# facebookresearch/momentum

Hardware: AMD Instinct MI355X
Metric: character IK solves/sec (72-joint, 10 GN iters) (higher is better)
Workload: dtype f32; 1 GPU; BASELINE configs[1]: B x 72-joint humanoid, P=128, pos+ori on 16 landmarks (M=192), GN lambda=0.05, 10 it; batch_per_gpu=4096, global_batch=4096, joints=72, params=128, rows=192, solved_parameters=96, route=fused, line_search=0, precision=f32

## Files before the change

include/mmx.h:

```cpp
#ifndef MMX_H_
#define MMX_H_

#include <stddef.h>
#include <stdint.h>

#ifdef __cplusplus
extern "C" {
#endif

#define MMX_ABI_VERSION 12
#define MMX_PARAMS_PER_JOINT 7
#define MMX_INVALID_PARENT (-1)
#define MMX_MAX_MODEL_PARAMS 2048

typedef enum mmx_status {
  MMX_OK = 0,
  MMX_ERR_INVALID_ARGUMENT = 1,
  MMX_ERR_SIZE_MISMATCH = 2,
  MMX_ERR_DEVICE = 3,
  MMX_ERR_UNSUPPORTED = 4,
  MMX_ERR_OUT_OF_MEMORY = 5,
  MMX_ERR_NO_DEVICE = 6
} mmx_status;

// ... 106 lines not shown
  float limit_function_weight;
  float pos_loss_alpha, pos_loss_c;
  float ori_loss_alpha, ori_loss_c;
  int32_t num_joint_blocks;
  const mmx_joint_constraint_block* joint_blocks;
  int32_t num_ellipsoid_limits;
  const mmx_ellipsoid_limit* ellipsoid_limits;
  const float* function_weights;
  int32_t num_function_weights;
} mmx_constraint_data;

#define MMX_LINE_SEARCH_NONE 0
#define MMX_LINE_SEARCH_GAUSS_NEWTON 1
#define MMX_LINE_SEARCH_DIRECTIONAL 2

typedef struct mmx_gn_options {
  int32_t min_iterations;
  int32_t max_iterations;
  float threshold;
  float regularization;
  int32_t do_line_search;
  int32_t step_rule;
  float lm_lambda_min;
  float lm_lambda_max;
  float lm_up;
  float lm_down;
  float trust_region_radius;
  int32_t precision;
  float precision_bound;
} mmx_gn_options;

typedef struct mmx_rig mmx_rig;
typedef struct mmx_problem mmx_problem;

void mmx_gn_options_default(mmx_gn_options* opt);

int32_t mmx_abi_version(void);
const char* mmx_last_error(void);
int32_t mmx_device_count(void);

int32_t mmx_rig_create(const mmx_rig_desc* desc, int32_t device, mmx_rig** out);
void mmx_rig_destroy(mmx_rig* rig);
int32_t mmx_rig_num_joints(const mmx_rig* rig);
int32_t mmx_rig_num_params(const mmx_rig* rig);

int32_t mmx_problem_create(
    mmx_rig* rig,
    int32_t batch,
    int32_t num_pos,
    const int32_t* pos_parent,
    int32_t num_ori,
    const int32_t* ori_parent,
    mmx_problem** out);
void mmx_problem_destroy(mmx_problem* problem);

int32_t mmx_problem_set_instance_rig(
    mmx_problem* problem,
    const float* translation_offset,
    const float* pre_rotation,
    int32_t memory,
    void* stream);

int32_t mmx_problem_set_instance_parents(
    mmx_problem* problem,
    const int32_t* pos_parent,
    const int32_t* ori_parent,
    int32_t memory,
    void* stream);

#define MMX_ROUTE_AUTO 0
#define MMX_ROUTE_FUSED 1
#define MMX_ROUTE_WIDE 2
#define MMX_ROUTE_EXPLICIT_JACOBIAN 3
#define MMX_ROUTE_WAVE 4
#define MMX_WAVE_MAX_JOINTS 64
#define MMX_WAVE_MAX_SOLVED 32
#define MMX_WAVE_MAX_UNITS 192
typedef struct mmx_tuning {
  int32_t route;
  int32_t max_refinement_steps;
  float mixed_tolerance;
  int32_t mixed_max_cg;
  int32_t joint_pruning;
  int32_t reserved[3];
} mmx_tuning;
int32_t mmx_problem_set_tuning(mmx_problem* problem, const mmx_tuning* tuning);
int32_t mmx_problem_last_route(const mmx_problem* problem);
int32_t mmx_problem_num_solve_joints(const mmx_problem* problem);

int32_t mmx_problem_num_rows(const mmx_problem* problem);
int32_t mmx_problem_batch(const mmx_problem* problem);

int32_t mmx_problem_set_enabled(mmx_problem* problem, const uint8_t* enabled);

int32_t mmx_problem_set_constraints(
    mmx_problem* problem,
    const mmx_constraint_data* data,
    void* stream);
int32_t mmx_problem_set_constraints_sized(
    mmx_problem* problem,
    const mmx_constraint_data* data,
    size_t data_size,
    void* stream);

int32_t mmx_eval_jacobian(
    mmx_problem* problem,
    const float* theta_dev,
    float* jac_dev,
    float* res_dev,
    double* err_dev,
    int32_t layout,
    void* stream);

int32_t mmx_eval_jacobian_timed(
    mmx_problem* problem,
    const float* theta_dev,
    float* jac_dev,
    float* res_dev,
    double* err_dev,
    int32_t layout,
    void* stream,
    float* kernel_ms);

int32_t mmx_debug_store_pattern(mmx_problem* problem, float* jac_dev, void* stream, float* kernel_ms);

int32_t mmx_eval_skeleton_state(
    mmx_problem* problem,
    const float* theta_dev,
    float* state_dev,
    void* stream);

int32_t mmx_eval_normal_equations(
    mmx_problem* problem,
    const float* theta_dev,
    float* jtj_dev,
    float* jtr_dev,
    double* err_dev,
    void* stream);

int32_t mmx_solve(
    mmx_problem* problem,
    const mmx_gn_options* options,
    float* theta_dev,
    double* final_error,
    int32_t* iterations,
    int32_t* status,
    double* error_history,
    void* stream);

int32_t mmx_solve_f64(
    mmx_problem* problem,
    const mmx_gn_options* options,
    double* theta_dev,
    double* final_error,
    int32_t* iterations,
    int32_t* status,
    double* error_history,
    void* stream);

int32_t mmx_solve_with_history(
    mmx_problem* problem,
    const mmx_gn_options* options,
    float* theta_dev,
    double* final_error,
    int32_t* iterations,
    int32_t* status,
    double* error_history,
    float* parameter_history,
    void* stream);

int32_t mmx_solve_with_step_history(
// ... 9 lines not shown
    void* stream);

int32_t mmx_solve_frames(
    mmx_problem* problem,
    const mmx_gn_options* options,
    int32_t num_frames,
    float* theta_dev,
    double* final_error,
    int32_t* iterations,
    int32_t* status,
    double* error_history,
    float* parameter_history,
    void* stream);
int32_t mmx_solve_frames_host(
    mmx_problem* problem,
    const mmx_gn_options* options,
    int32_t num_frames,
    float* theta_host,
    double* final_error_host,
    int32_t* iterations_host,
    int32_t* status_host);

int32_t mmx_problem_solve_diagnostics(mmx_problem* problem, float* diag_dev, void* stream);

int32_t mmx_debug_fused_normal_equations(
    mmx_problem* problem,
    const float* theta_dev,
    float* jtj_dev,
    float* jtr_dev,
    int32_t* solve_list_host,
    int32_t* num_solved,
    void* stream);

int32_t mmx_debug_tree_normal_equations(mmx_problem* problem, const float* theta_dev, float* jtj_dev, float* jtr_dev, void* stream);

int32_t mmx_solve_host(
    mmx_problem* problem,
    const mmx_gn_options* options,
    float* theta_host,
    double* final_error_host,
    int32_t* iterations_host,
    int32_t* status_host);
int32_t mmx_solve_f64_host(
    mmx_problem* problem,
    const mmx_gn_options* options,
    double* theta_host,
    double* final_error_host,
    int32_t* iterations_host,
    int32_t* status_host);
int32_t mmx_eval_jacobian_host(
    mmx_problem* problem,
    const float* theta_host,
    float* jac_host,
    float* res_host,
    double* err_host,
    int32_t layout);
int32_t mmx_eval_skeleton_state_host(mmx_problem* problem, const float* theta_host, float* state_host);

#define MMX_COMM_ID_BYTES 128
typedef struct mmx_comm mmx_comm;
int32_t mmx_comm_unique_id(uint8_t id[MMX_COMM_ID_BYTES]);
int32_t mmx_comm_create(const uint8_t id[MMX_COMM_ID_BYTES], int32_t world_size, int32_t rank, int32_t device, mmx_comm** out);
int32_t mmx_comm_create_all(int32_t num_devices, const int32_t* devices, mmx_comm** out );
int32_t mmx_comm_world_size(const mmx_comm* comm);
int32_t mmx_comm_rank(const mmx_comm* comm);
int32_t mmx_comm_all_reduce_norms(mmx_comm* comm, double* norms_dev, void* stream);
int32_t mmx_comm_all_reduce_norms_host(mmx_comm* comm, double norms_host[3]);
int32_t mmx_residual_norms(int32_t batch, const double* final_error, const int32_t* iterations, const int32_t* status, double* norms_dev, void* stream);
void mmx_comm_destroy(mmx_comm* comm);

int32_t mmx_host_tables(
    const mmx_rig_desc* desc,
    const uint8_t* enabled,
    int32_t* level,
    int32_t* tin,
    int32_t* tout,
    uint8_t* active_joint_params,
    int32_t* enabled_list,
    int32_t* num_enabled);

int32_t mmx_host_elimination_order(const mmx_rig_desc* desc, const uint8_t* enabled, int32_t* order, int32_t* num_enabled);
int32_t mmx_host_tile_structure(int32_t n, const uint8_t* related, uint32_t* row_mask, uint32_t* col_mask, int64_t* products);
int32_t mmx_host_live_joints(const mmx_rig_desc* desc, int32_t n, const int32_t* joints, uint8_t* live, int32_t* compact_of, int32_t* num_live);
int32_t mmx_problem_tile_structure(mmx_problem* problem, uint32_t* row_mask, uint32_t* col_mask, int32_t* num_blocks, int32_t* num_tiles, int64_t* products);
int32_t mmx_host_tile_level_schedule(int32_t n, const uint8_t* related, int32_t* steps);
int32_t mmx_host_f64_assembly_list(
    const mmx_rig_desc* desc,
    const int32_t* solve_list,
    int32_t n,
    const int32_t* pos_parent,
    int32_t num_pos,
    const int32_t* ori_parent,
    int32_t num_ori,
    int32_t units_per_chunk,
    uint32_t* groups,
    int32_t* num_groups,
    int32_t* extra,
    int32_t* num_extra,
    int32_t* chunk_start,
    int32_t* num_chunks);

#ifdef __cplusplus
}
#endif
#endif
```

momentum_amd/_abi.py:

```python
from __future__ import annotations

import ctypes as C

import numpy as np

c_float_p = C.POINTER(C.c_float)
c_double_p = C.POINTER(C.c_double)
c_int32_p = C.POINTER(C.c_int32)
c_uint8_p = C.POINTER(C.c_uint8)

MMX_ABI_VERSION = 12
MMX_OK = 0
MMX_SOLVE_OK, MMX_SOLVE_NONFINITE, MMX_SOLVE_NOT_PD = 0, 1, 2
MMX_SOLVE_DAMPING_FLOORED = 4
MMX_SOLVE_PRECISION_SUSPECT = 8
MMX_SOLVE_ESCALATED_F64 = 16
MMX_SOLVE_MIXED = 32
MMX_SOLVE_ERROR_MASK = 3
MMX_PRECISION_F32, MMX_PRECISION_F64, MMX_PRECISION_AUTO, MMX_PRECISION_MIXED = 0, 1, 2, 3
MMX_MEM_HOST, MMX_MEM_DEVICE = 0, 1
MMX_LAYOUT_COL_MAJOR, MMX_LAYOUT_ROW_MAJOR = 0, 1
MMX_STEP_GN_FIXED_LAMBDA, MMX_STEP_LM_SCHEDULE, MMX_STEP_TRUST_REGION = 0, 1, 2


# ... 219 lines not shown
        ("ori_weight", C.c_void_p),
        ("pos_function_weight", C.c_float),
        ("ori_function_weight", C.c_float),
        ("memory", C.c_int32),
        ("model_target", C.c_void_p),
        ("model_weights", C.c_void_p),
        ("model_function_weight", C.c_float),
        ("num_limits", C.c_int32),
        ("limits", C.c_void_p),
        ("limit_function_weight", C.c_float),
        ("pos_loss_alpha", C.c_float),
        ("pos_loss_c", C.c_float),
        ("ori_loss_alpha", C.c_float),
        ("ori_loss_c", C.c_float),
        ("num_joint_blocks", C.c_int32),
        ("joint_blocks", C.c_void_p),
        ("num_ellipsoid_limits", C.c_int32),
        ("ellipsoid_limits", C.c_void_p),
        ("function_weights", C.c_void_p),
        ("num_function_weights", C.c_int32),
    ]


class GnOptions(C.Structure):

    _fields_ = [
        ("min_iterations", C.c_int32),
        ("max_iterations", C.c_int32),
        ("threshold", C.c_float),
        ("regularization", C.c_float),
        ("do_line_search", C.c_int32),
        ("step_rule", C.c_int32),
        ("lm_lambda_min", C.c_float),
        ("lm_lambda_max", C.c_float),
        ("lm_up", C.c_float),
        ("lm_down", C.c_float),
        ("trust_region_radius", C.c_float),
        ("precision", C.c_int32),
        ("precision_bound", C.c_float),
    ]

    @classmethod
    def make(
        cls,
        min_iterations=1,
        max_iterations=2,
        threshold=1.0,
        regularization=0.05,
        do_line_search=False,
        step_rule=MMX_STEP_GN_FIXED_LAMBDA,
        lm_lambda_min=1e-6,
        lm_lambda_max=1e6,
        lm_up=4.0,
        lm_down=0.5,
        trust_region_radius=1.0,
        precision=MMX_PRECISION_F32,
        precision_bound=1e-5,
    ) -> "GnOptions":
        return cls(
            int(min_iterations),
            int(max_iterations),
            float(threshold),
            float(regularization),
            int(do_line_search),
            int(step_rule),
            float(lm_lambda_min),
            float(lm_lambda_max),
            float(lm_up),
            float(lm_down),
            float(trust_region_radius),
            int(precision),
            float(precision_bound),
        )


ROUTES = {"auto": 0, "fused": 1, "wide": 2, "explicit_jacobian": 3, "wave": 4}
WAVE_MAX_JOINTS = 64
WAVE_MAX_SOLVED = 32
WAVE_MAX_UNITS = 192


class Tuning(C.Structure):

    _fields_ = [("route", C.c_int32), ("max_refinement_steps", C.c_int32), ("mixed_tolerance", C.c_float), ("mixed_max_cg", C.c_int32), ("joint_pruning", C.c_int32), ("reserved", C.c_int32 * 3)]


def as_ptr(a: np.ndarray, ctype):
    assert a.flags["C_CONTIGUOUS"], "array must be C-contiguous"
    return a.ctypes.data_as(C.POINTER(ctype))


def void_p(a) -> C.c_void_p:
    if a is None:
        return C.c_void_p(0)
    if isinstance(a, np.ndarray):
        assert a.flags["C_CONTIGUOUS"]
        return C.c_void_p(a.ctypes.data)
    return C.c_void_p(int(a))
```

momentum_amd/capi.py:

```python
from __future__ import annotations

import ctypes as C
import os
from typing import Optional

import numpy as np

from . import _abi
from ._abi import ConstraintData, GnOptions, RigDesc, as_ptr
from .rigs import Rig

_HERE = os.path.dirname(os.path.abspath(__file__))
LIB_PATH = os.environ.get("MMX_LIB") or os.path.join(_HERE, "libmmx_hip.so")
_lib: Optional[C.CDLL] = None

SYMBOLS = [
    "mmx_gn_options_default", "mmx_abi_version", "mmx_last_error", "mmx_device_count",
    "mmx_rig_create", "mmx_rig_destroy", "mmx_rig_num_joints", "mmx_rig_num_params",
    "mmx_problem_create", "mmx_problem_destroy", "mmx_problem_num_rows", "mmx_problem_batch",
    "mmx_problem_set_tuning", "mmx_problem_last_route", "mmx_problem_num_solve_joints",
    "mmx_problem_set_enabled", "mmx_problem_set_constraints", "mmx_problem_set_constraints_sized", "mmx_problem_set_instance_rig", "mmx_problem_set_instance_parents", "mmx_eval_jacobian", "mmx_eval_jacobian_timed", "mmx_debug_store_pattern",
    "mmx_eval_skeleton_state", "mmx_eval_normal_equations", "mmx_solve", "mmx_solve_with_history", "mmx_solve_with_step_history", "mmx_problem_solve_diagnostics", "mmx_solve_f64", "mmx_solve_f64_host", "mmx_solve_host",
    "mmx_solve_frames", "mmx_solve_frames_host",
    "mmx_eval_jacobian_host", "mmx_eval_skeleton_state_host", "mmx_host_tables", "mmx_debug_fused_normal_equations", "mmx_debug_tree_normal_equations",
    "mmx_host_elimination_order", "mmx_host_tile_structure", "mmx_host_tile_level_schedule", "mmx_host_f64_assembly_list", "mmx_problem_tile_structure", "mmx_host_live_joints",
    "mmx_comm_unique_id", "mmx_comm_create", "mmx_comm_create_all", "mmx_comm_world_size", "mmx_comm_rank",
    "mmx_comm_all_reduce_norms", "mmx_comm_all_reduce_norms_host", "mmx_residual_norms", "mmx_comm_destroy",
]


class MmxError(RuntimeError):

    def __init__(self, code: int, msg: str):
        super().__init__(f"mmx error {code}: {msg}")
        self.code = code


def lib() -> C.CDLL:
    global _lib
    if _lib is not None:
        return _lib
    if not os.path.exists(LIB_PATH):
        raise MmxError(-1, f"{LIB_PATH} is missing: build it with `python -m momentum_amd.build` (no CPU fallback exists)")
    try:
        import torch
    except Exception:
        pass
    L = C.CDLL(LIB_PATH)
    vp, i32 = C.c_void_p, C.c_int32
    L.mmx_last_error.restype = C.c_char_p
    L.mmx_gn_options_default.restype = None
    L.mmx_gn_options_default.argtypes = [C.POINTER(GnOptions)]
    L.mmx_rig_create.argtypes = [C.POINTER(RigDesc), i32, C.POINTER(vp)]
    L.mmx_rig_destroy.argtypes = [vp]
    L.mmx_rig_destroy.restype = None
    L.mmx_rig_num_joints.argtypes = [vp]
    L.mmx_rig_num_params.argtypes = [vp]
    L.mmx_problem_create.argtypes = [vp, i32, i32, _abi.c_int32_p, i32, _abi.c_int32_p, C.POINTER(vp)]
    L.mmx_problem_destroy.argtypes = [vp]
    L.mmx_problem_destroy.restype = None
    L.mmx_problem_num_rows.argtypes = [vp]
    L.mmx_problem_batch.argtypes = [vp]
    L.mmx_problem_set_enabled.argtypes = [vp, _abi.c_uint8_p]
    L.mmx_problem_set_tuning.argtypes = [vp, C.POINTER(_abi.Tuning)]
    L.mmx_problem_last_route.argtypes = [vp]
    L.mmx_problem_num_solve_joints.argtypes = [vp]
    L.mmx_problem_set_constraints.argtypes = [vp, C.POINTER(ConstraintData), vp]
    L.mmx_problem_set_constraints_sized.argtypes = [vp, C.POINTER(ConstraintData), C.c_size_t, vp]
    L.mmx_problem_set_instance_rig.argtypes = [vp, vp, vp, i32, vp]
    L.mmx_problem_set_instance_parents.argtypes = [vp, vp, vp, i32, vp]
    L.mmx_eval_jacobian.argtypes = [vp, vp, vp, vp, vp, i32, vp]
    L.mmx_eval_jacobian_timed.argtypes = [vp, vp, vp, vp, vp, i32, vp, C.POINTER(C.c_float)]
    L.mmx_debug_store_pattern.argtypes = [vp, vp, vp, C.POINTER(C.c_float)]
    L.mmx_eval_skeleton_state.argtypes = [vp, vp, vp, vp]
    L.mmx_eval_normal_equations.argtypes = [vp, vp, vp, vp, vp, vp]
    L.mmx_solve.argtypes = [vp, C.POINTER(GnOptions), vp, vp, vp, vp, vp, vp]
    L.mmx_solve_with_history.argtypes = [vp, C.POINTER(GnOptions), vp, vp, vp, vp, vp, vp, vp]
    L.mmx_solve_with_step_history.argtypes = [vp, C.POINTER(GnOptions), vp, vp, vp, vp, vp, vp, vp, vp]
    L.mmx_problem_solve_diagnostics.argtypes = [vp, vp, vp]
    L.mmx_solve_f64.argtypes = [vp, C.POINTER(GnOptions), vp, vp, vp, vp, vp, vp]
    L.mmx_solve_host.argtypes = [vp, C.POINTER(GnOptions), vp, vp, vp, vp]
    L.mmx_solve_f64_host.argtypes = [vp, C.POINTER(GnOptions), vp, vp, vp, vp]
    L.mmx_solve_frames.argtypes = [vp, C.POINTER(GnOptions), i32, vp, vp, vp, vp, vp, vp, vp]
    L.mmx_solve_frames_host.argtypes = [vp, C.POINTER(GnOptions), i32, vp, vp, vp, vp]
    L.mmx_eval_jacobian_host.argtypes = [vp, vp, vp, vp, vp, i32]
    L.mmx_eval_skeleton_state_host.argtypes = [vp, vp, vp]
    L.mmx_debug_tree_normal_equations.argtypes = [vp, vp, vp, vp, vp]
    L.mmx_debug_fused_normal_equations.argtypes = [vp, vp, vp, vp, _abi.c_int32_p, _abi.c_int32_p, vp]
    L.mmx_comm_unique_id.argtypes = [vp]
    L.mmx_comm_create.argtypes = [vp, i32, i32, i32, C.POINTER(vp)]
    L.mmx_comm_create_all.argtypes = [i32, _abi.c_int32_p, C.POINTER(vp)]
    L.mmx_comm_world_size.argtypes = [vp]
    L.mmx_comm_rank.argtypes = [vp]
    L.mmx_comm_all_reduce_norms.argtypes = [vp, vp, vp]
    L.mmx_comm_all_reduce_norms_host.argtypes = [vp, vp]
    L.mmx_residual_norms.argtypes = [i32, vp, vp, vp, vp, vp]
    L.mmx_comm_destroy.argtypes = [vp]
    L.mmx_comm_destroy.restype = None
    L.mmx_host_tables.argtypes = [
        C.POINTER(RigDesc), _abi.c_uint8_p, _abi.c_int32_p, _abi.c_int32_p, _abi.c_int32_p,
        _abi.c_uint8_p, _abi.c_int32_p, _abi.c_int32_p,
    ]
    u32p, i64p = C.POINTER(C.c_uint32), C.POINTER(C.c_int64)
    L.mmx_host_elimination_order.argtypes = [C.POINTER(RigDesc), _abi.c_uint8_p, _abi.c_int32_p, _abi.c_int32_p]
    L.mmx_host_tile_structure.argtypes = [i32, _abi.c_uint8_p, u32p, u32p, i64p]
    L.mmx_host_tile_level_schedule.argtypes = [i32, _abi.c_uint8_p, C.POINTER(C.c_int32)]
    L.mmx_problem_tile_structure.argtypes = [vp, u32p, u32p, _abi.c_int32_p, _abi.c_int32_p, i64p]
    L.mmx_host_live_joints.argtypes = [C.POINTER(RigDesc), i32, _abi.c_int32_p, _abi.c_uint8_p, _abi.c_int32_p, _abi.c_int32_p]
    _lib = L
    return L


def _check(rc: int) -> None:
    if rc != 0:
        raise MmxError(rc, lib().mmx_last_error().decode("utf-8", "replace"))


def device_count() -> int:
    return int(lib().mmx_device_count())


def host_tables(rig: Rig, enabled=None) -> dict:
    J, P = rig.num_joints, rig.num_params
    level, tin, tout = (np.zeros(J, np.int32) for _ in range(3))
    active = np.zeros(7 * J, np.uint8)
    elist = np.zeros(P, np.int32)
    n = C.c_int32(0)
    d = rig.desc()
    if enabled is None:
        eptr = _abi.c_uint8_p()
    else:
        e = np.ascontiguousarray(enabled, dtype=np.uint8)
        eptr = as_ptr(e, C.c_uint8)
    _check(
        lib().mmx_host_tables(
            C.byref(d), eptr, as_ptr(level, C.c_int32), as_ptr(tin, C.c_int32), as_ptr(tout, C.c_int32),
            as_ptr(active, C.c_uint8), as_ptr(elist, C.c_int32), C.byref(n),
        )
    )
    order = np.zeros(P, np.int32)
    _check(lib().mmx_host_elimination_order(C.byref(d), eptr, as_ptr(order, C.c_int32), C.byref(n)))
    return dict(level=level, tin=tin, tout=tout, active_joint_params=active, enabled_list=elist[: n.value].copy(),
                elimination_order=order[: n.value].copy())


def host_live_joints(rig: Rig, joints) -> dict:
    J = rig.num_joints
    jl = np.ascontiguousarray(joints, dtype=np.int32).reshape(-1)
    live, compact = np.zeros(J, np.uint8), np.zeros(J, np.int32)
    n = C.c_int32(0)
    d = rig.desc()
    jptr = as_ptr(jl, C.c_int32) if jl.size else _abi.c_int32_p()
    _check(lib().mmx_host_live_joints(C.byref(d), C.c_int32(jl.size), jptr, as_ptr(live, C.c_uint8), as_ptr(compact, C.c_int32), C.byref(n)))
    return dict(live=live, compact_of=compact, num_live=int(n.value))


def host_tile_structure(related: np.ndarray):
    rel = np.ascontiguousarray(related, dtype=np.uint8)
    n = rel.shape[0]
    assert rel.shape == (n, n)
    row, col = np.zeros(32, np.uint32), np.zeros(32, np.uint32)
    prod = C.c_int64(0)
    _check(lib().mmx_host_tile_structure(C.c_int32(n), as_ptr(rel, C.c_uint8), as_ptr(row, C.c_uint32), as_ptr(col, C.c_uint32), C.byref(prod)))
    return dict(row_mask=row, col_mask=col, products=prod.value)


def host_tile_level_schedule(related: np.ndarray):
    rel = np.ascontiguousarray(related, dtype=np.uint8)
    n = rel.shape[0]
    assert rel.shape == (n, n)
    words = np.zeros(1 + 4 * 32, np.int32)
    _check(lib().mmx_host_tile_level_schedule(C.c_int32(n), as_ptr(rel, C.c_uint8), as_ptr(words, C.c_int32)))
    steps = []
    for s in range(int(words[0])):
        steps.append([(int(w) & 0xff, (int(w) >> 8) & 0xf, (int(w) >> 12) & 0xf) for w in words[1 + 4 * s : 5 + 4 * s] if w >= 0])
    return steps


def host_f64_assembly_list(rig: Rig, solve_list, pos_parent, ori_parent, units_per_chunk: int):
    sl = np.ascontiguousarray(solve_list, dtype=np.int32)
    pp = np.ascontiguousarray(pos_parent, dtype=np.int32)
    op = np.ascontiguousarray(ori_parent, dtype=np.int32)
    d = rig.desc()
    ng, ne, nc = C.c_int32(0), C.c_int32(0), C.c_int32(0)
    i32p = C.POINTER(C.c_int32)
    args = lambda g, e, cs: (C.byref(d), as_ptr(sl, C.c_int32), C.c_int32(len(sl)), as_ptr(pp, C.c_int32), C.c_int32(len(pp)), as_ptr(op, C.c_int32),
                             C.c_int32(len(op)), C.c_int32(units_per_chunk), g, C.byref(ng), e, C.byref(ne), cs, C.byref(nc))
    f = lib().mmx_host_f64_assembly_list
    f.restype = C.c_int32
    _check(f(*args(None, None, None)))
    groups = np.zeros(2 * max(ng.value, 1), np.uint32)
    extra = np.zeros(max(ne.value, 1), np.int32)
    cstart = np.zeros(2 * nc.value + 1, np.int32)
    _check(f(*args(groups.ctypes.data_as(C.POINTER(C.c_uint32)), extra.ctypes.data_as(i32p), cstart.ctypes.data_as(i32p))))
    chunks = []
    for ch in range(nc.value):
        entries = []
        for g in range(cstart[ch], cstart[ch + 1]):
            w0, w1 = int(groups[2 * g]), int(groups[2 * g + 1])
            c, ul, count = w0 & 0xfff, (w0 >> 12) & 0x3f, w0 >> 18
            entries.append((c, ul, [w1] if count == 1 else [int(x) for x in extra[w1 : w1 + count]]))
        chunks.append(dict(block_mask=int(cstart[nc.value + 1 + ch]), entries=entries))
    return chunks


def _stream_ptr() -> C.c_void_p:
    import torch

    return C.c_void_p(torch.cuda.current_stream().cuda_stream)


def _dev(t) -> C.c_void_p:
    return C.c_void_p(0 if t is None else t.data_ptr())


class RigHandle:

    def __init__(self, rig: Rig, device: int = 0):
        self.rig = rig
        self.device = int(device)
        self._h = C.c_void_p(0)
        d = rig.desc()
        _check(lib().mmx_rig_create(C.byref(d), self.device, C.byref(self._h)))

    def close(self) -> None:
        if self._h:
            lib().mmx_rig_destroy(self._h)
            self._h = C.c_void_p(0)

    def __del__(self):
        try:
            self.close()
        except Exception:
            pass


default_route = "auto"


class Problem:

    def __init__(self, rig_handle: RigHandle, batch: int, pos_parent, ori_parent):
        import torch

        self.rh = rig_handle
        self.B = int(batch)
        self.P = rig_handle.rig.num_params
        self.J = rig_handle.rig.num_joints
        self.pos_parent = np.ascontiguousarray(pos_parent, dtype=np.int32).reshape(-1)
        self.ori_parent = np.ascontiguousarray(ori_parent, dtype=np.int32).reshape(-1)
        self.Kp, self.Ko = len(self.pos_parent), len(self.ori_parent)
        self.M = 3 * self.Kp + 9 * self.Ko
        self.n = self.P
        self.device = torch.device("cuda", rig_handle.device)
        self._h = C.c_void_p(0)
        self._keep = []
        _check(
            lib().mmx_problem_create(
                rig_handle._h, self.B, self.Kp, as_ptr(self.pos_parent, C.c_int32), self.Ko,
                as_ptr(self.ori_parent, C.c_int32), C.byref(self._h),
            )
        )
        self._prefer_wide = default_route == "prefer_wide"
        if default_route not in ("auto", "prefer_wide"):
            self.set_route(default_route)

    def close(self) -> None:
        if self._h:
            lib().mmx_problem_destroy(self._h)
            self._h = C.c_void_p(0)

    def __del__(self):
        try:
            self.close()
        except Exception:
            pass

    def set_route(self, route: str, max_refinement_steps: int = 0) -> None:
        self._prefer_wide = default_route == "prefer_wide" and route == "auto"
        self._set_tuning(route, max_refinement_steps)

    def _set_tuning(self, route: str, max_refinement_steps: int = 0) -> None:
        t = _abi.Tuning()
        t.route = _abi.ROUTES[route]
        t.max_refinement_steps = int(max_refinement_steps)
        t.mixed_tolerance, t.mixed_max_cg = getattr(self, "_mixed", (0.0, 0))
        t.joint_pruning = 0 if getattr(self, "_joint_pruning", True) else -1
        self._route_args = (route, int(max_refinement_steps))
        _check(lib().mmx_problem_set_tuning(self._h, C.byref(t)))

    def set_mixed(self, tolerance: float = 0.0, max_cg: int = 0) -> None:
        self._mixed = (float(tolerance), int(max_cg))
        self._set_tuning(*getattr(self, "_route_args", ("auto", 0)))

    def set_joint_pruning(self, on: bool = True) -> None:
        self._joint_pruning = bool(on)
        self._set_tuning(*getattr(self, "_route_args", ("auto", 0)))

    def num_solve_joints(self) -> int:
        return int(lib().mmx_problem_num_solve_joints(self._h))

    def last_route(self) -> str:
        r = int(lib().mmx_problem_last_route(self._h))
        return {v: k for k, v in _abi.ROUTES.items()}[r]

    def set_enabled(self, enabled) -> None:
        e = np.ascontiguousarray(enabled, dtype=np.uint8).reshape(-1)
        assert e.shape[0] == self.P
        _check(lib().mmx_problem_set_enabled(self._h, as_ptr(e, C.c_uint8)))
        self.n = int(np.count_nonzero(e))

    def set_constraints(
        self, pos_offset, pos_target, pos_weight, ori_offset, ori_target, ori_weight,
        pos_function_weight: float = 1.0, ori_function_weight: float = 1.0,
        limits=None, limit_function_weight: float = 1.0,
        model_target=None, model_weights=None, model_function_weight: float = 1.0,
        pos_loss=(2.0, 1.0), ori_loss=(2.0, 1.0), joint_blocks=None, ellipsoid_limits=None, function_weights=None,
    ) -> None:
        import torch

        arrs = [pos_offset, pos_target, pos_weight, ori_offset, ori_target, ori_weight]
        shapes = [(self.B, self.Kp, 3), (self.B, self.Kp, 3), (self.B, self.Kp), (self.B, self.Ko, 4), (self.B, self.Ko, 4), (self.B, self.Ko)]
        if model_target is not None:
            arrs += [model_target, model_weights]
            shapes += [(self.B, self.P), (self.B, self.P)]
        on_dev = all(isinstance(a, torch.Tensor) for a in arrs)
        keep, ptrs = [], []
        for a, shp in zip(arrs, shapes):
            if on_dev:
                assert a.is_cuda and a.dtype == torch.float32 and a.is_contiguous() and tuple(a.shape) == shp, (a.shape, shp)
                keep.append(a)
                ptrs.append(C.c_void_p(a.data_ptr() if a.numel() else 0))
            else:
                x = np.ascontiguousarray(a, dtype=np.float32).reshape(shp)
                keep.append(x)
                ptrs.append(C.c_void_p(x.ctypes.data if x.size else 0))
        if model_target is None:
            ptrs += [C.c_void_p(0), C.c_void_p(0)]
        fw_ptr, fw_cols = C.c_void_p(0), 0
        if function_weights is not None:
            if on_dev:
                assert function_weights.is_cuda and function_weights.dtype == torch.float32 and function_weights.is_contiguous() and function_weights.shape[0] == self.B
                keep.append(function_weights)
                fw_ptr, fw_cols = C.c_void_p(function_weights.data_ptr()), int(function_weights.shape[1])
            else:
                fwh = np.ascontiguousarray(function_weights, dtype=np.float32).reshape(self.B, -1)
                keep.append(fwh)
                fw_ptr, fw_cols = C.c_void_p(fwh.ctypes.data), int(fwh.shape[1])
        limits = list(limits) if limits else []
        larr = _abi.limit_array(limits)
        blocks = list(joint_blocks) if joint_blocks else []
        bkeep: list = []
        barr = _abi.joint_block_array(blocks, bkeep, self.B, on_dev)
        ells = list(ellipsoid_limits) if ellipsoid_limits else []
        earr = _abi.ellipsoid_array(ells)
        cd = ConstraintData(
            *ptrs[:6], float(pos_function_weight), float(ori_function_weight), _abi.MMX_MEM_DEVICE if on_dev else _abi.MMX_MEM_HOST,
            ptrs[6], ptrs[7], float(model_function_weight), len(limits), C.cast(larr, C.c_void_p) if limits else None, float(limit_function_weight),
            float(pos_loss[0]), float(pos_loss[1]), float(ori_loss[0]), float(ori_loss[1]),
            len(blocks), C.cast(barr, C.c_void_p) if blocks else None,
            len(ells), C.cast(earr, C.c_void_p) if ells else None,
            fw_ptr, fw_cols,
        )
        _check(lib().mmx_problem_set_constraints_sized(self._h, C.byref(cd), C.sizeof(cd), _stream_ptr()))
        self._keep = keep + bkeep if on_dev else []
        self.M = int(lib().mmx_problem_num_rows(self._h))

    def set_instance_rig(self, translation_offset=None, pre_rotation=None) -> None:
        self._keep_rig = self._instance_call(
            lib().mmx_problem_set_instance_rig, [(translation_offset, (self.B, self.J, 3)), (pre_rotation, (self.B, self.J, 4))], "float32"
        )

    def set_instance_parents(self, pos_parent=None, ori_parent=None) -> None:
        self._keep_parents = self._instance_call(
            lib().mmx_problem_set_instance_parents, [(pos_parent, (self.B, self.Kp)), (ori_parent, (self.B, self.Ko))], "int32"
        )

    def _instance_call(self, fn, arrays, dtype):
        import torch

# ... 285 lines not shown
```

momentum_amd/csrc/mmx_capi.hip:

```cpp
#include "../../include/mmx.h"

#include <hip/hip_runtime.h>

#include <dlfcn.h>

#include <cfloat>
#include <cmath>
#include <cstdio>
#include <cstdlib>
#include <cstring>
#include <algorithm>
#include <new>
#include <map>
#include <memory>
#include <string>
#include <vector>

#include "mmx_host_tables.hpp"
#include "mmx_kernels.hpp"

namespace {

thread_local std::string g_lastError;

// ... 112 lines not shown

struct mmx_rig {
  int32_t device = 0;
  int32_t J = 0, P = 0;
  std::vector<int32_t> parent, ptOuter, ptInner;
  std::vector<float> preRot, offset, ptValue, ptOffsets;
  mmx::HostTables topo;
  DevBuf dParent, dPreRot, dOffset, dPtOuter, dPtInner, dPtValue, dPtOffsets, dLevelOrder, dLevelStart, dPtEll, dJumpParent, dPtRowRec;
  mmx::RigDev dev{};

  mmx_rig_desc desc() const {
    mmx_rig_desc d{};
    d.num_joints = J;
    d.num_params = P;
    d.parent = parent.data();
    d.pre_rotation = preRot.data();
    d.translation_offset = offset.data();
    d.pt_outer = ptOuter.data();
    d.pt_inner = ptInner.data();
    d.pt_value = ptValue.data();
    d.pt_offsets = ptOffsets.data();
    return d;
  }
};

struct mmx_problem {
  mmx_rig* rig = nullptr;
  int32_t B = 0, Kp = 0, Ko = 0, U = 0, M = 0;
  std::vector<int32_t> posParent, oriParent;
  mmx::RigDev rigDev{};
  DevBuf oInstOffset, oInstPreRot, oInstPosParent, oInstOriParent, dJointTin;
  std::vector<int32_t> unionPos, unionOri;
  std::vector<int32_t> instPosHost, instOriHost;
  bool instParentsFromHost = false;
  bool instPos = false, instOri = false;
  mmx::HostTables tables;
  mmx::FusedTables fused;
  DevBuf dUnitJoint, dUnitTin, dColStart, dColSources, dEnabledList, dJacRecs, dMultiCols, dZeroCols;
  DevBuf dSubSize, dPosUnitStart, dPosUnits, dSolveList, dSrcStart, dSrcs, dTerms, dTerms16, dComb, dDfsJoint, dLoadedPos;
  DevBuf dLimStart, dLimOf, dPairDest, dPairStart, dPairLim, dPairCols;
  mmx::FusedDev fdev{};
  DevBuf oPosOffset, oPosTarget, oPosWeight, oOriOffset, oOriTarget, oOriWeight, oMpTarget, oMpWeights, dLimits, dEnabledMask, oFnWeights;
  std::vector<mmx_parameter_limit> limits;
  struct JointBlockHost {
    int32_t type = 0, count = 0;
    std::vector<int32_t> parent;
    std::vector<int32_t> parentB;
    DevBuf oLocalPoint, oLocalDir, oGlobal, oPlaneD, oWeight, oProjection;
  };
  std::vector<std::unique_ptr<JointBlockHost>> blocks;
  std::vector<mmx::JointBlockDev> blockDev;
  std::vector<mmx_ellipsoid_limit> ellipsoids;
  DevBuf dEllipsoids;
  DevBuf dBlocks, dGenJoint, dGenTin, dGenBlock;
  int32_t genRows = 0;
  bool haveConstraints = false;
  bool tablesDirty = false;
  mmx::ProblemDev dev{};
  int32_t solveN = 0;
  DevBuf dSolveListV1;
  DevBuf sHess2F64;
  DevBuf dSolveListF64;
  std::vector<int32_t> solveListF64;
  std::vector<std::pair<int32_t, int32_t>> limitPairs;
  DevBuf dTileMasks, dTileList;
  mmx::TileMasks tileMasks;
  std::vector<int32_t> solveListV1;
  DevBuf sJac, sRes, sErr, sJtj, sJtr, sFactor, sThetaInit, sTheta;
  DevBuf sTreeState, sDvec, sRhoVec, sRefState, sGenState;
  DevBuf sJacColMajor;
  DevBuf sJacF64, sHessF64;
  DevBuf dF64Groups, dF64Extra, dF64ChunkStart;
  int32_t f64ListUnitsPerChunk = 0;
  DevBuf sDone, sIters, sStatus, sLastErr, sFinalErr, sHist, sClk, sDelta, sStepIter, sLambda, sTrust;
  DevBuf sFusedArgs;
  DevBuf sDiag;
  DevBuf sDiagAcc;
  DevBuf sDiagErr0;
  bool diagValid = false;
  DevBuf sThetaAuto, sAutoMap, sAutoCount;
  bool autoAbort = false;
  mmx_tuning tuning{};
  int32_t lastRoute = MMX_ROUTE_AUTO;
  mmx::LiveJoints liveJoints;
  bool viewBuilt = false;
  mmx::RigDev vRig{};
  int32_t vNnz = 0;
  DevBuf vParent, vPreRot, vOffset, vPtOuter, vPtInner, vPtValue, vPtOffsets, vLevelOrder, vLevelStart, vPtEll, vJumpParent, vPtRowRec;
  DevBuf vUnitJoint, vUnitTin, vJointTin, vGenJoint, vGenTin, vEllipsoids, vLimits;
  DevBuf vSubSize, vDfsJoint, vLoadedPos, vPosUnitStart, vSrcs;
};

namespace {

std::vector<int32_t> limitParameters(const mmx_rig* rig, const mmx_parameter_limit& lm) {
  std::vector<int32_t> out;
  auto add = [&](int32_t p) {
    if (std::find(out.begin(), out.end(), p) == out.end()) {
      out.push_back(p);
    }
  };
  auto addRow = [&](int32_t row) {
    for (int32_t k = rig->ptOuter[size_t(row)]; k < rig->ptOuter[size_t(row) + 1]; ++k) {
      add(rig->ptInner[size_t(k)]);
    }
  };
  switch (lm.type) {
    case MMX_LIMIT_MINMAX:
      add(lm.index0);
      break;
    case MMX_LIMIT_LINEAR:
    case MMX_LIMIT_HALFPLANE:
      add(lm.index0);
      add(lm.index1);
      break;
    case MMX_LIMIT_MINMAX_JOINT:
      addRow(lm.index0);
      break;
    case MMX_LIMIT_LINEAR_JOINT:
      addRow(lm.index1);
      addRow(lm.index0);
      break;
    default:
      break;
  }
  return out;
}

struct RigDerived {
  std::vector<int32_t> ell, jumpParent, rowRec;
  bool ellOk = true;
  int32_t jumpRounds = 0;
};
RigDerived deriveRigTables(
    int32_t J, int32_t P, const std::vector<int32_t>& parent, const std::vector<int32_t>& ptOuter, const std::vector<int32_t>& ptInner,
    const std::vector<float>& ptValue, int32_t numLevels) {
  RigDerived o;
  const int32_t R = MMX_PARAMS_PER_JOINT * J;
  o.ell.assign(size_t(R) * 4, 0);
  o.jumpParent.assign(size_t(J), 0);
  for (int32_t row = 0; row < R; ++row) {
    const int32_t k0 = ptOuter[size_t(row)], k1 = ptOuter[size_t(row) + 1];
    if (k1 - k0 > 2) {
      o.ellOk = false;
      break;
    }
    for (int s = 0; s < 2; ++s) {
      int32_t idx = -1, bits = 0;
      if (k0 + s < k1) {
        idx = ptInner[size_t(k0 + s)];
        std::memcpy(&bits, &ptValue[size_t(k0 + s)], 4);
      }
      o.ell[4 * size_t(row) + 2 * s] = idx;
      o.ell[4 * size_t(row) + 2 * s + 1] = bits;
    }
  }
  for (int32_t j = 0; j < J; ++j) {
    o.jumpParent[size_t(j)] = ((parent[size_t(j)] + 1) << 16) | (parent[size_t(j)] + 1);
  }
  if (R < 65536 && P <= 65535) {
    std::vector<int32_t> rows;
    for (int32_t row = 0; row < R; ++row) {
      if (ptOuter[size_t(row) + 1] > ptOuter[size_t(row)]) {
        rows.push_back(row);
      }
    }
// ... 1228 lines not shown
  if (batch <= 0 || num_pos < 0 || num_ori < 0) {
    return fail(MMX_ERR_INVALID_ARGUMENT, "batch must be > 0 and constraint counts >= 0");
  }
  if ((num_pos > 0 && pos_parent == nullptr) || (num_ori > 0 && ori_parent == nullptr)) {
    return fail(MMX_ERR_INVALID_ARGUMENT, "constraint parent array is null");
  }
  for (int32_t c = 0; c < num_pos; ++c) {
    if (pos_parent[c] < 0 || pos_parent[c] >= rig->J) {
      return fail(MMX_ERR_INVALID_ARGUMENT, "position constraint parent joint out of range");
    }
  }
  for (int32_t c = 0; c < num_ori; ++c) {
    if (ori_parent[c] < 0 || ori_parent[c] >= rig->J) {
      return fail(MMX_ERR_INVALID_ARGUMENT, "orientation constraint parent joint out of range");
    }
  }
  mmx_problem* pb = new (std::nothrow) mmx_problem();
  if (pb == nullptr) {
    return fail(MMX_ERR_OUT_OF_MEMORY, "host allocation failed");
  }
  pb->rig = rig;
  pb->B = batch;
  pb->Kp = num_pos;
  pb->Ko = num_ori;
  pb->U = num_pos + 3 * num_ori;
  pb->M = 3 * pb->U;
  pb->dev.lossPos = mmx::LossDev{0, 2.f, 1.f, 1.f};
  pb->dev.lossOri = mmx::LossDev{0, 2.f, 1.f, 1.f};
  if (num_pos > 0) {
    pb->posParent.assign(pos_parent, pos_parent + num_pos);
  }
  if (num_ori > 0) {
    pb->oriParent.assign(ori_parent, ori_parent + num_ori);
  }
  pb->tables = rig->topo;
  pb->rigDev = rig->dev;
  pb->dev.wPos = 1.f;
  pb->dev.wOri = 1.f;
  const int32_t rc = uploadProblemTables(pb);
  if (rc != MMX_OK) {
    delete pb;
    return rc;
  }
  *out = pb;
  return MMX_OK;
}

void mmx_problem_destroy(mmx_problem* pb) {
  if (pb != nullptr) {
    if (pb->rig != nullptr) {
      (void)hipSetDevice(pb->rig->device);
    }
    delete pb;
  }
}

int32_t mmx_problem_num_rows(const mmx_problem* pb) {
  return pb ? pb->M : 0;
}
int32_t mmx_problem_batch(const mmx_problem* pb) {
  return pb ? pb->B : 0;
}

int32_t mmx_problem_set_tuning(mmx_problem* pb, const mmx_tuning* tuning) {
  int32_t rc = checkProblem(pb, false);
  if (rc != MMX_OK) {
    return rc;
  }
  if (tuning == nullptr) {
    return fail(MMX_ERR_INVALID_ARGUMENT, "tuning is null");
  }
  if (tuning->route < MMX_ROUTE_AUTO || tuning->route > MMX_ROUTE_WAVE) {
    return fail(MMX_ERR_INVALID_ARGUMENT, "mmx_tuning::route: unknown MMX_ROUTE_* value");
  }
  if (tuning->max_refinement_steps < -1 || tuning->max_refinement_steps > 3) {
    return fail(MMX_ERR_INVALID_ARGUMENT, "mmx_tuning::max_refinement_steps: -1 (none), 0 (default) or 1..3");
  }
  if (!(tuning->mixed_tolerance >= 0.f) || tuning->mixed_tolerance > 1e-2f || tuning->mixed_max_cg < 0 || tuning->mixed_max_cg > 64) {
    return fail(MMX_ERR_INVALID_ARGUMENT, "mmx_tuning::mixed_tolerance: 0 (default) or (0, 1e-2]; mixed_max_cg: 0 (default) or 1..64");
  }
  if (tuning->joint_pruning != 0 && tuning->joint_pruning != -1) {
    return fail(MMX_ERR_INVALID_ARGUMENT, "mmx_tuning::joint_pruning: 0 (on) or -1 (off)");
  }
  for (int32_t r : tuning->reserved) {
    if (r != 0) {
      return fail(MMX_ERR_INVALID_ARGUMENT, "mmx_tuning::reserved must be zero");
    }
  }
  pb->tuning = *tuning;
  return MMX_OK;
}

int32_t mmx_problem_last_route(const mmx_problem* pb) {
  return pb != nullptr ? pb->lastRoute : MMX_ROUTE_AUTO;
}

int32_t mmx_problem_num_solve_joints(const mmx_problem* pb) {
  if (pb == nullptr || pb->rig == nullptr) {
    return 0;
  }
  return solveViewActive(pb) ? pb->liveJoints.numLive : pb->rig->J;
}

int32_t mmx_problem_set_enabled(mmx_problem* pb, const uint8_t* enabled) {
  MMX_ZONE("mmx_problem_set_enabled");
  int32_t rc = checkProblem(pb, false);
  if (rc != MMX_OK) {
    return rc;
  }
  if (enabled == nullptr) {
    return fail(MMX_ERR_INVALID_ARGUMENT, "enabled is null");
  }
  if (!pb->tablesDirty && pb->tables.enabled.size() == size_t(pb->rig->P)) {
    bool same = true;
    for (size_t p = 0; p < pb->tables.enabled.size() && same; ++p) {
      same = (pb->tables.enabled[p] != 0) == (enabled[p] != 0);
    }
    if (same) {
      return MMX_OK;
    }
  }
  const mmx_rig_desc d = pb->rig->desc();
  std::string err;
  mmx::HostTables t;
  rc = mmx::buildHostTables(&d, enabled, t, err);
  if (rc != MMX_OK) {
    return fail(rc, err);
  }
  pb->tables = std::move(t);
  return uploadProblemTables(pb);
}

int32_t mmx_problem_set_instance_rig(mmx_problem* pb, const float* translation_offset, const float* pre_rotation, int32_t memory, void* stream) {
  MMX_ZONE("mmx_problem_set_instance_rig");
  int32_t rc = checkProblem(pb, false);
  if (rc != MMX_OK) {
    return rc;
  }
  if (memory != MMX_MEM_HOST && memory != MMX_MEM_DEVICE) {
    return fail(MMX_ERR_INVALID_ARGUMENT, "instance rig: unknown memory space");
  }
  MMX_HIP(hipSetDevice(pb->rig->device));
  hipStream_t s = static_cast<hipStream_t>(stream);
  const size_t B = size_t(pb->B), J = size_t(pb->rig->J);
  auto bring = [&](DevBuf& buf, const float* src, size_t count, const float*& dst) -> hipError_t {
    if (src == nullptr) {
      dst = nullptr;
      return hipSuccess;
    }
    if (memory == MMX_MEM_DEVICE) {
      dst = src;
      return hipSuccess;
    }
    hipError_t e = buf.ensure(count * sizeof(float));
    if (e != hipSuccess) {
      return e;
    }
    dst = buf.as<float>();
    return hipMemcpyAsync(buf.p, src, count * sizeof(float), hipMemcpyHostToDevice, s);
  };
  const float *off = nullptr, *pre = nullptr;
  MMX_HIP(bring(pb->oInstOffset, translation_offset, B * J * 3, off));
  MMX_HIP(bring(pb->oInstPreRot, pre_rotation, B * J * 4, pre));
  if (memory == MMX_MEM_HOST) {
    MMX_HIP(hipStreamSynchronize(s));
  }
  pb->rigDev.instOffset = off;
  pb->rigDev.instPreRot = pre;
  return MMX_OK;
}

int32_t mmx_problem_set_instance_parents(mmx_problem* pb, const int32_t* pos_parent, const int32_t* ori_parent, int32_t memory, void* stream) {
  MMX_ZONE("mmx_problem_set_instance_parents");
  int32_t rc = checkProblem(pb, false);
  if (rc != MMX_OK) {
    return rc;
  }
  if (memory != MMX_MEM_HOST && memory != MMX_MEM_DEVICE) {
    return fail(MMX_ERR_INVALID_ARGUMENT, "instance parents: unknown memory space");
  }
  MMX_HIP(hipSetDevice(pb->rig->device));
  hipStream_t s = static_cast<hipStream_t>(stream);
  const size_t B = size_t(pb->B);
  std::vector<int32_t> hp, ho;
// ... 658 lines not shown
    double* error_history,
    double* step_history,
    const mmx::F64Select& select,
    void* stream);
static int32_t preflightF64(mmx_problem* pb);

static bool mixedUsable(const mmx_problem* pb, const mmx_gn_options* o) {
  if (o == nullptr || pb == nullptr || pb->rig == nullptr) {
    return false;
  }
  const int32_t route = pb->tuning.route;
  return (route == MMX_ROUTE_AUTO || route == MMX_ROUTE_FUSED) && o->step_rule != MMX_STEP_TRUST_REGION && pb->fdev.GT == 0 &&
      pb->U > 0 && pb->fdev.n > 0 && fusedUsable(pb) &&
      mmx::fusedMixedUsable(pb->rig->J, pb->rig->P, pb->U, pb->fdev.nsrc, pb->fdev.n, pb->fdev.numCells);
}

static const char* waveRefusal(const mmx_problem* pb, const mmx_gn_options* o, bool frames = false) {
  const mmx::ProblemDev& d = pb->dev;
  if (pb->rig->J > MMX_WAVE_MAX_JOINTS) {
    return "MMX_ROUTE_WAVE: more than MMX_WAVE_MAX_JOINTS (64) joints";
  }
  if (pb->fdev.n > MMX_WAVE_MAX_SOLVED) {
    return "MMX_ROUTE_WAVE: more than MMX_WAVE_MAX_SOLVED (32) solved parameters";
  }
  if (pb->fdev.n <= 0 || pb->U <= 0) {
    return "MMX_ROUTE_WAVE: no solved parameter, or no position / orientation constraint";
  }
  if (pb->U > MMX_WAVE_MAX_UNITS) {
    return "MMX_ROUTE_WAVE: more than MMX_WAVE_MAX_UNITS (192) constraint vectors (positions + 3 x orientations)";
  }
  if (d.lossPos.type != 0 || d.lossOri.type != 0) {
    return "MMX_ROUTE_WAVE: robust losses are outside the route (L2 only)";
  }
  if (d.numBlocks > 0 || d.G > 0 || pb->fdev.GT > 0) {
    return "MMX_ROUTE_WAVE: further joint-constraint blocks are outside the route";
  }
  if (d.NE > 0) {
    return "MMX_ROUTE_WAVE: ellipsoid limits are outside the route";
  }
  if (d.NL > 0) {
    return "MMX_ROUTE_WAVE: parameter limits are outside the route";
  }
  if (d.hasModel != 0 || d.M > d.rowsJoint) {
    return "MMX_ROUTE_WAVE: the model-parameter prior is outside the route";
  }
  if (d.instPosParent != nullptr || d.instOriParent != nullptr) {
    return "MMX_ROUTE_WAVE: per-instance constraint parents are outside the route";
  }
  if (o->step_rule != MMX_STEP_GN_FIXED_LAMBDA) {
    return "MMX_ROUTE_WAVE: only MMX_STEP_GN_FIXED_LAMBDA (not the LM schedule, not the trust region)";
  }
  if (mmx::waveLdsBytes(pb->rig->J, pb->rig->P, pb->U, pb->fdev.n, frames) > 160 * 1024) {
    return "MMX_ROUTE_WAVE: the parameter vector does not fit a wave's share of LDS";
  }
  return nullptr;
}

static int32_t solveMixedImpl(
    mmx_problem* pb,
    const mmx_gn_options* o,
    float* theta_dev,
    double* final_error,
    int32_t* iterations,
    int32_t* status,
    double* error_history,
    float* parameter_history,
    double* step_history,
    const mmx::MixSelect& sel,
    void* stream) {
  MMX_ZONE("mmx_solve, mixed precision (SolverT<double>::solve around a single-precision factor)");
  if (o->max_iterations < 0 || o->min_iterations < 0) {
    return fail(MMX_ERR_INVALID_ARGUMENT, "iteration counts must be >= 0");
  }
  if (o->step_rule != MMX_STEP_GN_FIXED_LAMBDA && o->step_rule != MMX_STEP_LM_SCHEDULE) {
    return fail(MMX_ERR_INVALID_ARGUMENT, "unknown step_rule");
  }
  if (o->do_line_search != MMX_LINE_SEARCH_NONE && o->do_line_search != MMX_LINE_SEARCH_GAUSS_NEWTON && o->do_line_search != MMX_LINE_SEARCH_DIRECTIONAL) {
    return fail(MMX_ERR_INVALID_ARGUMENT, "unknown do_line_search rule");
  }
  const size_t B = size_t(pb->B), P = size_t(pb->rig->P);
  hipStream_t s = static_cast<hipStream_t>(stream);
  const bool escalation = sel.map != nullptr;
  pb->lastRoute = MMX_ROUTE_FUSED;
  MMX_HIP(pb->sIters.ensure(B * sizeof(int32_t)));
  MMX_HIP(pb->sStatus.ensure(B * sizeof(int32_t)));
  MMX_HIP(pb->sFinalErr.ensure(B * sizeof(double)));
  mmx::SolveStateDev fst{};
  fst.iterations = iterations != nullptr ? iterations : pb->sIters.as<int32_t>();
  fst.status = status != nullptr ? status : pb->sStatus.as<int32_t>();
  fst.finalError = final_error != nullptr ? final_error : pb->sFinalErr.as<double>();
  fst.errorHistory = error_history;
  fst.paramHistory = parameter_history;
  fst.stepHistory = step_history;
  if (!escalation) {
    MMX_HIP(pb->sDiag.ensure(B * 4 * sizeof(float)));
    fst.diag = pb->sDiag.as<float>();
    pb->diagValid = true;
    if (step_history != nullptr && o->max_iterations > 0) {
      MMX_HIP(mmx::zeroAsync(step_history, B * size_t(o->max_iterations) * 2 * sizeof(double), s));
    }
    if (error_history != nullptr && o->max_iterations > 0) {
      MMX_HIP(mmx::zeroAsync(error_history, B * size_t(o->max_iterations) * sizeof(double), s));
    }
    if (parameter_history != nullptr && o->max_iterations > 0) {
      MMX_HIP(mmx::zeroAsync(parameter_history, B * size_t(o->max_iterations) * P * sizeof(float), s));
    }
  }
  fst.precisionBound = o->precision_bound > 0.f ? o->precision_bound : 1e-5f;
  mmx::FusedParams fp{};
  fp.lambda = o->regularization;
  fp.threshold = o->threshold;
  fp.minIterations = o->min_iterations;
  fp.maxIterations = o->max_iterations;
  fp.refine = 0;
  fp.doLineSearch = o->do_line_search;
  fp.stepRule = o->step_rule;
  fp.lmLambdaMin = o->lm_lambda_min;
  fp.lmLambdaMax = o->lm_lambda_max;
  fp.lmUp = o->lm_up;
  fp.lmDown = o->lm_down;
  fp.trustRadius = 1.f;
  fp.mixTol = pb->tuning.mixed_tolerance > 0.f ? pb->tuning.mixed_tolerance : 3e-9f;
  fp.mixMaxCg = pb->tuning.mixed_max_cg > 0 ? pb->tuning.mixed_max_cg : 12;
  long long* clk = nullptr;
  if (phaseClocksWanted()) {
    MMX_HIP(pb->sClk.ensure(32 * sizeof(long long)));
    MMX_HIP(hipMemsetAsync(pb->sClk.p, 0, 32 * sizeof(long long), s));
    clk = pb->sClk.as<long long>();
    MMX_HIP(armPhaseStop(clk, s));
  }
  const SolveView sv = solveView(pb);
  MMX_HIP(mmx::launchFusedMixed(sv.rig, sv.pb, sv.fd, theta_dev, fst, fp, sel, pb->B, clk, s));
  if (clk != nullptr) {
    long long h[32];
    MMX_HIP(hipMemcpyAsync(h, clk, sizeof(h), hipMemcpyDeviceToHost, s));
    MMX_HIP(hipStreamSynchronize(s));
    static const char* names[24] = {"-", "A-C fk + units (double)", "(reused state)", "D subtree sums", "E srcTables", "F g (double adjoint)",
                                    "G combine + pull", "H cholesky(tail)", "-", "-", "K update",
                                    "G extras: records", "G term records", "H.bc panel", "H.d mfma", "D own sums", "CG z0 solve + rz",
                                    "CG operator (double)", "CG decide + direction", "CG dots + update", "CG solve", "G extras: loads", "H.b load+barrier", "H.b chain"};
    long long tot = 0;
    for (int i = 0; i < 24; ++i) {
      tot += h[i];
    }
    fprintf(stderr, "[mmx phase clocks, MIXED, block 0, all iterations] total %lld\n", tot);
    for (int i = 0; i < 24; ++i) {
      fprintf(stderr, "  %-26s %10lld  %5.1f%%\n", names[i], h[i], 100.0 * double(h[i]) / double(tot > 0 ? tot : 1));
    }
  }
  return MMX_OK;
}

static int32_t solveImpl(
    mmx_problem* pb,
    const mmx_gn_options* o,
    float* theta_dev,
    double* final_error,
    int32_t* iterations,
    int32_t* status,
    double* error_history,
    float* parameter_history,
    double* step_history,
    void* stream) {
  if (o == nullptr || o->precision == MMX_PRECISION_F32) {
    return solveF32Impl(pb, o, theta_dev, final_error, iterations, status, error_history, parameter_history, step_history, stream);
  }
// ... 21 lines not shown
    return solveMixedImpl(pb, o, theta_dev, final_error, iterations, status, error_history, parameter_history, step_history, mmx::MixSelect{nullptr, nullptr, nullptr}, stream);
  }
  const bool autoTrust = o->precision == MMX_PRECISION_AUTO && o->step_rule == MMX_STEP_TRUST_REGION;
  if (o->precision == MMX_PRECISION_F64 || o->precision == MMX_PRECISION_MIXED || autoTrust) {
    return solveF64Impl(pb, o, nullptr, final_error, iterations, status, error_history, step_history, mmx::F64Select{nullptr, nullptr, theta_dev, theta_dev}, stream);
  }
  rc = preflightF64(pb);
  if (rc != MMX_OK) {
    return rc;
  }
  MMX_HIP(pb->sThetaAuto.ensure(B * P * sizeof(float)));
  MMX_HIP(pb->sAutoMap.ensure(B * sizeof(int32_t)));
  MMX_HIP(pb->sAutoCount.ensure(sizeof(int32_t)));
  MMX_HIP(pb->sStatus.ensure(B * sizeof(int32_t)));
  MMX_HIP(hipMemcpyAsync(pb->sThetaAuto.p, theta_dev, B * P * sizeof(float), hipMemcpyDeviceToDevice, s));
  int32_t* st = status != nullptr ? status : pb->sStatus.as<int32_t>();
  pb->autoAbort = mixedOk;
  rc = solveF32Impl(pb, o, theta_dev, final_error, iterations, st, error_history, nullptr, step_history, stream);
  pb->autoAbort = false;
  if (rc != MMX_OK) {
    return rc;
  }
  const int32_t mask = MMX_SOLVE_ERROR_MASK | MMX_SOLVE_PRECISION_SUSPECT | (pb->diagValid ? 0 : MMX_SOLVE_DAMPING_FLOORED);
  MMX_HIP(mmx::launchSelectSuspect(st, pb->B, mask, pb->sAutoMap.as<int32_t>(), pb->sAutoCount.as<int32_t>(), s));
  if (mixedOk) {
    rc = solveMixedImpl(
        pb, o, theta_dev, final_error, iterations, st, error_history, nullptr, step_history,
        mmx::MixSelect{pb->sAutoMap.as<int32_t>(), pb->sAutoCount.as<int32_t>(), pb->sThetaAuto.as<float>()}, stream);
    if (rc != MMX_OK) {
      return rc;
    }
    MMX_HIP(mmx::launchSelectSuspect(st, pb->B, MMX_SOLVE_ERROR_MASK | MMX_SOLVE_PRECISION_SUSPECT, pb->sAutoMap.as<int32_t>(), pb->sAutoCount.as<int32_t>(), s, MMX_SOLVE_MIXED));
  }
  return solveF64Impl(
      pb, o, nullptr, final_error, iterations, st, error_history, step_history,
      mmx::F64Select{pb->sAutoMap.as<int32_t>(), pb->sAutoCount.as<int32_t>(), pb->sThetaAuto.as<float>(), theta_dev}, stream);
}

static int32_t solveF32Impl(
    mmx_problem* pb,
    const mmx_gn_options* o,
    float* theta_dev,
    double* final_error,
    int32_t* iterations,
    int32_t* status,
    double* error_history,
    float* parameter_history,
    double* step_history,
    void* stream) {
  MMX_ZONE("mmx_solve (SolverT::solve)");
  int32_t rc = checkProblem(pb, true);
  if (rc != MMX_OK) {
    return rc;
  }
  if (o == nullptr || theta_dev == nullptr) {
    return fail(MMX_ERR_INVALID_ARGUMENT, "options / theta is null");
  }
  if (o->max_iterations < 0 || o->min_iterations < 0) {
    return fail(MMX_ERR_INVALID_ARGUMENT, "iteration counts must be >= 0");
  }
  if (o->step_rule != MMX_STEP_GN_FIXED_LAMBDA && o->step_rule != MMX_STEP_LM_SCHEDULE && o->step_rule != MMX_STEP_TRUST_REGION) {
    return fail(MMX_ERR_INVALID_ARGUMENT, "unknown step_rule");
  }
  if (o->do_line_search != MMX_LINE_SEARCH_NONE && o->do_line_search != MMX_LINE_SEARCH_GAUSS_NEWTON &&
      o->do_line_search != MMX_LINE_SEARCH_DIRECTIONAL) {
    return fail(MMX_ERR_INVALID_ARGUMENT, "unknown do_line_search rule");
  }
  const size_t B = size_t(pb->B), P = size_t(pb->rig->P);
  mmx::ProblemDev ds = pb->dev;
  ds.n = pb->solveN;
  ds.enabledList = pb->dSolveListV1.as<int32_t>();
  const int n = ds.n;
  MMX_HIP(hipSetDevice(pb->rig->device));
  hipStream_t s = static_cast<hipStream_t>(stream);
  const int32_t route = pb->tuning.route;
  if (route == MMX_ROUTE_WAVE) {
    if (const char* why = waveRefusal(pb, o)) {
      return fail(MMX_ERR_UNSUPPORTED, why);
    }
    if (step_history != nullptr) {
      return fail(MMX_ERR_UNSUPPORTED, "MMX_ROUTE_WAVE: step_history is the LM schedule's");
    }
    pb->lastRoute = MMX_ROUTE_WAVE;
    pb->diagValid = false;
    MMX_HIP(pb->sIters.ensure(B * sizeof(int32_t)));
    MMX_HIP(pb->sStatus.ensure(B * sizeof(int32_t)));
    MMX_HIP(pb->sFinalErr.ensure(B * sizeof(double)));
    mmx::SolveStateDev wst{};
    wst.iterations = iterations != nullptr ? iterations : pb->sIters.as<int32_t>();
    wst.status = status != nullptr ? status : pb->sStatus.as<int32_t>();
    wst.finalError = final_error != nullptr ? final_error : pb->sFinalErr.as<double>();
    wst.errorHistory = error_history;
    wst.paramHistory = parameter_history;
    if (error_history != nullptr && o->max_iterations > 0) {
      MMX_HIP(mmx::zeroAsync(error_history, B * size_t(o->max_iterations) * sizeof(double), s));
    }
    if (parameter_history != nullptr && o->max_iterations > 0) {
      MMX_HIP(mmx::zeroAsync(parameter_history, B * size_t(o->max_iterations) * P * sizeof(float), s));
    }
    mmx::FusedParams wp{};
    wp.lambda = o->regularization;
    wp.threshold = o->threshold;
    wp.minIterations = o->min_iterations;
    wp.maxIterations = o->max_iterations;
    wp.refine = refineSteps(pb);
    wp.doLineSearch = o->do_line_search;
    wp.stepRule = o->step_rule;
    MMX_ZONE("wave solve: all iterations in one launch, one wavefront per instance");
    const SolveView sv = solveView(pb);
    MMX_HIP(mmx::launchWaveSolve(sv.rig, sv.pb, sv.fd, theta_dev, wst, wp, s));
    return MMX_OK;
  }
  const bool forceWide = route == MMX_ROUTE_WIDE;
  const bool trust = o->step_rule == MMX_STEP_TRUST_REGION;
  const bool trustNeedsWide = trust && (!fusedUsable(pb) || pb->fdev.GT > 0);
  const bool preferWide = (forceWide || trustNeedsWide || (!trust && mmx::fusedBlocksFor(pb->fdev.n) >= 10)) &&
      treeNormalEquationsUsable(pb) && route != MMX_ROUTE_FUSED && route != MMX_ROUTE_EXPLICIT_JACOBIAN;
  const bool legacy = route == MMX_ROUTE_EXPLICIT_JACOBIAN;
  const bool takeFused = fusedUsable(pb) && !legacy && !preferWide && !(pb->fdev.GT > 0 && o->step_rule == MMX_STEP_TRUST_REGION);
  if (route == MMX_ROUTE_FUSED && !takeFused) {
    return fail(MMX_ERR_UNSUPPORTED, "MMX_ROUTE_FUSED: the problem does not fit the one-launch solve (more than 224 solved parameters, or its tables beyond the LDS budget)");
  }
  if (route == MMX_ROUTE_WIDE && !preferWide) {
    return fail(MMX_ERR_UNSUPPORTED, "MMX_ROUTE_WIDE: the problem is outside the tree kernels' scope");
  }
  if (takeFused) {
    pb->lastRoute = MMX_ROUTE_FUSED;
    MMX_HIP(pb->sIters.ensure(B * sizeof(int32_t)));
    MMX_HIP(pb->sStatus.ensure(B * sizeof(int32_t)));
    MMX_HIP(pb->sFinalErr.ensure(B * sizeof(double)));
    mmx::SolveStateDev fst{};
    fst.done = nullptr;
    fst.iterations = iterations != nullptr ? iterations : pb->sIters.as<int32_t>();
    fst.status = status != nullptr ? status : pb->sStatus.as<int32_t>();
    fst.lastError = nullptr;
    fst.finalError = final_error != nullptr ? final_error : pb->sFinalErr.as<double>();
    fst.errorHistory = error_history;
    fst.paramHistory = parameter_history;
    fst.stepHistory = step_history;
    MMX_HIP(pb->sDiag.ensure(B * 4 * sizeof(float)));
    fst.diag = pb->sDiag.as<float>();
    fst.precisionBound = o->precision_bound > 0.f ? o->precision_bound : 1e-5f;
    pb->diagValid = true;
    if (step_history != nullptr && o->max_iterations > 0) {
      MMX_HIP(mmx::zeroAsync(step_history, B * size_t(o->max_iterations) * 2 * sizeof(double), s));
    }
    if (error_history != nullptr && o->max_iterations > 0) {
      MMX_HIP(mmx::zeroAsync(error_history, B * size_t(o->max_iterations) * sizeof(double), s));
    }
    if (parameter_history != nullptr && o->max_iterations > 0) {
      MMX_HIP(mmx::zeroAsync(parameter_history, B * size_t(o->max_iterations) * P * sizeof(float), s));
    }
    mmx::FusedParams fp{};
    fp.lambda = o->regularization;
    fp.threshold = o->threshold;
    fp.minIterations = o->min_iterations;
    fp.maxIterations = o->max_iterations;
    fp.refine = refineSteps(pb);
    fp.doLineSearch = o->do_line_search;
    fp.stepRule = o->step_rule;
    fp.lmLambdaMin = o->lm_lambda_min;
    fp.lmLambdaMax = o->lm_lambda_max;
    fp.lmUp = o->lm_up;
    fp.lmDown = o->lm_down;
    fp.trustRadius = o->trust_region_radius > 0.f ? o->trust_region_radius : 1.f;
    fp.autoAbort = pb->autoAbort ? 1 : 0;
    long long* clk = nullptr;
    if (phaseClocksWanted()) {
      MMX_HIP(pb->sClk.ensure(32 * sizeof(long long)));
      MMX_HIP(hipMemsetAsync(pb->sClk.p, 0, 32 * sizeof(long long), s));
      clk = pb->sClk.as<long long>();
      MMX_HIP(armPhaseStop(clk, s));
    }
    {
      MMX_ZONE("fused solve: all iterations of GaussNewtonSolverT::doIteration in one launch");
      MMX_HIP(pb->sFusedArgs.ensure(mmx::fusedArgsBytes()));
      const SolveView sv = solveView(pb);
      MMX_HIP(mmx::launchFusedSolve(sv.rig, sv.pb, sv.fd, theta_dev, fst, fp, nullptr, nullptr, clk, pb->sFusedArgs.p, s));
    }
    if (clk != nullptr) {
      long long h[32];
      MMX_HIP(hipMemcpyAsync(h, clk, sizeof(h), hipMemcpyDeviceToHost, s));
      MMX_HIP(hipStreamSynchronize(s));
      static const char* names[24] = {"A jointParams", "B fk", "C units", "D subtree sums", "E srcTables", "F g + zero tiles",
                                      "G combine + pull", "H cholesky(tail)", "I solve", "J tail (d0 += rho)", "K update",
                                      "G extras: records", "G term records", "H.bc panel", "H.d mfma", "D own sums", "J jd",
                                      "J tangent+own", "J subtree", "J rho", "J solve", "G extras: loads", "H.b load+barrier", "H.b chain"};
      long long tot = h[24] + h[25] + h[26];
      for (int i = 0; i < 24; ++i) {
        tot += h[i];
      }
      fprintf(stderr, "[mmx phase clocks, block 0, all iterations] total %lld  (termRounds %d, numComb %d, nsrc %d, n %d)\n", tot, pb->fdev.termRounds, pb->fdev.numComb, pb->fdev.nsrc, pb->fdev.n);
      for (int i = 0; i < 24; ++i) {
        fprintf(stderr, "  %-16s %10lld  %5.1f%%\n", names[i], h[i], 100.0 * double(h[i]) / double(tot > 0 ? tot : 1));
      }
      fprintf(stderr, "  (of B fk: joint parameters %lld, local transforms %lld, pointer jumping %lld, axes = the rest of B)\n", h[26], h[24], h[25]);
    }
    return MMX_OK;
  }
  if (trust && !(preferWide && treeNormalEquationsUsable(pb) && route != MMX_ROUTE_EXPLICIT_JACOBIAN)) {
    return fail(MMX_ERR_UNSUPPORTED, "MMX_STEP_TRUST_REGION: available in the one-launch solve and on the wide route (tree kernels); this problem takes neither (MMX_ROUTE_EXPLICIT_JACOBIAN, or outside the tree kernels' scope)");
  }
  if (n > mmx::kMaxSolved) {
    return fail(MMX_ERR_UNSUPPORTED, "more than 2048 solved parameters (kMaxModelParams; 512 on the tree routes, the explicit-Jacobian route takes the rest)");
  }
  const bool wide = mmx::choleskyStepLdsBytes(ds.n, ds.M) > 160 * 1024;
  const bool treeRefine = (wide || preferWide) && treeNormalEquationsUsable(pb) && route != MMX_ROUTE_EXPLICIT_JACOBIAN;
  if (route == MMX_ROUTE_WIDE && !treeRefine) {
    return fail(MMX_ERR_UNSUPPORTED, "MMX_ROUTE_WIDE: the tree-refined wide solve is not available for this problem");
  }
  pb->lastRoute = treeRefine ? MMX_ROUTE_WIDE : MMX_ROUTE_EXPLICIT_JACOBIAN;
  rc = ensureStepScratch(pb, !treeRefine);
  if (rc != MMX_OK) {
    return rc;
  }
  MMX_HIP(pb->sThetaInit.ensure(B * P * sizeof(float)));
  MMX_HIP(pb->sDone.ensure(B * sizeof(int32_t)));
  MMX_HIP(pb->sIters.ensure(B * sizeof(int32_t)));
  MMX_HIP(pb->sStatus.ensure(B * sizeof(int32_t)));
  MMX_HIP(pb->sLastErr.ensure(B * sizeof(double)));
  MMX_HIP(pb->sFinalErr.ensure(B * sizeof(double)));
  mmx::SolveStateDev st{};
  st.done = pb->sDone.as<int32_t>();
  st.iterations = iterations != nullptr ? iterations : pb->sIters.as<int32_t>();
  st.status = status != nullptr ? status : pb->sStatus.as<int32_t>();
  st.lastError = pb->sLastErr.as<double>();
  st.finalError = final_error != nullptr ? final_error : pb->sFinalErr.as<double>();
  st.errorHistory = error_history;
  st.paramHistory = nullptr;
  st.stepHistory = step_history;
  pb->diagValid = false;
  if (step_history != nullptr && o->max_iterations > 0) {
    MMX_HIP(mmx::zeroAsync(step_history, B * size_t(o->max_iterations) * 2 * sizeof(double), s));
  }
  if (error_history != nullptr && o->max_iterations > 0) {
    MMX_HIP(mmx::zeroAsync(error_history, B * size_t(o->max_iterations) * sizeof(double), s));
  }
  MMX_HIP(hipMemcpyAsync(pb->sThetaInit.p, theta_dev, B * P * sizeof(float), hipMemcpyDeviceToDevice, s));
  const bool deferred = trust || o->do_line_search != 0 || o->step_rule == MMX_STEP_LM_SCHEDULE;
  const bool schedule = trust || o->step_rule == MMX_STEP_LM_SCHEDULE;
  if (deferred) {
    MMX_HIP(pb->sDelta.ensure(B * size_t(std::max(n, 1)) * sizeof(float)));
    MMX_HIP(pb->sStepIter.ensure(B * sizeof(int32_t)));
    MMX_HIP(mmx::zeroAsync(pb->sStepIter.p, B * sizeof(int32_t), s));
  }
  if (schedule) {
    MMX_HIP(pb->sLambda.ensure(B * sizeof(float)));
  }
  const bool wideDiag = treeRefine && !trust && refineSteps(pb) > 0;
  if (wideDiag) {
    MMX_HIP(pb->sDiag.ensure(B * 4 * sizeof(float)));
    MMX_HIP(pb->sDiagAcc.ensure(B * 4 * sizeof(float)));
    MMX_HIP(pb->sDiagErr0.ensure(B * sizeof(float)));
    st.diag = pb->sDiag.as<float>();
    st.precisionBound = o->precision_bound > 0.f ? o->precision_bound : 1e-5f;
    pb->diagValid = true;
  }
  MMX_HIP(mmx::launchSolveInit(st, pb->B, schedule ? pb->sLambda.as<float>() : nullptr, o->regularization, s, wideDiag ? pb->sDiagAcc.as<float>() : nullptr));
  mmx::StepParams sp{};
  sp.diagAcc = wideDiag ? pb->sDiagAcc.as<float>() : nullptr;
  sp.diagErr0 = wideDiag ? pb->sDiagErr0.as<float>() : nullptr;
  sp.lambda = o->regularization;
  sp.threshold = o->threshold;
  sp.minIterations = o->min_iterations;
  sp.maxIterations = o->max_iterations;
  sp.refine = refineSteps(pb);
  sp.tileMasks = pb->dTileMasks.as<uint32_t>();
  sp.numTiles = int32_t(pb->tileMasks.tiles.size());
  sp.delta = deferred ? pb->sDelta.as<float>() : nullptr;
  sp.stepIter = deferred ? pb->sStepIter.as<int32_t>() : nullptr;
  sp.lambdaPer = schedule ? pb->sLambda.as<float>() : nullptr;
  sp.stepHistory = step_history;
  sp.doLineSearch = trust ? 0 : o->do_line_search;
  sp.stepRule = o->step_rule;
  if (trust) {
    MMX_HIP(pb->sTrust.ensure(B * 6 * sizeof(int32_t) + 16));
    char* base = static_cast<char*>(pb->sTrust.p);
    sp.tr.lambda = reinterpret_cast<float*>(base);
    sp.tr.radius = reinterpret_cast<float*>(base + B * 4);
    sp.tr.phase = reinterpret_cast<int32_t*>(base + B * 8);
    sp.tr.newton = reinterpret_cast<int32_t*>(base + B * 12);
    sp.tr.step = reinterpret_cast<int32_t*>(base + B * 16);
    sp.tr.mask = reinterpret_cast<int32_t*>(base + B * 20);
    sp.tr.active = reinterpret_cast<int32_t*>(base + B * 24);
    MMX_HIP(mmx::launchTrustInit(sp.tr, pb->B, o->trust_region_radius > 0.f ? o->trust_region_radius : 1.f, s));
  }
  sp.lmLambdaMin = o->lm_lambda_min;
  sp.lmLambdaMax = o->lm_lambda_max;
  sp.lmUp = o->lm_up;
  sp.lmDown = o->lm_down;
  if (phaseClocksWanted()) {
    MMX_HIP(pb->sClk.ensure(32 * sizeof(long long)));
    MMX_HIP(hipMemsetAsync(pb->sClk.p, 0, 32 * sizeof(long long), s));
    sp.clk = pb->sClk.as<long long>();
// ... 305 lines not shown

int32_t mmx_solve_host(
    mmx_problem* pb,
    const mmx_gn_options* o,
    float* theta_host,
    double* final_error_host,
    int32_t* iterations_host,
    int32_t* status_host) {
  MMX_ZONE("mmx_solve_host");
  int32_t rc = checkProblem(pb, true);
  if (rc != MMX_OK) {
    return rc;
  }
  if (theta_host == nullptr) {
    return fail(MMX_ERR_INVALID_ARGUMENT, "theta is null");
  }
  const size_t B = size_t(pb->B), P = size_t(pb->rig->P);
  MMX_HIP(hipSetDevice(pb->rig->device));
  MMX_HIP(pb->sTheta.ensure(B * P * sizeof(float)));
  MMX_HIP(pb->sIters.ensure(B * sizeof(int32_t)));
  MMX_HIP(pb->sStatus.ensure(B * sizeof(int32_t)));
  MMX_HIP(pb->sFinalErr.ensure(B * sizeof(double)));
  MMX_HIP(hipMemcpy(pb->sTheta.p, theta_host, B * P * sizeof(float), hipMemcpyHostToDevice));
  rc = mmx_solve(pb, o, pb->sTheta.as<float>(), pb->sFinalErr.as<double>(), pb->sIters.as<int32_t>(), pb->sStatus.as<int32_t>(), nullptr, nullptr);
  if (rc != MMX_OK) {
    return rc;
  }
  MMX_HIP(hipDeviceSynchronize());
  MMX_HIP(hipMemcpy(theta_host, pb->sTheta.p, B * P * sizeof(float), hipMemcpyDeviceToHost));
  if (final_error_host) {
    MMX_HIP(hipMemcpy(final_error_host, pb->sFinalErr.p, B * sizeof(double), hipMemcpyDeviceToHost));
  }
  if (iterations_host) {
    MMX_HIP(hipMemcpy(iterations_host, pb->sIters.p, B * sizeof(int32_t), hipMemcpyDeviceToHost));
  }
  if (status_host) {
    MMX_HIP(hipMemcpy(status_host, pb->sStatus.p, B * sizeof(int32_t), hipMemcpyDeviceToHost));
  }
  return MMX_OK;
}

int32_t mmx_solve_frames(
    mmx_problem* pb,
    const mmx_gn_options* o,
    int32_t num_frames,
    float* theta_dev,
    double* final_error,
    int32_t* iterations,
    int32_t* status,
    double* error_history,
    float* parameter_history,
    void* stream) {
  MMX_ZONE("mmx_solve_frames (SolverT::solve per frame, warm-started along the sequence)");
  int32_t rc = checkProblem(pb, true);
  if (rc != MMX_OK) {
    return rc;
  }
  if (o == nullptr || theta_dev == nullptr) {
    return fail(MMX_ERR_INVALID_ARGUMENT, "options / theta is null");
  }
  if (num_frames < 1 || pb->B % num_frames != 0) {
    return fail(MMX_ERR_INVALID_ARGUMENT, "mmx_solve_frames: num_frames must be >= 1 and divide the problem's batch (num_frames x sequences instances, frame-major)");
  }
  if (o->max_iterations < 0 || o->min_iterations < 0) {
    return fail(MMX_ERR_INVALID_ARGUMENT, "iteration counts must be >= 0");
  }
  if (o->do_line_search != MMX_LINE_SEARCH_NONE && o->do_line_search != MMX_LINE_SEARCH_GAUSS_NEWTON &&
      o->do_line_search != MMX_LINE_SEARCH_DIRECTIONAL) {
    return fail(MMX_ERR_INVALID_ARGUMENT, "unknown do_line_search rule");
  }
  if (o->precision != MMX_PRECISION_F32) {
    return fail(MMX_ERR_UNSUPPORTED, "mmx_solve_frames runs on MMX_ROUTE_WAVE: only MMX_PRECISION_F32 (not F64 / AUTO / MIXED)");
  }
  if (pb->tuning.route != MMX_ROUTE_AUTO && pb->tuning.route != MMX_ROUTE_WAVE) {
    return fail(MMX_ERR_UNSUPPORTED, "mmx_solve_frames runs on the one-wavefront route only: the handle's route is pinned to another (MMX_ROUTE_AUTO or MMX_ROUTE_WAVE)");
  }
  if (const char* why = waveRefusal(pb, o, true)) {
    return fail(MMX_ERR_UNSUPPORTED, why);
  }
  const size_t B = size_t(pb->B), P = size_t(pb->rig->P);
  MMX_HIP(hipSetDevice(pb->rig->device));
  hipStream_t s = static_cast<hipStream_t>(stream);
  pb->lastRoute = MMX_ROUTE_WAVE;
  pb->diagValid = false;
  MMX_HIP(pb->sIters.ensure(B * sizeof(int32_t)));
  MMX_HIP(pb->sStatus.ensure(B * sizeof(int32_t)));
  MMX_HIP(pb->sFinalErr.ensure(B * sizeof(double)));
  mmx::SolveStateDev wst{};
  wst.iterations = iterations != nullptr ? iterations : pb->sIters.as<int32_t>();
  wst.status = status != nullptr ? status : pb->sStatus.as<int32_t>();
  wst.finalError = final_error != nullptr ? final_error : pb->sFinalErr.as<double>();
  wst.errorHistory = error_history;
  wst.paramHistory = parameter_history;
  if (error_history != nullptr && o->max_iterations > 0) {
    MMX_HIP(mmx::zeroAsync(error_history, B * size_t(o->max_iterations) * sizeof(double), s));
  }
  if (parameter_history != nullptr && o->max_iterations > 0) {
    MMX_HIP(mmx::zeroAsync(parameter_history, B * size_t(o->max_iterations) * P * sizeof(float), s));
  }
  mmx::FusedParams wp{};
  wp.lambda = o->regularization;
  wp.threshold = o->threshold;
  wp.minIterations = o->min_iterations;
  wp.maxIterations = o->max_iterations;
  wp.refine = refineSteps(pb);
  wp.doLineSearch = o->do_line_search;
  wp.stepRule = o->step_rule;
  const SolveView sv = solveView(pb);
  MMX_HIP(mmx::launchWaveFrames(sv.rig, sv.pb, sv.fd, theta_dev, wst, wp, num_frames, s));
  return MMX_OK;
}

int32_t mmx_solve_frames_host(
    mmx_problem* pb,
    const mmx_gn_options* o,
    int32_t num_frames,
    float* theta_host,
    double* final_error_host,
    int32_t* iterations_host,
    int32_t* status_host) {
  MMX_ZONE("mmx_solve_frames_host");
  int32_t rc = checkProblem(pb, true);
  if (rc != MMX_OK) {
    return rc;
  }
  if (theta_host == nullptr) {
    return fail(MMX_ERR_INVALID_ARGUMENT, "theta is null");
  }
  const size_t B = size_t(pb->B), P = size_t(pb->rig->P);
  MMX_HIP(hipSetDevice(pb->rig->device));
  MMX_HIP(pb->sTheta.ensure(B * P * sizeof(float)));
  MMX_HIP(pb->sIters.ensure(B * sizeof(int32_t)));
  MMX_HIP(pb->sStatus.ensure(B * sizeof(int32_t)));
  MMX_HIP(pb->sFinalErr.ensure(B * sizeof(double)));
  MMX_HIP(hipMemcpy(pb->sTheta.p, theta_host, B * P * sizeof(float), hipMemcpyHostToDevice));
  rc = mmx_solve_frames(pb, o, num_frames, pb->sTheta.as<float>(), pb->sFinalErr.as<double>(), pb->sIters.as<int32_t>(), pb->sStatus.as<int32_t>(), nullptr, nullptr, nullptr);
  if (rc != MMX_OK) {
    return rc;
  }
  MMX_HIP(hipDeviceSynchronize());
  MMX_HIP(hipMemcpy(theta_host, pb->sTheta.p, B * P * sizeof(float), hipMemcpyDeviceToHost));
  if (final_error_host) {
    MMX_HIP(hipMemcpy(final_error_host, pb->sFinalErr.p, B * sizeof(double), hipMemcpyDeviceToHost));
  }
  if (iterations_host) {
    MMX_HIP(hipMemcpy(iterations_host, pb->sIters.p, B * sizeof(int32_t), hipMemcpyDeviceToHost));
  }
  if (status_host) {
    MMX_HIP(hipMemcpy(status_host, pb->sStatus.p, B * sizeof(int32_t), hipMemcpyDeviceToHost));
  }
  return MMX_OK;
}

int32_t mmx_solve_f64_host(
    mmx_problem* pb,
    const mmx_gn_options* o,
    double* theta_host,
    double* final_error_host,
    int32_t* iterations_host,
    int32_t* status_host) {
  MMX_ZONE("mmx_solve_f64_host");
  int32_t rc = checkProblem(pb, true);
  if (rc != MMX_OK) {
    return rc;
  }
  if (theta_host == nullptr) {
// ... 91 lines not shown
```

momentum_amd/csrc/mmx_fused.hip:

```cpp
#include "mmx_device.hpp"
#include "mmx_kernels.hpp"
#include "mmx_mixed.hpp"
#include "mmx_tree.hpp"

#include <cfloat>
#include <cstdlib>

namespace mmx {

struct FusedLds {
  int16_t* mStart;
  int* mTin;
  int* mInfo;
  float* mW;
  float* th;
  float* js;
  float* up;
  float* ur;
  float* uy;
  float* us;
  float* own1;
  float* sub1;
  float* g;
  float* d0;
  float* rho;
  float* invDiag;
  float* dfull;
  float* jd;
  float* tanOwn;
  float* tanPre;
  double* red;
  int* flags;
  float* gEv;
  float* gRes;
  float* gW;
  float* gJ;
  double* fkA;
  double* fkB;
  float* own2;
  float* umom;
  float* sub2;
  float* L;
  float* srcT;
};

struct RigView {
  int32_t J, P, R, numLevels, jumpRounds;
  const int32_t* parent;
  const float* preRot;
  const float* offset;
  const int32_t* ptOuter;
  const int32_t* ptInner;
  const float* ptValue;
  const float* ptOffsets;
  bool hasOffsets;
  const int32_t* levelOrder;
  const int32_t* levelStart;
  const int4* rowRec;
  int32_t numRowRec;
};
template <class I>
struct FusedViewT {
  int32_t U, Kp;
  const I* subSize;
  const I* dfsJoint;
  const I* loadedPos;
  int32_t numLoaded;
  const I* colToSolve;
  const I* unitPos;
  const I* posUnitStart;
  const I* posUnits;
  const I* solveList;
};
using FusedView = FusedViewT<int32_t>;
using FusedViewS = FusedViewT<int16_t>;

__host__ __device__ __forceinline__ size_t alignUp4(size_t x) {
  return (x + 3) & ~size_t(3);
}
__host__ __device__ __forceinline__ int srcStrideFor(int nsrc) {
  int x = (nsrc + 15) & ~15;
  return (x & 31) == 16 ? x : x + 16;
}
constexpr int kSrcCh = 15;

__device__ __forceinline__ void firstOrderMoments(float* o, F3 p, float yx, float yy, float yz, bool point) {
  o[3] = p.y * yz - p.z * yy;
  o[4] = p.z * yx - p.x * yz;
  o[5] = p.x * yy - p.y * yx;
  o[0] = point ? yx : 0.f;
  o[1] = point ? yy : 0.f;
  o[2] = point ? yz : 0.f;
  o[6] = point ? p.x * yx + p.y * yy + p.z * yz : 0.f;
}

template <int NCH, int STRIDE, int kT = 256, class FV = FusedView, bool kSecondOnly = false>
__device__ __forceinline__ void gatherOwnSums(const FV& fd, const FusedLds& s, const float* umom, int tid) {
  for (int item = tid; item < fd.numLoaded * NCH; item += kT) {
    const int li = item / NCH, c = item - li * NCH;
    const int k = fd.loadedPos[li];
    float acc = 0.f;
    const int e1 = fd.posUnitStart[k + 1];
    for (int e = fd.posUnitStart[k]; e < e1; ++e) {
      acc += umom[STRIDE * fd.posUnits[e] + c];
    }
    if (kSecondOnly) {
      s.own2[kC2 * k + c] = acc;
    } else if (c < kC1) {
      s.own1[kC1 * k + c] = acc;
    } else {
      s.own2[kC2 * k + (c - kC1)] = acc;
    }
  }
}
constexpr int kUmom = 25;

template <int kT = 256, class FV = FusedView, bool kSecondOnly = false>
__device__ __forceinline__ void ownSums(const FV& fd, const FusedLds& s, float* umom, int U, int tid, const double* upD = nullptr, const double* usD = nullptr) {
  constexpr int NCH = kSecondOnly ? kC2Used : kC1 + kC2Used;
  for (int u = tid; u < U; u += kT) {
    const F3 p = kSecondOnly ? F3{float(upD[3 * u]), float(upD[3 * u + 1]), float(upD[3 * u + 2])} : F3{s.up[3 * u], s.up[3 * u + 1], s.up[3 * u + 2]};
    const bool point = u < fd.Kp;
    float* o = umom + kUmom * u;
    if (!kSecondOnly) {
      firstOrderMoments(o, p, s.uy[3 * u], s.uy[3 * u + 1], s.uy[3 * u + 2], point);
    }
    const float sg = kSecondOnly ? float(usD[u]) : s.us[u];
    const float s2 = sg * sg;
    float* o2 = kSecondOnly ? o : o + kC1;
#pragma unroll
    for (int c = 0; c < kC2Used; ++c) {
      o2[c] = 0.f;
    }
    const int q = point ? 4 : 10;
    o2[q + 0] = s2 * p.x * p.x;
    o2[q + 1] = s2 * p.x * p.y;
    o2[q + 2] = s2 * p.x * p.z;
    o2[q + 3] = s2 * p.y * p.y;
    o2[q + 4] = s2 * p.y * p.z;
    o2[q + 5] = s2 * p.z * p.z;
    if (point) {
      o2[0] = s2;
      o2[1] = s2 * p.x;
// ... 98 lines not shown
  }
  return o;
}
template <bool kJacobianRows>
__device__ __forceinline__ double paramRowsErrorD(const RigDev& rig, const ProblemDev& pb, int P, const double* th, int b, int tid) {
  double e = 0.0;
  if (pb.NL > 0 && pb.wLimit > 0.f) {
    const double tWeight = double(1e+1f * pb.wLimit);
    for (int l = tid; l < pb.NL; l += 256) {
      e += evalLimit<double>(rig, pb.limits[l], th, pb.enabledMask, tWeight).err;
    }
  }
  if (pb.hasModel && pb.wModel > 0.f) {
    const float* tp = pb.mpTarget + size_t(b) * P;
    const float* tw = pb.mpWeights + size_t(b) * P;
    double em = 0.0;
    for (int i = tid; i < P; i += 256) {
      if (pb.enabledMask[i] != 0) {
        const double w = double(tw[i]);
        if (!kJacobianRows || w > 0.0) {
          const double pd = w * (th[i] - double(tp[i]));
          em += pd * pd;
        }
      }
    }
    e += em * double(pb.wModel) * 1e-1;
  }
  return e;
}

template <int kT = 256, typename Gather, typename Store>
__device__ __forceinline__ void csrRowsPrefetched(const int32_t* outer, const int32_t* inner, const float* value, int R, int tid, Gather x, Store out) {
  for (int r0 = tid; r0 < R; r0 += 4 * kT) {
    int ka[4], kb[4], in0[4];
    float v0[4];
#pragma unroll
    for (int i = 0; i < 4; ++i) {
      const int r = min(r0 + kT * i, R - 1);
      ka[i] = outer[r], kb[i] = outer[r + 1];
    }
#pragma unroll
    for (int i = 0; i < 4; ++i) {
      const bool has = kb[i] > ka[i];
      in0[i] = has ? inner[ka[i]] : 0, v0[i] = has ? value[ka[i]] : 0.f;
    }
#pragma unroll
    for (int i = 0; i < 4; ++i) {
      const int r = r0 + kT * i;
      if (r < R) {
        decltype(x(0)) acc = 0;
        if (kb[i] > ka[i]) {
          acc += v0[i] * x(in0[i]);
          for (int k = ka[i] + 1; k < kb[i]; ++k) {
            acc += value[k] * x(inner[k]);
          }
        }
        out(r, acc);
      }
    }
  }
}

template <int kT = 256, typename Gather, typename Store>
__device__ __forceinline__ void csrRowsFromRecords(const int4* rec, int numRec, const int32_t* inner, const float* value, int R, int tid, Gather x, Store out) {
  for (int t = tid; t < numRec; t += kT) {
    const int4 q = rec[t];
    const int row = q.x & 0xffff, span = int(uint32_t(q.x) >> 16), in0 = q.y & 0xffff, cnt = int(uint32_t(q.y) >> 16);
    auto acc = __int_as_float(q.z) * x(in0);
    for (int k = q.w + 1; k < q.w + cnt; ++k) {
      acc += value[k] * x(inner[k]);
    }
    out(row, acc);
    for (int r = row + 1; r < row + span; ++r) {
      out(r, decltype(acc)(0));
    }
    if (t == 0) {
      for (int r = 0; r < row; ++r) {
        out(r, decltype(acc)(0));
      }
    }
  }
}

template <bool kGlobalTables = false, int kT = 256>
__device__ __forceinline__ void
blockFk(const RigView& rig, const FusedLds& s, const float* th, int tid, bool withAxes, long long* clk = nullptr, long long* clkLast = nullptr) {
  auto stamp = [&](int slot) {
    if (clk != nullptr && blockIdx.x == 0 && threadIdx.x == 0) {
      const long long now = clock64();
      clk[slot] += now - *clkLast;
      *clkLast = now;
    }
  };
  if (kGlobalTables && rig.rowRec != nullptr) {
    csrRowsFromRecords<kT>(
        rig.rowRec, rig.numRowRec, rig.ptInner, rig.ptValue, rig.R, tid, [&](int c) { return th[c]; }, [&](int r, float acc) { s.jd[r] = acc + (rig.hasOffsets ? rig.ptOffsets[r] : 0.f); });
  } else if (kGlobalTables) {
    csrRowsPrefetched<kT>(
        rig.ptOuter, rig.ptInner, rig.ptValue, rig.R, tid, [&](int c) { return th[c]; }, [&](int r, float acc) { s.jd[r] = acc + (rig.hasOffsets ? rig.ptOffsets[r] : 0.f); });
  } else {
    for (int r = tid; r < rig.R; r += kT) {
      const float off = rig.hasOffsets ? rig.ptOffsets[r] : 0.f;
      float acc = 0.f;
      const int k1 = rig.ptOuter[r + 1];
      for (int k = rig.ptOuter[r]; k < k1; ++k) {
        acc += rig.ptValue[k] * th[rig.ptInner[k]];
      }
      s.jd[r] = acc + off;
    }
  }
  float pre[4] = {0.f, 0.f, 0.f, 1.f}, off3[3] = {0.f, 0.f, 0.f};
  if (tid < rig.J) {
#pragma unroll
    for (int d = 0; d < 4; ++d) {
      pre[d] = rig.preRot[4 * tid + d];
    }
#pragma unroll
    for (int d = 0; d < 3; ++d) {
      off3[d] = rig.offset[3 * tid + d];
    }
  }
  __syncthreads();
  stamp(26);
  const int Jp = fkPad(rig.J);
  for (int j = tid; j < rig.J; j += kT) {
    float* slot = s.js + kJs * j;
    float loc[8];
    if (j == tid) {
      fkLocalFromParams(s.jd + 7 * j, pre, off3, loc, slot + 8);
    } else {
      fkLocalFromParams(s.jd + 7 * j, rig.preRot + 4 * j, rig.offset + 3 * j, loc, slot + 8);
    }
    if (rig.jumpRounds == 0) {
#pragma unroll
      for (int c = 0; c < 8; ++c) {
        slot[c] = loc[c];
      }
    } else {
      fkStoreLocalD(s.fkA, Jp, j, loc, rig.parent[j] + 1);
    }
  }
  __syncthreads();
  stamp(24);
  fkJumpRoundsD(s.js, s.fkA, s.fkB, rig.J, rig.jumpRounds, tid, kT);
  stamp(25);
  if (withAxes) {
    for (int j = tid; j < rig.J; j += kT) {
      fkAxesInPlaceP(rig, j, rig.parent[j], s.js);
    }
    __syncthreads();
  }
}

struct MixRowRec {
  int4 q{0, 0, 0, 0};
  bool has = false;
};
template <typename Gather, typename Store>
__device__ __forceinline__ void mixTransformRows(const RigView& rig, int tid, Gather x, Store out, const MixRowRec& regRec = MixRowRec{}) {
  if (regRec.has) {
    if (tid < rig.numRowRec) {
      const int4 q = regRec.q;
      const int row = q.x & 0xffff, span = int(uint32_t(q.x) >> 16), in0 = q.y & 0xffff, cnt = int(uint32_t(q.y) >> 16);
      auto acc = __int_as_float(q.z) * x(in0);
      for (int k = q.w + 1; k < q.w + cnt; ++k) {
        acc += rig.ptValue[k] * x(rig.ptInner[k]);
      }
      out(row, acc);
      for (int r = row + 1; r < row + span; ++r) {
        out(r, decltype(acc)(0));
      }
      if (tid == 0) {
        for (int r = 0; r < row; ++r) {
          out(r, decltype(acc)(0));
        }
      }
    }
  } else if (rig.rowRec != nullptr) {
    csrRowsFromRecords<256>(rig.rowRec, rig.numRowRec, rig.ptInner, rig.ptValue, rig.R, tid, x, out);
  } else {
    csrRowsPrefetched<256>(rig.ptOuter, rig.ptInner, rig.ptValue, rig.R, tid, x, out);
  }
}

__device__ __forceinline__ void blockFkD(const RigView& rig, const MixLds& m, const double* th, int tid, int myLevel, bool withAxes, const MixRowRec& regRec = MixRowRec{}) {
  mixTransformRows(
      rig, tid, [&](int c) { return th[c]; }, [&](int r, double acc) { m.X[r] = acc + (rig.hasOffsets ? double(rig.ptOffsets[r]) : 0.0); }, regRec);
  __syncthreads();
  double loc[8];
  const int j = tid;
  double* slot = m.js + kJsD * (j < rig.J ? j : 0);
  if (j < rig.J) {
    fkLocalFromParamsD(m.X + 7 * j, rig.preRot + 4 * j, rig.offset + 3 * j, loc, slot + 8);
    if (myLevel == 0) {
#pragma unroll
      for (int c = 0; c < 8; ++c) {
        slot[c] = loc[c];
      }
    }
  }
  __syncthreads();
  for (int lvl = 1; lvl < rig.numLevels; ++lvl) {
    if (j < rig.J && myLevel == lvl) {
      const double* w = m.js + kJsD * rig.parent[j];
      const DQ qp{w[3], w[4], w[5], w[6]};
      const D3 t = D3{w[0], w[1], w[2]} + dqrot(qp, w[7] * D3{loc[0], loc[1], loc[2]});
      const DQ q = dqmul(qp, DQ{loc[3], loc[4], loc[5], loc[6]});
      slot[0] = t.x, slot[1] = t.y, slot[2] = t.z, slot[3] = q.x, slot[4] = q.y, slot[5] = q.z, slot[6] = q.w, slot[7] = w[7] * loc[7];
    }
    __syncthreads();
  }
  if (withAxes) {
    if (j < rig.J) {
      fkAxesInPlaceD(rig.preRot + 4 * j, j, rig.parent[j], m.js);
    }
    __syncthreads();
  }
}

template <bool kStore>
__device__ __forceinline__ double mixUnits(const ProblemDev& pb, const FusedLds& s, const MixLds& m, int b, int U, int tid) {
  double e = 0.0;
  for (int u = tid; u < U; u += 256) {
    const UnitD un = evalUnitD(pb, loadUnitInput(pb, b, u), m.js, u);
    if (kStore) {
      m.up[3 * u] = un.v.x, m.up[3 * u + 1] = un.v.y, m.up[3 * u + 2] = un.v.z;
      m.uf[3 * u] = un.f.x, m.uf[3 * u + 1] = un.f.y, m.uf[3 * u + 2] = un.f.z;
      m.us[u] = un.sigma;
    }
    e += un.werr;
  }
// ... 118 lines not shown
      const int par = rig.parent[q];
      Tv = d[0] * transAxisColD(m.js, par, 0) + d[1] * transAxisColD(m.js, par, 1) + d[2] * transAxisColD(m.js, par, 2);
    }
    const D3 Om = d[3] * D3{ja[8], ja[9], ja[10]} + d[4] * D3{ja[11], ja[12], ja[13]} + d[5] * D3{ja[14], ja[15], ja[16]};
    const D3 C = Tv - dcross(Om, ta) - (kLn2D * d[6]) * ta;
    acc[0] = C.x, acc[1] = C.y, acc[2] = C.z, acc[3] = Om.x, acc[4] = Om.y, acc[5] = Om.z, acc[6] = d[6];
    target = parentPos[tid];
    double* o = m.Y + kTanD * tid;
#pragma unroll
    for (int c = 0; c < 7; ++c) {
      o[c] = acc[c];
    }
    reinterpret_cast<int*>(o + 7)[0] = target;
  }
  __syncthreads();
  for (int r = 0; r < rig.jumpRounds; ++r) {
    int next = -1;
    if (target >= 0) {
      const double* t = m.Y + kTanD * target;
#pragma unroll
      for (int c = 0; c < 7; ++c) {
        acc[c] += t[c];
      }
      next = reinterpret_cast<const int*>(t + 7)[0];
    }
    __syncthreads();
    if (target >= 0) {
      double* o = m.Y + kTanD * tid;
#pragma unroll
      for (int c = 0; c < 7; ++c) {
        o[c] = acc[c];
      }
      reinterpret_cast<int*>(o + 7)[0] = next;
    }
    target = next;
    __syncthreads();
  }
}

template <class FV>
__device__ __forceinline__ void mixApply(
    const RigView& rig, const FV& fd, const FusedLds& s, const MixLds& m, const int16_t* parentPos, int J, int NP, int n, int nsrc, double mu, const double* p, double* q, int tid, const MixRowRec& regRec = MixRowRec{}) {
  mixTangent(
      rig, fd, m, parentPos, J, tid,
      [&](int c) {
        const int cs = fd.colToSolve[c];
        return cs >= 0 ? p[cs] : 0.0;
      },
      regRec);
  mixAdjoint(
      fd, s, m, J, NP, n, nsrc, tid,
      [&](int u, int k, const D3& pu) {
        const double* pre = m.Y + kTanD * k;
        D3 v = dcross(D3{pre[3], pre[4], pre[5]}, pu);
        if (u < fd.Kp) {
          v = D3{pre[0], pre[1], pre[2]} + v + (kLn2D * pre[6]) * pu;
        }
        const double sg = m.us[u];
        return (sg * sg) * v;
      },
      q);
  for (int c = tid; c < n; c += 256) {
    q[c] += mu * p[c];
  }
  __syncthreads();
}

constexpr int kGenEv = 29;

template <int NB, bool kTR, bool kGen, int kRule>
struct FusedFour {
  static constexpr bool value = NB <= 6 && !kGen && !kTR;
};

struct FusedLayout {
  size_t uyFloats;
  size_t auxOff;
  size_t cellOff;
  size_t t9;
  size_t arenaFloats;
  size_t umomFloats;
  size_t regionFloats;
  size_t genFloats;
  size_t total;
};
__host__ __device__ inline FusedLayout fusedLayout(int NB, int J, int P, int U, int nsrc, int n, int numCells, bool cellsBehindRho, int GT, int genRows, bool separateUy = false, size_t csrFloats = 0, bool mix = false) {
  auto a4 = [](size_t x) { return (x + 3) & ~size_t(3); };
  auto h4 = [&](size_t x) { return a4((x + 1) / 2); };
  auto mx = [](size_t x, size_t y) { return x > y ? x : y; };
  const size_t T = size_t(NB) * (NB + 1) / 2, NP = 16 * size_t(NB);
  FusedLayout l;
  l.cellOff = cellsBehindRho ? 2 * NP : 0;
  const size_t aux = a4(mx(2 * NP, mx(size_t(nsrc), l.cellOff + size_t(numCells))));
  l.auxOff = separateUy ? a4(3 * size_t(U)) : 0;
  l.uyFloats = separateUy ? l.auxOff + aux : mx(a4(3 * size_t(U)), aux);
  l.t9 = a4(size_t(kTan) * J);
  l.arenaFloats = mx(size_t(kSrcCh - 1) * size_t(srcStrideFor(nsrc)), 2 * l.t9 + a4(P));
  if (mix) {
    l.arenaFloats = mx(size_t(kSrcCh - 1) * size_t(srcStrideFor(nsrc)), a4(2 * (mixXDoubles(J, nsrc) + mixYDoubles(J, P))));
  }
  l.umomFloats = mx(a4(size_t(kUmom) * U), a4(size_t(kC1) * J));
  const size_t scratch = fkBufFloats(J) + 2 * a4(size_t(kC2) * J) + l.umomFloats;
  l.regionFloats = mx(scratch, T * 256);
  const size_t rowsGp = a4(size_t(genRows));
  l.genFloats = GT > 0 ? a4(size_t(kGenEv) * GT) + 2 * a4(rowsGp) + a4(rowsGp * size_t(srcStrideFor(int(NP)))) : 0;
  const size_t meta = h4(NP + 1) + 3 * a4(nsrc) + a4(J) + 4 * h4(J) + h4(size_t(J) + 1) + 2 * h4(U) + h4(n) + h4(P);
  size_t fixed = a4(P) + a4(size_t(kJs) * J) + 2 * a4(3 * size_t(U)) + a4(U) + 2 * a4(NP) + l.uyFloats + 16 + 8;
  if (mix) {
    fixed = l.uyFloats + 40 + 8 + a4(2 * mixPersistentDoubles(J, P, U, int(NP))) + 2 * h4(J);
  }
  l.total = meta + fixed + l.genFloats + l.arenaFloats + l.regionFloats + csrFloats;
  return l;
}

__device__ __forceinline__ double generalRowsError(const ProblemDev& pb, const float* js, int b, int tid) {
  double e = 0.0;
  for (int g = tid; g < pb.G; g += 256) {
    const JointBlockDev k = jointBlockOf(pb, b, pb.genBlock[g]);
    e += double(evalJointConstraint(k, js, pb.genJoint[g], jointBlockSecondJoint(pb, k, g), size_t(b) * size_t(k.count) + size_t(g - k.first)).werr);
  }
  if (pb.wLimit > 0.f) {
    const float tWeightE = 1e+1f * pb.wLimit;
    for (int q = tid; q < pb.NE; q += 256) {
      e += double(evalEllipsoid(pb.ellipsoids[q], js, tWeightE).werr);
    }
  }
  return e;
}

__device__ __forceinline__ double generalRowsEvaluate(const ProblemDev& pb, const float* js, int b, int U, int tid, float* gEv, float* gRes) {
  double e = 0.0;
  int* evi = reinterpret_cast<int*>(gEv);
  for (int g = tid; g < pb.G; g += 256) {
    const JointBlockDev k = jointBlockOf(pb, b, pb.genBlock[g]);
    const int i = g - k.first;
    const JointEval o = evalJointConstraint(k, js, pb.genJoint[g], jointBlockSecondJoint(pb, k, g), size_t(b) * size_t(k.count) + size_t(i));
    const int row = k.rowStart + o.nrows * i - 3 * U;
    e += double(o.werr);
    for (int q = 0; q < o.nrows; ++q) {
      gRes[row + q] = o.sigma * o.f[q];
    }
    const float sg = fabsf(o.sigma) <= 1e-9f ? 0.f : o.sigma;
    float* w = gEv + kGenEv * g;
    w[0] = o.vp.x, w[1] = o.vp.y, w[2] = o.vp.z;
    w[3] = o.vn.x, w[4] = o.vn.y, w[5] = o.vn.z;
#pragma unroll
    for (int q = 0; q < 9; ++q) {
      w[6 + q] = sg * o.dp[q];
      w[15 + q] = sg * o.dn[q];
    }
    evi[kGenEv * g + 24] = pb.genTin[g];
    evi[kGenEv * g + 25] = row;
    evi[kGenEv * g + 26] = jointEvalFlags(o);
    evi[kGenEv * g + 27] = jointBlockSecondTin(pb, k, g);
  }
  const float tWeightE = 1e+1f * pb.wLimit;
  for (int q = tid; q < pb.NE; q += 256) {
    const EllipsoidDev ct = pb.ellipsoids[q];
    const int row = pb.rowsJoint - 3 * pb.NE + 3 * q - 3 * U, g = pb.G + q;
    EllipsoidEval o = evalEllipsoid(ct, js, tWeightE);
    if (!(pb.wLimit > 0.f)) {
      o.jwgt = o.werr = 0.f;
    }
    e += double(o.werr);
    gRes[row] = o.diff.x * o.jwgt, gRes[row + 1] = o.diff.y * o.jwgt, gRes[row + 2] = o.diff.z * o.jwgt;
    float* w = gEv + kGenEv * g;
    w[0] = o.position.x, w[1] = o.position.y, w[2] = o.position.z;
    w[3] = w[4] = w[5] = 0.f;
#pragma unroll
    for (int k = 0; k < 9; ++k) {
      w[6 + k] = (k == 0 || k == 4 || k == 8) ? o.jwgt : 0.f;
      w[15 + k] = 0.f;
    }
    evi[kGenEv * g + 24] = ct.tinParent;
    evi[kGenEv * g + 25] = row;
    evi[kGenEv * g + 26] = 3 | 16;
    evi[kGenEv * g + 27] = ct.tinStop;
  }
  return e;
}

struct GenSlot {
  int tin, tout, joint, dof, parent;
  float weight;
};
template <typename SlotFn, typename ExtrasFn>
__device__ __forceinline__ void generalRowsGather(const float* js, const float* gEv, float* gJ, int gst, int GT, int n, int tid, SlotFn slot, ExtrasFn extras) {
  const int* evi = reinterpret_cast<const int*>(gEv);
  for (int item = tid; item < GT * n; item += 256) {
    const int c = item / GT, g = item - c * GT;
    const float* w = gEv + kGenEv * g;
    const int tin = evi[kGenEv * g + 24], row = evi[kGenEv * g + 25], fl = evi[kGenEv * g + 26], tinStop = evi[kGenEv * g + 27];
    const bool hasPoint = (fl & 16) != 0, hasDir = (fl & 32) != 0;
    const F3 vp{w[0], w[1], w[2]}, vn{w[3], w[4], w[5]};
    float acc[3] = {0.f, 0.f, 0.f};
    auto addSlot = [&](int e) {
      const GenSlot sl = slot(e);
      if (!(sl.tin <= tin && tin < sl.tout)) {
        return;
      }
      if (tinStop >= 0 && sl.tin <= tinStop && tinStop < sl.tout) {
        return;
      }
      const float* a = js + kJs * sl.joint;
      F3 gp{0.f, 0.f, 0.f}, gn{0.f, 0.f, 0.f};
      if (sl.dof >= 3 && sl.dof < 6) {
        const float* ax = a + 8 + 3 * (sl.dof - 3);
        const F3 axis{ax[0], ax[1], ax[2]};
        if (hasPoint) {
          gp = cross(axis, vp - F3{a[0], a[1], a[2]});
        }
        if (hasDir) {
          gn = cross(axis, vn);
        }
      } else if (hasPoint) {
        gp = sl.dof < 3 ? transAxisCol(js, sl.parent, sl.dof) : kLn2 * (vp - F3{a[0], a[1], a[2]});
      }
#pragma unroll
      for (int q = 0; q < 3; ++q) {
        const float jc = (w[6 + 3 * q] * gp.x + w[7 + 3 * q] * gp.y + w[8 + 3 * q] * gp.z) +
            (w[15 + 3 * q] * gn.x + w[16 + 3 * q] * gn.y + w[17 + 3 * q] * gn.z);
        acc[q] += jc * sl.weight;
      }
    };
    auto addSlotPair = [&](int e) {
      const GenSlot sl = slot(e);
      const bool anc = sl.tin <= tin && tin < sl.tout, anc2 = sl.tin <= tinStop && tinStop < sl.tout;
      if (!anc && !anc2) {
        return;
      }
      const F3 gd = pairSourceDerivative(js, sl.joint, sl.dof, anc, anc2, vp, vn, [&]() { return transAxisCol(js, sl.parent, sl.dof); });
      acc[0] += (w[6] * gd.x + w[7] * gd.y + w[8] * gd.z) * sl.weight;
    };
    int e0, e1;
    extras(c, e0, e1);
    if ((fl & 64) != 0) {
      addSlotPair(c);
      for (int e = e0; e < e1; ++e) {
        addSlotPair(e);
      }
    } else {
      addSlot(c);
      for (int e = e0; e < e1; ++e) {
        addSlot(e);
      }
    }
    gJ[row * gst + c] = acc[0];
    if ((fl & 15) >= 2) {
      gJ[(row + 1) * gst + c] = acc[1];
    }
    if ((fl & 15) == 3) {
      gJ[(row + 2) * gst + c] = acc[2];
    }
  }
}

template <bool kGen = false, bool kStore = false, bool kGlobalCsr = true, class FV = FusedViewS>
__device__ __forceinline__ double blockError(
    const RigDev& rigDev,
    const RigView& rig,
    const ProblemDev& pb,
    const FV& fd,
    const FusedLds& s,
    const float* th,
    int b,
    int tid,
    double* unrounded = nullptr) {
  const int lane = tid & 63, wave = tid >> 6;
  blockFk<kGlobalCsr>(rig, s, th, tid, kStore);
  double e = 0.0;
  for (int u = tid; u < fd.U; u += 256) {
    const Unit un = evalUnit(pb, s.js, b, u);
    if (kStore) {
      s.up[3 * u] = un.v.x, s.up[3 * u + 1] = un.v.y, s.up[3 * u + 2] = un.v.z;
      const float rx = un.sigma * un.f.x, ry = un.sigma * un.f.y, rz = un.sigma * un.f.z;
      s.ur[3 * u] = rx, s.ur[3 * u + 1] = ry, s.ur[3 * u + 2] = rz;
      s.uy[3 * u] = un.sigma * rx, s.uy[3 * u + 1] = un.sigma * ry, s.uy[3 * u + 2] = un.sigma * rz;
      s.us[u] = un.sigma;
    }
    e += double(un.werr);
  }
  if (pb.M > pb.rowsJoint) {
    e += paramRowsError<false>(rigDev, pb, rig.P, th, b, tid);
  }
  if (kGen) {
    e += generalRowsError(pb, s.js, b, tid);
  }
  e = waveReduceSum(e);
  if (lane == 0) {
    s.red[wave] = e;
  }
  __syncthreads();
  const double tot = (s.red[0] + s.red[1]) + (s.red[2] + s.red[3]);
  __syncthreads();
  if (unrounded != nullptr) {
    *unrounded = tot;
  }
  return double(float(tot));
}

__device__ __forceinline__ float blockSumF(const FusedLds& s, float v, int tid) {
  v = waveReduceSumF(v);
  if ((tid & 63) == 0) {
    s.red[4 + (tid >> 6)] = double(v);
  }
  __syncthreads();
  const float tot = float((s.red[4] + s.red[5]) + (s.red[6] + s.red[7]));
  __syncthreads();
  return tot;
}

__device__ __forceinline__ float quadSum(float v) {
  v += __int_as_float(__builtin_amdgcn_update_dpp(0, __float_as_int(v), 0xB1, 0xF, 0xF, true));
  v += __int_as_float(__builtin_amdgcn_update_dpp(0, __float_as_int(v), 0x4E, 0xF, 0xF, true));
  return v;
}

template <int NB>
__device__ __forceinline__ void solveLLtLeft(const float* L, const float* invDiag, float* x, int tid) {
  if (tid < 64) {
    const int i = tid >> 2, g = tid & 3;
#pragma unroll
    for (int k = 0; k < NB; ++k) {
      float acc = 0.f;
#pragma unroll
      for (int j = 0; j < k; ++j) {
        acc = dot4(ldsRow4(L + 256 * tileIndex(k, j), i, g), *reinterpret_cast<const float4*>(x + 16 * j + 4 * g), acc);
      }
      acc = quadSum(acc);
      float* xk = x + 16 * k;
      const float rhs = xk[i] - acc;
      const float invd = invDiag[16 * k + i];
      const float* Dk = L + 256 * tileIndex(k, k);
      float p = 0.f;
#pragma unroll
      for (int t = 0; t < 4; ++t) {
        const int c = 4 * t + g;
        const float m = Dk[tileAddr(c, i)];
        const float rc = __shfl(rhs, 4 * c, 64);
        p += (c < i ? m : (c == i ? invd : 0.f)) * rc;
      }
      p = quadSum(p);
      if (g == 0) {
        xk[i] = p;
      }
      __builtin_amdgcn_fence(__ATOMIC_ACQ_REL, "wavefront");
    }
#pragma unroll
    for (int k = NB - 1; k >= 0; --k) {
      float acc = 0.f;
#pragma unroll
      for (int j = k + 1; j < NB; ++j) {
        const float* Tj = L + 256 * tileIndex(j, k);
#pragma unroll
        for (int t = 0; t < 4; ++t) {
// ... 311 lines not shown
  for (int k = tid; k < J; k += 256) {
    if (posUnitStart[k + 1] > posUnitStart[k]) {
      int rank = 0;
      for (int q = 0; q < k; ++q) {
        rank += posUnitStart[q + 1] > posUnitStart[q] ? 1 : 0;
      }
      loadedPos[rank] = I(k);
    }
  }
  int numLoaded = 0;
  for (int k = 0; k < J; ++k) {
    numLoaded += posUnitStart[k + 1] > posUnitStart[k] ? 1 : 0;
  }
  __syncthreads();
  return numLoaded;
}

struct FusedArgs {
  RigDev rig;
  ProblemDev pb;
  FusedDev fd;
  SolveStateDev st;
  FusedParams fp;
};
static __global__ void stashFusedArgsKernel(FusedArgs a, FusedArgs* dst) {
  *dst = a;
}
template <int NB, int MODE, bool kTR, bool kGen = false, int kRule = -1, bool kArgLazy = false, bool kMix = false>
__global__ void __launch_bounds__(256, (NB <= 6 && !kGen ? (FusedFour<NB, kTR, kGen, kRule>::value && !kMix ? 4 : 3) : (NB <= 8 ? 2 : 1))) fusedSolveKernel(
    const FusedArgs* __restrict__ argsDev,
    const RigDev rigArg,
    const ProblemDev pbArg,
    FusedDev fdV,
    float* __restrict__ theta,
    SolveStateDev stV,
    FusedParams fpV,
    float* __restrict__ dbgH,
    float* __restrict__ dbgG,
    long long* __restrict__ dbgClk,
    MixSelect sel) {
  static_assert(!kMix || (!kTR && !kGen && kRule == -1 && !kArgLazy), "the mixed-precision instantiation: generic rule, reference rows");
  constexpr int T = NB * (NB + 1) / 2;
  constexpr int NP = 16 * NB;
  constexpr bool kLook = NB <= 8;
  long long clkLast = 0;
  const int dbgStop = (MODE == 2 && dbgClk != nullptr) ? int(dbgClk[31]) : 0;
#define MMX_CLK(slot)                                             \
  if (MODE == 2 && blockIdx.x == 0 && threadIdx.x == 0) {         \
    const long long now_ = clock64();                             \
    dbgClk[slot] += now_ - clkLast;                               \
    clkLast = now_;                                               \
  }                                                               \
  if (MODE == 2 && dbgStop == (slot) + 1) {                       \
    __builtin_amdgcn_endpgm();                                    \
  }
  extern __shared__ __attribute__((aligned(16))) float smem[];
  int bSel = blockIdx.x;
  if (kMix && sel.map != nullptr) {
    if (int(blockIdx.x) >= *sel.count) {
      return;
    }
    bSel = sel.map[blockIdx.x];
  }
  const int b = bSel, tid = threadIdx.x;
  const int wave = tid >> 6, lane = tid & 63;
  RigDev rigV;
  ProblemDev pbV;
  if (!kArgLazy) {
    rigV = rigArg;
    pbV = pbArg;
    selectInstanceRig(rigV, b);
    selectInstanceWeights(pbV, b);
  }
  const RigDev& rig = kArgLazy ? argsDev->rig : rigV;
  const ProblemDev& pb = kArgLazy ? argsDev->pb : pbV;
  const FusedDev& fd = kArgLazy ? argsDev->fd : fdV;
  const SolveStateDev& st = kArgLazy ? argsDev->st : stV;
  const FusedParams& fp = kArgLazy ? argsDev->fp : fpV;
  const int J = rig.J, P = rig.P, U = fd.U, n = fd.n, nsrc = fd.nsrc;
  const int JL = rig.layoutJ;
  const int kR = rig.R;

  FusedLds s;
  int16_t *lParentPos, *lSubSize, *lPosUnitStart, *lPosUnits, *lUnitJoint, *lSolveList, *lDfsJoint, *lLoadedPos, *lColToSolve;
  int *lParent, *lPtOuter = nullptr, *lPtInner = nullptr;
  float *srcGu, *cells, *arena, *lPtValue = nullptr;
  constexpr bool kFour = FusedFour<NB, kTR, kGen, kRule>::value && !kMix;
  constexpr bool kCsrLds = !kFour && !kMix;
  constexpr bool kLeanSolve = kFour;
  constexpr bool kRide = kFour && NB >= 2;
  constexpr bool kLeanOps = kFour;
  constexpr bool kLeanAcc = kFour;
  const int kNnz = fd.nnz;
  const FusedLayout lay = fusedLayout(NB, JL, P, U, nsrc, n, fd.numCells, kRule < 0, kGen ? fd.GT : 0, kGen ? fd.genRows : 0, kTR, 0, kMix);
  MixLds m{};
  m.layoutJ = JL;
  {
    float* p = smem;
    auto take = [&](size_t count) {
      float* r = p;
      p += alignUp4(count);
      return r;
    };
    auto takeS = [&](size_t count) { return reinterpret_cast<int16_t*>(take((count + 1) / 2)); };
    s.mStart = takeS(NP + 1);
    s.mTin = reinterpret_cast<int*>(take(nsrc));
    s.mInfo = reinterpret_cast<int*>(take(nsrc));
    s.mW = take(nsrc);
    lParent = reinterpret_cast<int*>(take(JL));
    lParentPos = takeS(JL);
    lSubSize = takeS(JL);
    lPosUnitStart = takeS(JL + 1);
    lPosUnits = takeS(U);
    lUnitJoint = takeS(U);
    lSolveList = takeS(n);
    lDfsJoint = takeS(JL);
    lLoadedPos = takeS(JL);
    lColToSolve = takeS(P);
    if (kCsrLds) {
      lPtOuter = reinterpret_cast<int*>(take(kR + 1));
      lPtInner = reinterpret_cast<int*>(take(kNnz));
      lPtValue = take(kNnz);
    }
    if (kMix) {
      s.th = s.js = s.up = s.us = s.ur = s.g = s.d0 = nullptr;
      m.lo = takeS(JL);
      m.hi = takeS(JL);
    } else {
      s.th = take(P);
      s.js = take(size_t(kJs) * JL);
      s.up = take(3 * size_t(U));
      s.ur = take(3 * size_t(U));
      s.us = take(U);
      s.g = take(NP);
      s.d0 = take(NP);
    }
    s.uy = take(lay.uyFloats);
    s.rho = s.uy + lay.auxOff, s.invDiag = s.rho + NP, srcGu = s.rho, cells = s.rho + lay.cellOff;
    s.red = reinterpret_cast<double*>(take(kMix ? 40 : 16));
    s.flags = reinterpret_cast<int*>(take(8));
    s.gEv = s.gRes = s.gW = s.gJ = nullptr;
    if (kGen) {
      const int rowsGp = (fd.genRows + 3) & ~3;
      s.gEv = take(size_t(kGenEv) * size_t(fd.GT));
      s.gRes = take(rowsGp);
      s.gW = take(rowsGp);
      s.gJ = take(size_t(rowsGp) * size_t(srcStrideFor(NP)));
    }
    arena = take(lay.arenaFloats);
    if (kMix) {
      m.X = reinterpret_cast<double*>(arena);
      m.Y = m.X + mixXDoubles(JL, nsrc);
    }
    s.srcT = arena;
    s.tanOwn = arena, s.jd = arena + lay.t9, s.tanPre = arena + lay.t9, s.dfull = arena + 2 * lay.t9;
    float* region = p;
    s.fkA = reinterpret_cast<double*>(take(fkBufFloats(JL)));
    s.fkB = reinterpret_cast<double*>(p);
    s.own2 = take(size_t(kC2) * JL);
    s.sub2 = take(size_t(kC2) * JL);
    s.umom = take(lay.umomFloats);
    s.own1 = region, s.sub1 = s.umom;
    s.L = region;
    if (kMix) {
      double* d = reinterpret_cast<double*>(smem + (lay.total - alignUp4(2 * mixPersistentDoubles(JL, P, U, NP))));
      m.th = d, d += P;
      m.js = d, d += size_t(kJsD) * JL;
      m.up = d, d += 3 * size_t(U);
      m.uf = d, d += 3 * size_t(U);
      m.us = d, d += U;
      m.g = d, d += NP;
      m.x = d, d += NP;
      m.r = d, d += NP;
      m.p = d, d += NP;
      m.q = d;
    }
  }

  float* thg = theta + size_t(b) * P;
  if (kMix) {
    const float* th0 = sel.thetaInit != nullptr ? sel.thetaInit + size_t(b) * P : thg;
    for (int i = tid; i < P; i += 256) {
      m.th[i] = double(th0[i]);
    }
  } else {
    for (int i = tid; i < P; i += 256) {
      s.th[i] = thg[i];
    }
  }
  for (int c = tid; c <= NP; c += 256) {
    s.mStart[c] = int16_t(fd.srcStart[c]);
  }
  for (int e = tid; e < nsrc; e += 256) {
    const ColumnSourceDev cs = fd.srcs[e];
    s.mTin[e] = cs.tin | (cs.tout << 16);
    s.mInfo[e] = cs.joint | (cs.dof << 12) | ((cs.parent + 1) << 16);
    s.mW[e] = cs.weight;
  }
  for (int i = tid; i < J; i += 256) {
    lParent[i] = rig.parent[i];
    lSubSize[i] = int16_t(fd.subSize[i]);
  }
  for (int i = tid; i <= J; i += 256) {
    lPosUnitStart[i] = int16_t(fd.posUnitStart[i]);
  }
  if (kCsrLds) {
    for (int i = tid; i <= kR; i += 256) {
      lPtOuter[i] = rig.ptOuter[i];
    }
    for (int i = tid; i < kNnz; i += 256) {
      lPtInner[i] = rig.ptInner[i];
      lPtValue[i] = rig.ptValue[i];
    }
  }
  for (int i = tid; i < U; i += 256) {
    lPosUnits[i] = int16_t(fd.posUnits[i]);
    lUnitJoint[i] = int16_t(pb.unitTin[i]);
  }
  for (int i = tid; i < n; i += 256) {
    lSolveList[i] = int16_t(fd.solveList[i]);
  }
  for (int i = tid; i < J; i += 256) {
    lDfsJoint[i] = int16_t(fd.dfsJoint[i]);
    lLoadedPos[i] = int16_t(i < fd.numLoaded ? fd.loadedPos[i] : 0);
  }
  for (int i = tid; i < P; i += 256) {
    lColToSolve[i] = -1;
  }
  if (kGen) {
    const int rowsGp = (fd.genRows + 3) & ~3;
    for (int i = tid; i < rowsGp * srcStrideFor(NP); i += 256) {
      s.gJ[i] = 0.f;
    }
    for (int i = tid; i < rowsGp; i += 256) {
      s.gRes[i] = 0.f;
      s.gW[i] = 0.f;
    }
  }
  __syncthreads();
  for (int i = tid; i < n; i += 256) {
    lColToSolve[fd.solveList[i]] = int16_t(i);
  }
  int numLoadedInst = fd.numLoaded;
  if (pb.instPosParent != nullptr || pb.instOriParent != nullptr) {
    __syncthreads();
    numLoadedInst = buildInstanceUnitTables(pb, fd, b, J, U, tid, lUnitJoint, lPosUnitStart, lPosUnits, lLoadedPos);
  }
  {
    int* posOf = reinterpret_cast<int*>(s.fkA);
    for (int k = tid; k < J; k += 256) {
      posOf[fd.dfsJoint[k]] = k;
    }
    __syncthreads();
    for (int k = tid; k < J; k += 256) {
      const int par = rig.parent[fd.dfsJoint[k]];
      lParentPos[k] = int16_t(par >= 0 ? posOf[par] : -1);
    }
  }
  RigView rv;
  rv.J = J, rv.P = P, rv.R = kR, rv.numLevels = rig.numLevels, rv.jumpRounds = rig.jumpRounds;
  rv.parent = lParent, rv.preRot = asGlobal(rig.preRot), rv.offset = asGlobal(rig.offset);
  rv.ptOuter = kCsrLds ? lPtOuter : asGlobal(rig.ptOuter), rv.ptInner = kCsrLds ? lPtInner : asGlobal(rig.ptInner), rv.ptValue = kCsrLds ? lPtValue : asGlobal(rig.ptValue);
  rv.ptOffsets = asGlobal(rig.ptOffsets);
  rv.hasOffsets = rig.ptOffsetsNonZero != 0;
  rv.levelOrder = nullptr, rv.levelStart = nullptr;
  rv.rowRec = asGlobal(rig.ptRowRec), rv.numRowRec = rig.numRowRec;
  FusedViewS fv;
  fv.U = U, fv.Kp = fd.Kp;
  fv.dfsJoint = lDfsJoint, fv.loadedPos = lLoadedPos, fv.numLoaded = numLoadedInst, fv.colToSolve = lColToSolve;
  fv.subSize = lSubSize, fv.unitPos = lUnitJoint, fv.posUnitStart = lPosUnitStart, fv.posUnits = lPosUnits;
  fv.solveList = lSolveList;
  float* estAcc = reinterpret_cast<float*>(s.flags + 4);
  if (tid == 0) {
    s.flags[0] = 0;
    s.flags[1] = 0;
    s.flags[2] = 0;
    estAcc[0] = estAcc[1] = 0.f, estAcc[2] = -1.f;
  }
  int4 mixRec{0, 0, 0, 0};
  const bool mixHasRec = kMix && rv.rowRec != nullptr && rv.numRowRec <= 256;
  if (mixHasRec && tid < rv.numRowRec) {
    mixRec = rv.rowRec[tid];
  }
  const MixRowRec mixRecP{mixRec, mixHasRec};
  int mixLevel = 0;
  if (kMix && tid < J) {
    for (int a = lParent[tid]; a >= 0; a = lParent[a]) {
      ++mixLevel;
    }
  }
  if (kMix) {
    for (int k = tid; k < J; k += 256) {
      const int end = k + lSubSize[k];
      int lo = 0, hi = 0;
      for (int li = 0; li < numLoadedInst; ++li) {
        const int pp = lLoadedPos[li];
        lo += pp < k ? 1 : 0;
        hi += pp < end ? 1 : 0;
      }
      m.lo[k] = int16_t(lo), m.hi[k] = int16_t(hi);
    }
  }
  const bool hasParamRows = kRule >= 0 ? false : (pb.M > pb.rowsJoint);
  double lastError = DBL_MAX;
  float lambda = fp.lambda;
  double lambdaD = double(fp.lambda);
  bool mixUnconverged = false;
  int mixApplied = 0;
  float trRadius = fp.trustRadius;
  double curError = DBL_MAX;
  int itersDone = 0;
  float pivotWorst = 0.f;
  float refineWorst = 0.f;
  constexpr bool kReuse = !kGen && !kTR && kRule != 0;
  const int stepRule = kRule < 0 ? fp.stepRule : (kRule == 1 ? 1 : 0);
  const int doLineSearch = kRule < 0 || kRule == 2 ? fp.doLineSearch : 0;
  bool stateValid = false;
  double stateError = 0.0;
  __syncthreads();

  if (MODE == 2) {
    clkLast = clock64();
  }
  const int tidOuter = tid;
  for (int it = 0; it < fp.maxIterations; ++it) {
    int tid = tidOuter;
    asm volatile("" : "+v"(tid));
    const int lane = tid & 63;
    const int wave = __builtin_amdgcn_readfirstlane(tid >> 6);
    constexpr bool kLateUnit = kFour || kMix;
    const UnitInput uin0 = kLateUnit ? UnitInput{} : loadUnitInput(pb, b, tid < U ? tid : U);
    float trLambda = 1e-10f;
    int trustStep = 0;
    bool trNoStep = false;
    float trDn2 = 0.f, trDg = 0.f, trMu = 0.f;
    bool notPd = false;
    bool badPivot = false;
    bool floored = false;
    for (;;) {
    int tidT = tid;
    if (kTR) {
      asm volatile("" : "+v"(tidT));
    }
    {
    const int tid = tidT;
    const int lane = tid & 63;
    const int wave = __builtin_amdgcn_readfirstlane(tid >> 6);
    if (kReuse && stateValid) {
      curError = stateError;
    } else if (kMix) {
      blockFkD(rv, m, m.th, tid, mixLevel, true, mixRecP);
      double e = mixUnits<true>(pb, s, m, b, U, tid);
      if (hasParamRows) {
        e += paramRowsErrorD<true>(rig, pb, P, m.th, b, tid);
      }
      e = waveReduceSum(e);
      if (lane == 0) {
        s.red[wave] = e;
      }
      __syncthreads();
      curError = (s.red[0] + s.red[1]) + (s.red[2] + s.red[3]);
      MMX_CLK(1)
    } else {
    blockFk<!kCsrLds>(rv, s, s.th, tid, true, MODE == 2 ? dbgClk : nullptr, &clkLast);
    MMX_CLK(1)
    {
      double e = 0.0;
      for (int u = tid; u < U; u += 256) {
        const Unit un = evalUnitFrom(pb, (!kLateUnit && u == tid) ? uin0 : loadUnitInput(pb, b, u), s.js, u);
        s.up[3 * u] = un.v.x, s.up[3 * u + 1] = un.v.y, s.up[3 * u + 2] = un.v.z;
        const float rx = un.sigma * un.f.x, ry = un.sigma * un.f.y, rz = un.sigma * un.f.z;
        s.ur[3 * u] = rx, s.ur[3 * u + 1] = ry, s.ur[3 * u + 2] = rz;
        s.uy[3 * u] = un.sigma * rx, s.uy[3 * u + 1] = un.sigma * ry, s.uy[3 * u + 2] = un.sigma * rz;
        s.us[u] = un.sigma;
        e += double(un.werr);
      }
      if (hasParamRows) {
        e += paramRowsError<true>(rig, pb, P, s.th, b, tid);
      }
      if (kGen) {
        e += generalRowsEvaluate(pb, s.js, b, U, tid, s.gEv, s.gRes);
      }
      e = waveReduceSum(e);
      if (lane == 0) {
        s.red[wave] = e;
      }
    }
    __syncthreads();
    curError = (s.red[0] + s.red[1]) + (s.red[2] + s.red[3]);
    }
    if (kGen) {
      generalRowsGather(
          s.js, s.gEv, s.gJ, srcStrideFor(NP), fd.GT, n, tid,
          [&](int e) {
            const int span = s.mTin[e], info = s.mInfo[e];
            return GenSlot{span & 0xffff, span >> 16, info & 0xfff, (info >> 12) & 7, (info >> 16) - 1, s.mW[e]};
          },
          [&](int c, int& e0, int& e1) { e0 = NP + s.mStart[c], e1 = NP + s.mStart[c + 1]; });
      __syncthreads();
    }
    MMX_CLK(2)
    if (kMix) {
      __syncthreads();
      mixAdjoint(
          fv, s, m, J, NP, n, nsrc, tid,
          [&](int u, int, const D3&) {
            const double sg = m.us[u];
            return (sg * sg) * D3{m.uf[3 * u], m.uf[3 * u + 1], m.uf[3 * u + 2]};
          },
          m.g);
      __syncthreads();
      MMX_CLK(5)
    }
    int newtonIter = 0, pdRetries = 0;
    for (;;) {
    int tidS = tid;
    if (kTR) {
      asm volatile("" : "+v"(tidS));
    }
    {
    const int tid = tidS;
    const int lane = tid & 63;
    const int wave = __builtin_amdgcn_readfirstlane(tid >> 6);
    const float mu = kTR ? 1e-20f + (trLambda - 1e-10f) : lambda;
    if (kMix) {
      ownSums<256, FusedViewS, true>(fv, s, s.umom, U, tid, m.up, m.us);
    } else {
      ownSums(fv, s, s.umom, U, tid);
    }
    __syncthreads();
    MMX_CLK(15)
    constexpr int kUnD = kFusedTreeUn;
    if (!kMix) {
      treeSum<kC1, true, kC1, kUnD>(fv, s.own1, s.sub1, J, wave, lane);
    }
    treeSum<kC2Used, true, kC2, kUnD>(fv, s.own2, s.sub2, J, wave, lane);
    __syncthreads();
    MMX_CLK(3)
    const int sst = srcStrideFor(nsrc);
    float* srcD = s.srcT;
    float* srcA = s.srcT + 7 * sst;
    float* srcG = srcGu;
    for (int e = tid; e < nsrc; e += 256) {
      ColumnSourceDev cs;
      {
        const int info = s.mInfo[e];
        cs.joint = info & 0xfff;
        cs.dof = (info >> 12) & 7;
        cs.parent = (info >> 16) - 1;
        cs.tin = s.mTin[e] & 0xffff;
      }
      float jaMix[kJs];
// ... 490 lines not shown
        }
        const double alpha = rz / pq;
        double sums[5] = {0.0, 0.0, 0.0, 0.0, 0.0};
        for (int c = tid; c < NP; c += 256) {
          float rc = 0.f;
          if (c < n) {
            const double dx = alpha * m.p[c], xn = m.x[c] + dx, rn = m.r[c] - alpha * m.q[c];
            m.x[c] = xn, m.r[c] = rn;
            sums[0] += dx * dx, sums[1] += xn * xn;
            rc = float(rn);
          }
          s.rho[c] = rc;
        }
        __syncthreads();
        MMX_CLK(19)
        solveLLt<NB, false>(s.L, s.invDiag, s.rho, tid);
        MMX_CLK(20)
        for (int c = tid; c < n; c += 256) {
          const double z = double(s.rho[c]);
          sums[2] += m.r[c] * z, sums[3] += z * m.q[c], sums[4] += z * z;
        }
#pragma unroll
        for (int q = 0; q < 5; ++q) {
          sums[q] = waveReduceSum(sums[q]);
        }
        if (lane == 0) {
#pragma unroll
          for (int q = 0; q < 5; ++q) {
            s.red[4 * q + wave] = sums[q];
          }
        }
        __syncthreads();
#pragma unroll
        for (int q = 0; q < 5; ++q) {
          sums[q] = (s.red[4 * q] + s.red[4 * q + 1]) + (s.red[4 * q + 2] + s.red[4 * q + 3]);
        }
        __syncthreads();
        const double am2 = alpha > 1.0 ? alpha * alpha : 1.0;
        if (am2 * sums[4] * am2 * sums[4] <= tol2 * sums[1] * sums[0]) {
          for (int c = tid; c < n; c += 256) {
            m.x[c] += double(s.rho[c]);
          }
          converged = true;
        } else {
          const double beta = -alpha * sums[3] / rz;
          for (int c = tid; c < n; c += 256) {
            m.p[c] = double(s.rho[c]) + beta * m.p[c];
          }
          rz = sums[2];
          converged = !(rz > 0.0);
          if (k >= 5 && am2 * sums[4] > 1e-6 * sums[1]) {
            __syncthreads();
            break;
          }
        }
        __syncthreads();
        MMX_CLK(18)
      }
      mixUnconverged = mixUnconverged || !converged;
    } else if (kRide) {
      solveLLtAheadTail<NB>(s.L, s.invDiag, s.d0, tid);
    } else if (!notPd) {
      solveLLt<NB, kLeanSolve>(s.L, s.invDiag, s.d0, tid);
    }
    MMX_CLK(8)
    const int nRefine = (!notPd && !kMix) ? fp.refine : 0;
    float prevCorr2 = FLT_MAX;
    for (int rf = 0; rf < nRefine; ++rf) {
      {
        auto xd = [&](int c) {
          const int cs = fv.colToSolve[c];
          return cs >= 0 ? s.d0[cs] : 0.f;
        };
        auto od = [&](int r, float a) { s.jd[r] = a; };
        if (kCsrLds) {
          for (int r = tid; r < rv.R; r += 256) {
            float a = 0.f;
            const int k1 = rv.ptOuter[r + 1];
            for (int k = rv.ptOuter[r]; k < k1; ++k) {
              a += rv.ptValue[k] * xd(rv.ptInner[k]);
            }
            od(r, a);
          }
        } else if (rv.rowRec != nullptr) {
          csrRowsFromRecords<256>(rv.rowRec, rv.numRowRec, rv.ptInner, rv.ptValue, rv.R, tid, xd, od);
        } else {
          csrRowsPrefetched<256>(rv.ptOuter, rv.ptInner, rv.ptValue, rv.R, tid, xd, od);
        }
      }
      __syncthreads();
      MMX_CLK(16)
      if (kGen) {
        const int gst = srcStrideFor(NP);
        for (int r = tid; r < fd.genRows; r += 256) {
          float a = s.gRes[r];
          for (int c = 0; c < n; ++c) {
            a -= s.gJ[r * gst + c] * s.d0[c];
          }
          s.gW[r] = a;
        }
      }
      for (int k = tid; k < J; k += 256) {
        const int q = fv.dfsJoint[k];
        const float* ja = s.js + kJs * q;
        const float* d = s.jd + 7 * q;
        const F3 ta{ja[0], ja[1], ja[2]};
        F3 Tv{0.f, 0.f, 0.f};
        if (d[0] != 0.f || d[1] != 0.f || d[2] != 0.f) {
          const int par = rv.parent[q];
          Tv = d[0] * transAxisCol(s.js, par, 0) + d[1] * transAxisCol(s.js, par, 1) + d[2] * transAxisCol(s.js, par, 2);
        }
        const F3 Om = d[3] * F3{ja[8], ja[9], ja[10]} + d[4] * F3{ja[11], ja[12], ja[13]} + d[5] * F3{ja[14], ja[15], ja[16]};
        const F3 C = Tv - cross(Om, ta) - (kLn2 * d[6]) * ta;
        float* o = s.tanOwn + kTan * k;
        o[0] = C.x, o[1] = C.y, o[2] = C.z, o[3] = Om.x, o[4] = Om.y, o[5] = Om.z, o[6] = d[6], o[7] = 0.f;
      }
      __syncthreads();
      if (JL <= 256) {
        float acc[7];
        int target = -1;
        if (tid < J) {
#pragma unroll
          for (int c = 0; c < 7; ++c) {
            acc[c] = s.tanOwn[kTan * tid + c];
          }
          target = lParentPos[tid];
          s.tanPre[kTan * tid + 7] = __int_as_float(target);
#pragma unroll
          for (int c = 0; c < 7; ++c) {
            s.tanPre[kTan * tid + c] = acc[c];
          }
        }
        __syncthreads();
        for (int r = 0; r < rv.jumpRounds; ++r) {
          int next = -1;
          if (target >= 0) {
            const float* t = s.tanPre + kTan * target;
#pragma unroll
            for (int c = 0; c < 7; ++c) {
              acc[c] += t[c];
            }
            next = __float_as_int(t[7]);
          }
          __syncthreads();
          if (target >= 0) {
            float* o = s.tanPre + kTan * tid;
#pragma unroll
            for (int c = 0; c < 7; ++c) {
              o[c] = acc[c];
            }
            o[7] = __int_as_float(next);
          }
          target = next;
          __syncthreads();
        }
      } else {
        treeSum<7, false, kTan>(fv, s.tanOwn, s.tanPre, J, wave, lane);
        __syncthreads();
      }
      const bool unitPath = U <= JL;
      float* refOwn = unitPath ? arena + lay.t9 : arena;
      float* refSub = unitPath ? arena : arena + lay.t9;
      FusedLds sr = s;
      sr.own1 = refOwn;
      if (unitPath) {
        for (int u = tid; u < U; u += 256) {
// ... 172 lines not shown
          part += m.x[c] * m.g[c] + lambdaD * m.x[c] * m.x[c];
        }
        const double predicted = blockSumD(s.red, part, tid);
        for (int i = tid; i < P; i += 256) {
          m.Y[i] = m.th[i];
        }
        __syncthreads();
        for (int c = tid; c < n; c += 256) {
          m.Y[fv.solveList[c]] -= m.x[c];
        }
        __syncthreads();
        double eFull = 0.0;
        const double eNew = blockErrorD<true>(rv, pb, s, m, m.Y, b, U, tid, mixLevel, &eFull, mixRecP, &rig, hasParamRows);
        const double rho = predicted > 0.0 ? (curError - eNew) / predicted : -1.0;
        if (st.stepHistory != nullptr && tid == 0) {
          double* sh = st.stepHistory + (size_t(b) * fp.maxIterations + it) * 2;
          sh[0] = lambdaD;
          sh[1] = rho;
        }
        stateValid = false;
        if (rho > 0.0) {
          for (int i = tid; i < P; i += 256) {
            m.th[i] = m.Y[i];
          }
          stateValid = !hasParamRows;
          stateError = eFull;
        }
        if (!(rho >= 0.25)) {
          lambdaD = fmin(lambdaD * double(fp.lmUp), double(fp.lmLambdaMax));
        } else if (rho > 0.75) {
          lambdaD = fmax(lambdaD * double(fp.lmDown), double(fp.lmLambdaMin));
        }
        lambda = float(lambdaD);
      } else if (doLineSearch) {
        const double scaledError = 1e-3 * curError;
        double gd = 0.0;
        if (doLineSearch == 2) {
          double part = 0.0;
          for (int c = tid; c < n; c += 256) {
            part += m.g[c] * m.x[c];
          }
          gd = blockSumD(s.red, part, tid);
        }
        float scale = 1.f;
        for (int ls = 0; ls < 10; ++ls) {
          for (int i = tid; i < P; i += 256) {
            m.Y[i] = m.th[i];
          }
          __syncthreads();
          for (int c = tid; c < n; c += 256) {
            m.Y[fv.solveList[c]] -= double(scale) * m.x[c];
          }
          __syncthreads();
          const double eNew = blockErrorD<true>(rv, pb, s, m, m.Y, b, U, tid, mixLevel, &stateError, mixRecP, &rig, hasParamRows);
          if ((curError - eNew) >= (doLineSearch == 2 ? double(1e-4f * scale) * gd : double(scale) * scaledError)) {
            break;
          }
          scale *= 0.5f;
        }
        for (int i = tid; i < P; i += 256) {
          m.th[i] = m.Y[i];
        }
        stateValid = !hasParamRows;
      } else {
        for (int c = tid; c < n; c += 256) {
          m.th[fv.solveList[c]] -= m.x[c];
        }
        stateValid = false;
      }
      break;
    }
    if (kTR) {
      if (trNoStep) {
        break;
      }
      for (int i = tid; i < P; i += 256) {
        s.dfull[i] = s.th[i];
      }
      __syncthreads();
      for (int c = tid; c < n; c += 256) {
        s.dfull[fv.solveList[c]] -= s.d0[c];
      }
      __syncthreads();
      const double eNew = blockError<kGen, false, !kCsrLds>(rig, rv, pb, fv, s, s.dfull, b, tid);
      const float predicted = trDg + (trMu - 1e-20f) * trDn2;
      const float rho = float((curError - eNew) / double(predicted));
      if (rho < 0.25f) {
        trRadius = 0.25f * trRadius;
      } else if (rho > 0.75f) {
        trRadius = fminf(2.f * trRadius, 10.f);
      }
      if (rho > 0.f) {
        for (int i = tid; i < P; i += 256) {
          s.th[i] = s.dfull[i];
        }
        break;
      }
      if (++trustStep >= 10) {
        break;
      }
      __syncthreads();
      continue;
    }
    if (!notPd && stepRule == 1) {
      float part = 0.f;
      for (int c = tid; c < n; c += 256) {
        part += s.d0[c] * s.g[c] + lambda * s.d0[c] * s.d0[c];
      }
      const float predicted = blockSumF(s, part, tid);
      for (int i = tid; i < P; i += 256) {
        s.dfull[i] = s.th[i];
      }
      __syncthreads();
      for (int c = tid; c < n; c += 256) {
        s.dfull[fv.solveList[c]] -= s.d0[c];
      }
      __syncthreads();
      double eFull = 0.0;
      const double eNew = blockError<kGen, kReuse, !kCsrLds>(rig, rv, pb, fv, s, s.dfull, b, tid, &eFull);
      const float rho = predicted > 0.f ? float((curError - eNew) / double(predicted)) : -1.f;
      if (st.stepHistory != nullptr && tid == 0) {
        double* sh = st.stepHistory + (size_t(b) * fp.maxIterations + it) * 2;
        sh[0] = double(lambda);
        sh[1] = double(rho);
      }
      stateValid = false;
      if (rho > 0.f) {
        for (int i = tid; i < P; i += 256) {
          s.th[i] = s.dfull[i];
        }
        stateValid = kReuse && !hasParamRows;
        stateError = eFull;
      }
      if (!(rho >= 0.25f)) {
        lambda = fminf(lambda * fp.lmUp, fp.lmLambdaMax);
      } else if (rho > 0.75f) {
        lambda = fmaxf(lambda * fp.lmDown, fp.lmLambdaMin);
      }
    } else if (notPd && stepRule == 1) {
      if (st.stepHistory != nullptr && tid == 0) {
        double* sh = st.stepHistory + (size_t(b) * fp.maxIterations + it) * 2;
        sh[0] = double(lambda);
        sh[1] = -1.0;
      }
      lambda = fminf(lambda * fp.lmUp, fp.lmLambdaMax);
    } else if (!notPd && doLineSearch) {
      const float scaledError = 1e-3f * float(curError);
      double gd = 0.0;
      if (doLineSearch == 2) {
        float part = 0.f;
        for (int c = tid; c < n; c += 256) {
          part += s.g[c] * s.d0[c];
        }
        gd = double(blockSumF(s, part, tid));
      }
      float scale = 1.f;
      for (int ls = 0; ls < 10; ++ls) {
        for (int i = tid; i < P; i += 256) {
          s.dfull[i] = s.th[i];
        }
        __syncthreads();
        for (int c = tid; c < n; c += 256) {
          s.dfull[fv.solveList[c]] -= scale * s.d0[c];
        }
        __syncthreads();
        const double eNew = blockError<kGen, kReuse, !kCsrLds>(rig, rv, pb, fv, s, s.dfull, b, tid, &stateError);
        if ((curError - eNew) >= (doLineSearch == 2 ? double(1e-4f * scale) * gd : double(scale * scaledError))) {
          break;
        }
        scale *= 0.5f;
      }
      for (int i = tid; i < P; i += 256) {
        s.th[i] = s.dfull[i];
      }
      stateValid = kReuse && !hasParamRows;
    } else if (!notPd) {
      for (int c = tid; c < n; c += 256) {
        s.th[fv.solveList[c]] -= s.d0[c];
      }
      stateValid = false;
    }
    break;
    }
    }
    if (st.paramHistory != nullptr) {
      float* ph = st.paramHistory + (size_t(b) * fp.maxIterations + it) * size_t(P);
      for (int i = tid; i < P; i += 256) {
        ph[i] = kMix ? float(m.th[i]) : s.th[i];
      }
    }
    if (wave == 0) {
      float w = pivotWorst;
      w = fmaxf(w, dppMoveF<0xB1>(w));
      w = fmaxf(w, dppMoveF<0x4E>(w));
      w = fmaxf(w, dppMoveF<0x141>(w));
      w = fmaxf(w, dppMoveF<0x140>(w));
      pivotWorst = 0.f;
      if (lane == 0) {
        float e0 = estAcc[2];
        if (e0 < 0.f) {
          e0 = estAcc[2] = float(curError);
        }
        estAcc[0] = fmaxf(estAcc[0], w);
        estAcc[1] = fmaxf(estAcc[1], w * (e0 > 0.f ? sqrtf(float(curError) / e0) : 1.f));
      }
    }
    if (tid == 0) {
      const double e = curError;
      if (st.errorHistory != nullptr) {
        st.errorHistory[size_t(b) * fp.maxIterations + it] = e;
      }
      itersDone = it + 1;
      if (badPivot && !kMix) {
        s.flags[2] |= 2;
      }
      if (floored) {
        s.flags[2] |= 4;
      }

      const bool converged = fabs(lastError - e) / (fabs(e) + double(FLT_MIN)) <= double(fp.threshold) * double(FLT_EPSILON);
      s.flags[0] = (it >= fp.minIterations && converged) ? 1 : 0;
      lastError = e;
      if (!kMix && !kTR && fp.autoAbort != 0 && st.precisionBound > 0.f) {
        const float estNow = kPrecisionGain * FLT_EPSILON * estAcc[1] / kPivotFloorOrOne;
        if (!(estNow <= st.precisionBound)) {
          s.flags[0] = 2;
        }
      }
    }
    __syncthreads();
    MMX_CLK(10)
    if (s.flags[0] != 0) {
      break;
    }
  }

  int bad = 0;
  for (int i = tid; i < P; i += 256) {
    if (!isfinite(kMix ? float(m.th[i]) : s.th[i])) {
      bad = 1;
    }
  }
  bad = __syncthreads_or(bad);
  const bool aborted = !kMix && !kTR && s.flags[0] == 2;
  float th2 = 0.f;
  if (!bad && !aborted) {
    for (int i = tid; i < P; i += 256) {
      const float v = kMix ? float(m.th[i]) : s.th[i];
      thg[i] = v;
// ... 824 lines not shown
    }
  }
  __syncthreads();
  treeSumT<kC1, true, kC1, 8>(fv.subSize, fv.loadedPos, fv.numLoaded, s.own1, s.sub1, J, wave, kWaves, lane, t.kRange);
  __syncthreads();
  for (int c = tid; c < NP; c += kT) {
    float a = 0.f;
    if (c < n) {
      auto slotShare = [&](int e) {
        const ColumnSourceDev cs = fd.srcs[e];
        return cs.weight * sourceGradient(cs.joint, cs.dof, cs.parent, s.js, s.sub1 + kC1 * cs.tin);
      };
      a = slotShare(c);
      const int e1 = fd.slotBase + fd.srcStart[c + 1];
      for (int e = fd.slotBase + fd.srcStart[c]; e < e1; ++e) {
        a += slotShare(e);
      }
      if (pb.M > pb.rowsJoint) {
        a += paramRowsColumn(rig, pb, fd, t.th, s.d0, t.col, P, b, c, fd.solveList[c]).g;
      }
      if (hasGen) {
        for (int r = 0; r < fd.genRows; ++r) {
          a += t.gJ[r * gst + c] * t.gRes[r];
        }
      }
      a -= lambda * s.d0[c];
    }
    rhoVec[size_t(b) * NP + c] = a;
  }
}

size_t treeStateFloats(int J, int U) {
  return treeStateLayout(J, U).total;
}
size_t treeRefineLdsBytes(int J, int P, int U, int n, int genRows) {
  return treeRefineLdsFloats(J, P, U, n, nullptr, nullptr, genRows) * sizeof(float);
}

hipError_t launchTreeRefine(
    const RigDev& rig,
    const ProblemDev& pb,
    const FusedDev& fd,
    const float* theta,
    const float* state,
    const float* genState,
    const float* dvec,
    float* rhoVec,
    const int32_t* refState,
    float lambda,
    const float* lambdaPer,
    hipStream_t stream) {
  const size_t lds = treeRefineLdsBytes(rig.layoutJ, rig.P, fd.U, fd.n, fd.genRows);
  if (lds > 160 * 1024 - 64) {
    return hipErrorInvalidValue;
  }
  const bool extra = pb.M > pb.rowsJoint || fd.GT > 0 || pb.instPosParent != nullptr || pb.instOriParent != nullptr;
  if (!extra) {
    constexpr int kRefWaves = 8;
    static LdsLimitCache ldsLimitWide;
    hipError_t rc = ldsLimitWide.ensure(reinterpret_cast<const void*>(treeRefineKernel<kRefWaves>), lds);
    if (rc != hipSuccess) {
      return rc;
    }
    hipLaunchKernelGGL((treeRefineKernel<kRefWaves>), dim3(pb.B), dim3(64 * kRefWaves), lds, stream, rig, pb, fd, theta, state, genState, dvec, rhoVec, refState, lambda, lambdaPer);
    return hipGetLastError();
  }
  static LdsLimitCache ldsLimit;
  {
    hipError_t rc = ldsLimit.ensure(reinterpret_cast<const void*>(treeRefineKernel<4>), lds);
    if (rc != hipSuccess) {
      return rc;
    }
  }
  hipLaunchKernelGGL(treeRefineKernel<4>, dim3(pb.B), dim3(256), lds, stream, rig, pb, fd, theta, state, genState, dvec, rhoVec, refState, lambda, lambdaPer);
  return hipGetLastError();
}
#endif

#if !defined(MMX_FUSED_GROUP) || MMX_FUSED_GROUP == 0
size_t fusedCsrFloats(int J, int nnz) {
  auto a4 = [](size_t x) { return (x + 3) & ~size_t(3); };
  return a4(7 * size_t(J) + 1) + 2 * a4(nnz);
}
size_t fusedLdsBytes(int NB, int J, int P, int U, int nsrc, int n, int numCells, bool cellsBehindRho, int GT, int genRows, bool separateUy, size_t csrFloats, bool mix) {
  return fusedLayout(NB, J, P, U, nsrc, n, numCells, cellsBehindRho, GT, genRows, separateUy, csrFloats, mix).total * sizeof(float);
}
#endif

template <int NB, int MODE, bool kTR, bool kGen = false, int kRule = -1>
static hipError_t launchFusedMode(
    const RigDev& rig,
    const ProblemDev& pb,
    const FusedDev& fd,
    float* theta,
    const SolveStateDev& st,
    const FusedParams& fp,
    float* dbgH,
    float* dbgG,
    long long* dbgClk,
    void* argsBuf,
    hipStream_t stream) {
  constexpr bool kFourL = FusedFour<NB, kTR, kGen, kRule>::value;
  const size_t lds = fusedLdsBytes(NB, rig.layoutJ, rig.P, fd.U, fd.nsrc, fd.n, fd.numCells, kRule < 0, kGen ? fd.GT : 0, kGen ? fd.genRows : 0, kTR, kFourL ? 0 : fusedCsrFloats(rig.layoutJ, fd.nnz));
  if (lds > 160 * 1024) {
    return hipErrorInvalidValue;
  }
  constexpr bool kLazyBuilt = kFourL && MODE == 0;
  const bool lazy = kLazyBuilt && argsBuf != nullptr && rig.instPreRot == nullptr && rig.instOffset == nullptr && pb.fnWeights == nullptr;
  if (lazy) {
    static LdsLimitCache ldsLimit;
    hipError_t rc = ldsLimit.ensure(reinterpret_cast<const void*>(fusedSolveKernel<NB, MODE, kTR, kGen, kRule, kLazyBuilt>), lds);
    if (rc != hipSuccess) {
      return rc;
    }
    FusedArgs* dst = static_cast<FusedArgs*>(argsBuf);
    hipLaunchKernelGGL(stashFusedArgsKernel, dim3(1), dim3(1), 0, stream, FusedArgs{rig, pb, fd, st, fp}, dst);
    hipLaunchKernelGGL((fusedSolveKernel<NB, MODE, kTR, kGen, kRule, kLazyBuilt>), dim3(pb.B), dim3(256), lds, stream, dst, RigDev{}, ProblemDev{}, FusedDev{}, theta, SolveStateDev{}, FusedParams{}, dbgH, dbgG, dbgClk, MixSelect{});
  } else {
    static LdsLimitCache ldsLimit;
    hipError_t rc = ldsLimit.ensure(reinterpret_cast<const void*>(fusedSolveKernel<NB, MODE, kTR, kGen, kRule, false>), lds);
    if (rc != hipSuccess) {
      return rc;
    }
    hipLaunchKernelGGL((fusedSolveKernel<NB, MODE, kTR, kGen, kRule, false>), dim3(pb.B), dim3(256), lds, stream, static_cast<const FusedArgs*>(nullptr), rig, pb, fd, theta, st, fp, dbgH, dbgG, dbgClk, MixSelect{});
  }
  return hipGetLastError();
}

template <int NB>
static hipError_t launchFusedNB(
    const RigDev& rig,
    const ProblemDev& pb,
    const FusedDev& fd,
    float* theta,
    const SolveStateDev& st,
    const FusedParams& fp,
    float* dbgH,
    float* dbgG,
    long long* dbgClk,
    void* argsBuf,
    hipStream_t stream) {
  if (fd.GT > 0) {
    if (fp.stepRule == 2) {
      return hipErrorInvalidValue;
    }
    if (dbgH != nullptr || dbgG != nullptr) {
      return launchFusedMode<NB, 1, false, true>(rig, pb, fd, theta, st, fp, dbgH, dbgG, nullptr, argsBuf, stream);
    }
    return launchFusedMode<NB, 0, false, true>(rig, pb, fd, theta, st, fp, nullptr, nullptr, nullptr, argsBuf, stream);
  }
  if (fp.stepRule == 2) {
    return launchFusedMode<NB, 0, true>(rig, pb, fd, theta, st, fp, nullptr, nullptr, nullptr, argsBuf, stream);
  }
  if (dbgClk != nullptr) {
    return launchFusedMode<NB, 2, false>(rig, pb, fd, theta, st, fp, dbgH, dbgG, dbgClk, argsBuf, stream);
  }
  if (dbgH != nullptr || dbgG != nullptr) {
    return launchFusedMode<NB, 1, false>(rig, pb, fd, theta, st, fp, dbgH, dbgG, dbgClk, argsBuf, stream);
  }
  if (pb.M == pb.rowsJoint) {
    if (fp.stepRule == 0 && fp.doLineSearch == 0) {
      return launchFusedMode<NB, 0, false, false, 0>(rig, pb, fd, theta, st, fp, nullptr, nullptr, nullptr, argsBuf, stream);
    }
    if (fp.stepRule == 1) {
      return launchFusedMode<NB, 0, false, false, 1>(rig, pb, fd, theta, st, fp, nullptr, nullptr, nullptr, argsBuf, stream);
    }
  }
  return launchFusedMode<NB, 0, false>(rig, pb, fd, theta, st, fp, dbgH, dbgG, dbgClk, argsBuf, stream);
}

template <int NB>
static hipError_t launchFusedMixedNB(const RigDev& rig, const ProblemDev& pb, const FusedDev& fd, float* theta, const SolveStateDev& st, const FusedParams& fp, const MixSelect& sel, int blocks, long long* dbgClk, hipStream_t stream) {
  const size_t lds = fusedLdsBytes(NB, rig.layoutJ, rig.P, fd.U, fd.nsrc, fd.n, fd.numCells, true, 0, 0, false, 0, true);
  if (lds > 160 * 1024) {
    return hipErrorInvalidValue;
  }
  if (NB == 6 && dbgClk != nullptr) {
    static LdsLimitCache ldsLimitClk;
    hipError_t rc = ldsLimitClk.ensure(reinterpret_cast<const void*>(fusedSolveKernel<NB == 6 ? 6 : 1, 2, false, false, -1, false, true>), lds);
    if (rc != hipSuccess) {
      return rc;
    }
    hipLaunchKernelGGL((fusedSolveKernel<NB == 6 ? 6 : 1, 2, false, false, -1, false, true>), dim3(blocks), dim3(256), lds, stream, static_cast<const FusedArgs*>(nullptr), rig, pb, fd, theta, st, fp, nullptr, nullptr, dbgClk, sel);
    return hipGetLastError();
  }
  static LdsLimitCache ldsLimit;
  hipError_t rc = ldsLimit.ensure(reinterpret_cast<const void*>(fusedSolveKernel<NB, 0, false, false, -1, false, true>), lds);
  if (rc != hipSuccess) {
    return rc;
  }
  hipLaunchKernelGGL((fusedSolveKernel<NB, 0, false, false, -1, false, true>), dim3(blocks), dim3(256), lds, stream, static_cast<const FusedArgs*>(nullptr), rig, pb, fd, theta, st, fp, nullptr, nullptr, nullptr, sel);
  return hipGetLastError();
}

#ifndef MMX_FUSED_GROUP
#define MMX_FUSED_GROUP 0
#endif

#define MMX_FUSED_ARGS \
  const RigDev &rig, const ProblemDev &pb, const FusedDev &fd, float *theta, const SolveStateDev &st, const FusedParams &fp, \
      float *dbgH, float *dbgG, long long *dbgClk, void *argsBuf, hipStream_t stream
#define MMX_FUSED_PASS rig, pb, fd, theta, st, fp, dbgH, dbgG, dbgClk, argsBuf, stream

hipError_t launchFusedGroup0(int nb, MMX_FUSED_ARGS);
hipError_t launchFusedGroup1(int nb, MMX_FUSED_ARGS);
hipError_t launchFusedGroup2(int nb, MMX_FUSED_ARGS);
hipError_t launchFusedGroup3(int nb, MMX_FUSED_ARGS);
#define MMX_MIXED_ARGS \
  const RigDev &rig, const ProblemDev &pb, const FusedDev &fd, float *theta, const SolveStateDev &st, const FusedParams &fp, const MixSelect &sel, int blocks, long long *dbgClk, hipStream_t stream
hipError_t launchFusedMixedGroup5(int nb, MMX_MIXED_ARGS);
hipError_t launchFusedMixedGroup6(int nb, MMX_MIXED_ARGS);
#define MMX_MIXED_CASE(NB_) \
  case NB_:                 \
    return launchFusedMixedNB<NB_>(rig, pb, fd, theta, st, fp, sel, blocks, dbgClk, stream);

#define MMX_CASE(NB_) \
  case NB_:           \
    return launchFusedNB<NB_>(MMX_FUSED_PASS);

#if MMX_FUSED_GROUP == 0
hipError_t launchFusedGroup0(int nb, MMX_FUSED_ARGS) {
  switch (nb) {
    MMX_CASE(1) MMX_CASE(2) MMX_CASE(3) default : return hipErrorInvalidValue;
  }
}
#elif MMX_FUSED_GROUP == 1
hipError_t launchFusedGroup1(int nb, MMX_FUSED_ARGS) {
  switch (nb) {
    MMX_CASE(4) MMX_CASE(5) MMX_CASE(6) default : return hipErrorInvalidValue;
  }
}
#elif MMX_FUSED_GROUP == 2
hipError_t launchFusedGroup2(int nb, MMX_FUSED_ARGS) {
  switch (nb) {
    MMX_CASE(7) MMX_CASE(8) MMX_CASE(10) default : return hipErrorInvalidValue;
  }
}
#elif MMX_FUSED_GROUP == 9
#ifndef MMX_PROBE_RULE
#define MMX_PROBE_RULE 0
#endif
template __global__ void fusedSolveKernel<6, 0, false, false, MMX_PROBE_RULE, true>(
    const FusedArgs*, RigDev, ProblemDev, FusedDev, float*, SolveStateDev, FusedParams, float*, float*, long long*, MixSelect);
#elif MMX_FUSED_GROUP == 8
template __global__ void fusedSolveKernel<6, 0, false, false, -1, false, true>(
    const FusedArgs*, RigDev, ProblemDev, FusedDev, float*, SolveStateDev, FusedParams, float*, float*, long long*, MixSelect);
#elif MMX_FUSED_GROUP == 3
hipError_t launchFusedGroup3(int nb, MMX_FUSED_ARGS) {
  switch (nb) {
    MMX_CASE(12) MMX_CASE(14) default : return hipErrorInvalidValue;
  }
}
#elif MMX_FUSED_GROUP == 5
hipError_t launchFusedMixedGroup5(int nb, MMX_MIXED_ARGS) {
  switch (nb) {
    MMX_MIXED_CASE(1) MMX_MIXED_CASE(2) MMX_MIXED_CASE(3) MMX_MIXED_CASE(4) default : return hipErrorInvalidValue;
  }
}
#elif MMX_FUSED_GROUP == 6
hipError_t launchFusedMixedGroup6(int nb, MMX_MIXED_ARGS) {
  switch (nb) {
    MMX_MIXED_CASE(5) MMX_MIXED_CASE(6) MMX_MIXED_CASE(7) MMX_MIXED_CASE(8) default : return hipErrorInvalidValue;
  }
}
#endif
#undef MMX_CASE
#undef MMX_MIXED_CASE

#if MMX_FUSED_GROUP == 0
int fusedBlocksFor(int n) {
  const int nb = (n + 15) / 16;
  const int avail[] = {1, 2, 3, 4, 5, 6, 7, 8, 10, 12, 14};
  for (int a : avail) {
    if (nb <= a) {
      return a;
    }
  }
  return -1;
}

size_t fusedArgsBytes() {
  return sizeof(FusedArgs);
}

bool fusedMixedUsable(int J, int P, int U, int nsrc, int n, int numCells) {
// ... 31 lines not shown
```

momentum_amd/csrc/mmx_kernels.hpp:

```cpp
#pragma once

#include <atomic>

#include <hip/hip_runtime.h>

#include <cstddef>
#include <cstdint>

#include "mmx_device.hpp"

namespace mmx {

struct SolveStateDev {
  int32_t* done;
  int32_t* iterations;
  int32_t* status;
  double* lastError;
  double* finalError;
  double* errorHistory;
  float* paramHistory;
  double* stepHistory;
  float* diag;
  float precisionBound;
};
// ... 28 lines not shown
    }
    return hipSuccess;
  }
};

struct TrustStateDev {
  float* lambda;
  float* radius;
  int32_t* phase;
  int32_t* newton;
  int32_t* step;
  int32_t* mask;
  int32_t* active;
};

struct StepParams {
  float lambda;
  float threshold;
  int32_t iteration;
  int32_t minIterations;
  int32_t maxIterations;
  int32_t refine;
  float* delta;
  int32_t* stepIter;
  float* lambdaPer;
  double* stepHistory;
  float* diagErr0;
  float* diagAcc;
  TrustStateDev tr;
  int32_t doLineSearch;
  int32_t stepRule;
  float lmLambdaMin, lmLambdaMax, lmUp, lmDown;
  long long* clk;
  const uint32_t* tileMasks;
  int32_t numTiles;
};

struct FusedDev {
  int32_t U, Kp, n, nsrc, nnz;
  int32_t slotBase;
  const int32_t* subSize;
  const int32_t* dfsJoint;
  const int32_t* loadedPos;
  int32_t numLoaded;
  const int32_t* unitJoint;
  const int32_t* posUnitStart;
  const int32_t* posUnits;
  const int32_t* solveList;
  const int32_t* srcStart;
  const ColumnSourceDev* srcs;
  const uint4* gTerms;
  int32_t termRounds;
  const uint4* gTerms16;
  int32_t termRounds16;
  const int32_t* comb;
  int32_t numComb;
  int32_t numCells;
  int32_t numLimits;
  const int32_t* limStart;
  const int32_t* limOf;
  int32_t numPairDests;
  const int32_t* pairDest;
  const int32_t* pairCols;
  const int32_t* pairStart;
  const int32_t* pairLim;
  int32_t GT, genRows;
  const int32_t* tileList;
  int32_t numTiles;
};

struct FusedParams {
  float lambda;
  float threshold;
  int32_t minIterations;
  int32_t maxIterations;
  int32_t refine;
  int32_t doLineSearch;
  int32_t stepRule;
  float lmLambdaMin, lmLambdaMax, lmUp, lmDown;
  float trustRadius;
  float mixTol;
  int32_t mixMaxCg;
  int32_t autoAbort;
};

struct MixSelect {
  const int32_t* map;
  const int32_t* count;
  const float* thetaInit;
};

size_t fusedLdsBytes(int NB, int J, int P, int U, int nsrc, int n, int numCells, bool cellsBehindRho, int GT = 0, int genRows = 0, bool separateUy = false, size_t csrFloats = 0, bool mix = false);
size_t fusedCsrFloats(int J, int nnz);
size_t treeNormalEquationsLdsBytes(int J, int P, int U, int nsrc, int n, int GT = 0, int genRows = 0);
size_t treeRefineLdsBytes(int J, int P, int U, int n, int genRows);
size_t treeGenStateFloats(int n, int genRows);
hipError_t launchTreeNormalEquations(
    const RigDev& rig,
    const ProblemDev& pb,
    const FusedDev& fd,
    const float* theta,
    float* jtj,
    float* jtr,
    const int32_t* done,
    double* errOut,
    float* state,
    long long* clk,
    float* genState,
    bool tileMajor,
    hipStream_t stream);
size_t treeStateFloats(int J, int U);
hipError_t launchTreeRefine(
    const RigDev& rig,
    const ProblemDev& pb,
    const FusedDev& fd,
    const float* theta,
    const float* state,
    const float* genState,
    const float* dvec,
    float* rhoVec,
    const int32_t* refState,
    float lambda,
    const float* lambdaPer,
    hipStream_t stream);
int fusedBlocksFor(int n);
hipError_t launchFusedSolve(
    const RigDev& rig,
    const ProblemDev& pb,
    const FusedDev& fd,
    float* theta,
    const SolveStateDev& st,
    const FusedParams& fp,
    float* dbgH,
    float* dbgG,
    long long* dbgClk,
    void* argsBuf,
    hipStream_t stream);
size_t fusedArgsBytes();
bool fusedMixedUsable(int J, int P, int U, int nsrc, int n, int numCells);
hipError_t launchFusedMixed(
    const RigDev& rig, const ProblemDev& pb, const FusedDev& fd, float* theta, const SolveStateDev& st, const FusedParams& fp, const MixSelect& sel, int blocks, long long* dbgClk, hipStream_t stream);

size_t waveLdsBytes(int J, int P, int U, int n, bool frames = false);
hipError_t launchWaveSolve(const RigDev& rig, const ProblemDev& pb, const FusedDev& fd, float* theta, const SolveStateDev& st, const FusedParams& fp, hipStream_t stream);
hipError_t launchWaveFrames(const RigDev& rig, const ProblemDev& pb, const FusedDev& fd, float* theta, const SolveStateDev& st, const FusedParams& fp, int numFrames, hipStream_t stream);

size_t solveF64LdsBytes(int J, int P, int U, int n, int G = 0, int genRows = 0);
bool solveF64IsResident(int J, int P, int U, int n, int G = 0, int genRows = 0);
int solveF64ResidentChunkRows(int J, int P, int U, int n, int G = 0, int genRows = 0);
struct F64AssemblyList {
  const uint2* groups;
  const int32_t* extra;
  const int32_t* chunkStart;
  int32_t unitsPerChunk;
};
hipError_t launchSolveF64(
    const RigDev& rig,
    const ProblemDev& pb,
    const int32_t* solveList,
    int n,
    double* theta,
    const SolveStateDev& st,
    const FusedParams& fp,
    double* Jg,
    double* Hg,
    double* Hg2,
    hipStream_t stream,
    const F64AssemblyList& list = F64AssemblyList{nullptr, nullptr, nullptr, 0},
    const F64Select& select = F64Select{nullptr, nullptr, nullptr, nullptr});
hipError_t launchSelectSuspect(const int32_t* status, int B, int32_t mask, int32_t* map, int32_t* count, hipStream_t stream, int32_t require = 0);

size_t fkJacobianLdsBytes(int J, int P, int U);
int fkJacobianWavesPerInstance(const RigDev& rig, const ProblemDev& pb, bool withJacobian);
hipError_t launchStorePattern(float* jac, int B, int M, int P, int waves, hipStream_t stream, hipEvent_t startEvent, hipEvent_t stopEvent);
hipError_t launchTransposeJacobian(const float* colMajor, float* rowMajor, int B, int M, int P, hipStream_t stream);
constexpr int kMaxSolved = 2048;
size_t normalEquationsLdsBytes(int n);
size_t choleskyStepLdsBytes(int n, int M);

hipError_t launchFkJacobian(
    const RigDev& rig,
    const ProblemDev& pb,
    const float* theta,
    float* jac,
    float* res,
    double* err,
    float* state,
    const int32_t* done,
    hipStream_t stream,
    hipEvent_t startEvent = nullptr,
    hipEvent_t stopEvent = nullptr,
    bool accurateFk = false);

hipError_t launchNormalEquations(
    const ProblemDev& pb,
    int P,
    const float* jac,
    const float* res,
    float* jtj,
    float* jtr,
    const int32_t* done,
    bool lowerOnly,
    hipStream_t stream);

hipError_t launchCholeskyStep(
    const ProblemDev& pb,
    int P,
    const float* jac,
    const float* res,
    const float* jtj,
    const float* jtr,
    const double* errIter,
    float* theta,
    const SolveStateDev& st,
    const StepParams& sp,
    float* factor,
    hipStream_t stream);
hipError_t launchCholeskyFactorTiled(
    const ProblemDev& pb,
    int P,
// ... 48 lines not shown
```

Before: 2.234 million solves/s.

## Stage parameter-transform records, unit inputs and joint tables in LDS for fused solve

Adds an optional resident-table mode to the fused GN kernel. The parameter-transform row records, per-unit constraint inputs and joint constants/offsets are copied into LDS once per block and read from there on every iteration instead of from global memory. A chooser enables each table only if the larger LDS footprint still fits the same occupancy class budget, so waves per CU are not meant to drop. The cost is added LDS staging, more code paths, and a new tuning field and ABI entry point.

Result: slower. 2.211 million solves/s (-1.0%).

```diff
diff --git a/include/mmx.h b/include/mmx.h
--- a/include/mmx.h
+++ b/include/mmx.h
@@ -212,11 +212,16 @@
   float mixed_tolerance;
   int32_t mixed_max_cg;
   int32_t joint_pruning;
-  int32_t reserved[3];
+  int32_t resident_tables;
+  int32_t reserved[2];
 } mmx_tuning;
+#define MMX_RESIDENT_ROWS 1
+#define MMX_RESIDENT_UNITS 2
+#define MMX_RESIDENT_JOINTS 4
 int32_t mmx_problem_set_tuning(mmx_problem* problem, const mmx_tuning* tuning);
 int32_t mmx_problem_last_route(const mmx_problem* problem);
 int32_t mmx_problem_num_solve_joints(const mmx_problem* problem);
+int32_t mmx_problem_resident_tables(const mmx_problem* problem);
 
 int32_t mmx_problem_num_rows(const mmx_problem* problem);
 int32_t mmx_problem_batch(const mmx_problem* problem);
@@ -392,6 +397,7 @@
 int32_t mmx_host_elimination_order(const mmx_rig_desc* desc, const uint8_t* enabled, int32_t* order, int32_t* num_enabled);
 int32_t mmx_host_tile_structure(int32_t n, const uint8_t* related, uint32_t* row_mask, uint32_t* col_mask, int64_t* products);
 int32_t mmx_host_live_joints(const mmx_rig_desc* desc, int32_t n, const int32_t* joints, uint8_t* live, int32_t* compact_of, int32_t* num_live);
+int32_t mmx_host_fused_lds_bytes(const int32_t shape[12], int32_t resident_mask, int32_t offsets, int64_t* bytes, int32_t* chosen_mask);
 int32_t mmx_problem_tile_structure(mmx_problem* problem, uint32_t* row_mask, uint32_t* col_mask, int32_t* num_blocks, int32_t* num_tiles, int64_t* products);
 int32_t mmx_host_tile_level_schedule(int32_t n, const uint8_t* related, int32_t* steps);
 int32_t mmx_host_f64_assembly_list(
diff --git a/momentum_amd/_abi.py b/momentum_amd/_abi.py
--- a/momentum_amd/_abi.py
+++ b/momentum_amd/_abi.py
@@ -325,7 +325,7 @@
 
 class Tuning(C.Structure):
 
-    _fields_ = [("route", C.c_int32), ("max_refinement_steps", C.c_int32), ("mixed_tolerance", C.c_float), ("mixed_max_cg", C.c_int32), ("joint_pruning", C.c_int32), ("reserved", C.c_int32 * 3)]
+    _fields_ = [("route", C.c_int32), ("max_refinement_steps", C.c_int32), ("mixed_tolerance", C.c_float), ("mixed_max_cg", C.c_int32), ("joint_pruning", C.c_int32), ("resident_tables", C.c_int32), ("reserved", C.c_int32 * 2)]
 
 
 def as_ptr(a: np.ndarray, ctype):
diff --git a/momentum_amd/capi.py b/momentum_amd/capi.py
--- a/momentum_amd/capi.py
+++ b/momentum_amd/capi.py
@@ -18,12 +18,12 @@
     "mmx_gn_options_default", "mmx_abi_version", "mmx_last_error", "mmx_device_count",
     "mmx_rig_create", "mmx_rig_destroy", "mmx_rig_num_joints", "mmx_rig_num_params",
     "mmx_problem_create", "mmx_problem_destroy", "mmx_problem_num_rows", "mmx_problem_batch",
-    "mmx_problem_set_tuning", "mmx_problem_last_route", "mmx_problem_num_solve_joints",
+    "mmx_problem_set_tuning", "mmx_problem_last_route", "mmx_problem_num_solve_joints", "mmx_problem_resident_tables",
     "mmx_problem_set_enabled", "mmx_problem_set_constraints", "mmx_problem_set_constraints_sized", "mmx_problem_set_instance_rig", "mmx_problem_set_instance_parents", "mmx_eval_jacobian", "mmx_eval_jacobian_timed", "mmx_debug_store_pattern",
     "mmx_eval_skeleton_state", "mmx_eval_normal_equations", "mmx_solve", "mmx_solve_with_history", "mmx_solve_with_step_history", "mmx_problem_solve_diagnostics", "mmx_solve_f64", "mmx_solve_f64_host", "mmx_solve_host",
     "mmx_solve_frames", "mmx_solve_frames_host",
     "mmx_eval_jacobian_host", "mmx_eval_skeleton_state_host", "mmx_host_tables", "mmx_debug_fused_normal_equations", "mmx_debug_tree_normal_equations",
-    "mmx_host_elimination_order", "mmx_host_tile_structure", "mmx_host_tile_level_schedule", "mmx_host_f64_assembly_list", "mmx_problem_tile_structure", "mmx_host_live_joints",
+    "mmx_host_elimination_order", "mmx_host_tile_structure", "mmx_host_tile_level_schedule", "mmx_host_f64_assembly_list", "mmx_problem_tile_structure", "mmx_host_live_joints", "mmx_host_fused_lds_bytes",
     "mmx_comm_unique_id", "mmx_comm_create", "mmx_comm_create_all", "mmx_comm_world_size", "mmx_comm_rank",
     "mmx_comm_all_reduce_norms", "mmx_comm_all_reduce_norms_host", "mmx_residual_norms", "mmx_comm_destroy",
 ]
@@ -65,6 +65,7 @@
     L.mmx_problem_set_tuning.argtypes = [vp, C.POINTER(_abi.Tuning)]
     L.mmx_problem_last_route.argtypes = [vp]
     L.mmx_problem_num_solve_joints.argtypes = [vp]
+    L.mmx_problem_resident_tables.argtypes = [vp]
     L.mmx_problem_set_constraints.argtypes = [vp, C.POINTER(ConstraintData), vp]
     L.mmx_problem_set_constraints_sized.argtypes = [vp, C.POINTER(ConstraintData), C.c_size_t, vp]
     L.mmx_problem_set_instance_rig.argtypes = [vp, vp, vp, i32, vp]
@@ -107,6 +108,7 @@
     L.mmx_host_tile_level_schedule.argtypes = [i32, _abi.c_uint8_p, C.POINTER(C.c_int32)]
     L.mmx_problem_tile_structure.argtypes = [vp, u32p, u32p, _abi.c_int32_p, _abi.c_int32_p, i64p]
     L.mmx_host_live_joints.argtypes = [C.POINTER(RigDesc), i32, _abi.c_int32_p, _abi.c_uint8_p, _abi.c_int32_p, _abi.c_int32_p]
+    L.mmx_host_fused_lds_bytes.argtypes = [_abi.c_int32_p, i32, i32, i64p, _abi.c_int32_p]
     _lib = L
     return L
 
@@ -153,6 +155,17 @@
     jptr = as_ptr(jl, C.c_int32) if jl.size else _abi.c_int32_p()
     _check(lib().mmx_host_live_joints(C.byref(d), C.c_int32(jl.size), jptr, as_ptr(live, C.c_uint8), as_ptr(compact, C.c_int32), C.byref(n)))
     return dict(live=live, compact_of=compact, num_live=int(n.value))
+
+
+RESIDENT_ROWS, RESIDENT_UNITS, RESIDENT_JOINTS = 1, 2, 4
+
+
+def host_fused_lds_bytes(blocks: int, size_joints: int, path_joints: int, params: int, units: int, sources: int, solved: int, cells: int,
+                         generic_rule: bool, row_records: int, entries: int, num_pos: int, resident_mask: int = 0, offsets: bool = False):
+    shape = np.array([blocks, size_joints, path_joints, params, units, sources, solved, cells, int(generic_rule), row_records, entries, num_pos], np.int32)
+    nbytes, chosen = C.c_int64(0), C.c_int32(0)
+    _check(lib().mmx_host_fused_lds_bytes(as_ptr(shape, C.c_int32), C.c_int32(resident_mask), C.c_int32(int(offsets)), C.byref(nbytes), C.byref(chosen)))
+    return int(nbytes.value), int(chosen.value)
 
 
 def host_tile_structure(related: np.ndarray):
@@ -286,6 +299,7 @@
         t.max_refinement_steps = int(max_refinement_steps)
         t.mixed_tolerance, t.mixed_max_cg = getattr(self, "_mixed", (0.0, 0))
         t.joint_pruning = 0 if getattr(self, "_joint_pruning", True) else -1
+        t.resident_tables = int(getattr(self, "_resident_tables", 0))
         self._route_args = (route, int(max_refinement_steps))
         _check(lib().mmx_problem_set_tuning(self._h, C.byref(t)))
 
@@ -296,6 +310,13 @@
     def set_joint_pruning(self, on: bool = True) -> None:
         self._joint_pruning = bool(on)
         self._set_tuning(*getattr(self, "_route_args", ("auto", 0)))
+
+    def set_resident_tables(self, setting: int = 0) -> None:
+        self._resident_tables = int(setting)
+        self._set_tuning(*getattr(self, "_route_args", ("auto", 0)))
+
+    def resident_tables(self) -> int:
+        return int(lib().mmx_problem_resident_tables(self._h))
 
     def num_solve_joints(self) -> int:
         return int(lib().mmx_problem_num_solve_joints(self._h))
diff --git a/momentum_amd/csrc/mmx_capi.hip b/momentum_amd/csrc/mmx_capi.hip
--- a/momentum_amd/csrc/mmx_capi.hip
+++ b/momentum_amd/csrc/mmx_capi.hip
@@ -218,6 +218,7 @@
   bool autoAbort = false;
   mmx_tuning tuning{};
   int32_t lastRoute = MMX_ROUTE_AUTO;
+  int32_t lastResident = 0;
   mmx::LiveJoints liveJoints;
   bool viewBuilt = false;
   mmx::RigDev vRig{};
@@ -1612,6 +1613,9 @@
   if (tuning->joint_pruning != 0 && tuning->joint_pruning != -1) {
     return fail(MMX_ERR_INVALID_ARGUMENT, "mmx_tuning::joint_pruning: 0 (on) or -1 (off)");
   }
+  if (tuning->resident_tables < -1 || tuning->resident_tables > (MMX_RESIDENT_ROWS | MMX_RESIDENT_UNITS | MMX_RESIDENT_JOINTS)) {
+    return fail(MMX_ERR_INVALID_ARGUMENT, "mmx_tuning::resident_tables: 0 (default), -1 (none) or a mask of MMX_RESIDENT_*");
+  }
   for (int32_t r : tuning->reserved) {
     if (r != 0) {
       return fail(MMX_ERR_INVALID_ARGUMENT, "mmx_tuning::reserved must be zero");
@@ -1630,6 +1634,29 @@
     return 0;
   }
   return solveViewActive(pb) ? pb->liveJoints.numLive : pb->rig->J;
+}
+
+int32_t mmx_problem_resident_tables(const mmx_problem* pb) {
+  return pb != nullptr ? pb->lastResident : 0;
+}
+
+int32_t mmx_host_fused_lds_bytes(const int32_t shape[12], int32_t resident_mask, int32_t offsets, int64_t* bytes, int32_t* chosen_mask) {
+  if (shape == nullptr || bytes == nullptr) {
+    return fail(MMX_ERR_INVALID_ARGUMENT, "mmx_host_fused_lds_bytes: shape / bytes is null");
+  }
+  const int32_t nb = shape[0], J = shape[1], JP = shape[2] < 0 ? shape[1] : shape[2], P = shape[3], U = shape[4], nsrc = shape[5], n = shape[6], cells = shape[7];
+  const int32_t numRec = shape[9], nnz = shape[10], Kp = shape[11];
+  const int32_t all = MMX_RESIDENT_ROWS | MMX_RESIDENT_UNITS | MMX_RESIDENT_JOINTS;
+  if (nb < 1 || nb > 14 || J < 1 || JP < J || P < 1 || U < 0 || nsrc < 0 || n < 0 || n > 16 * nb || cells < 0 || numRec < 0 || nnz < numRec || Kp < 0 || Kp > U || (U - Kp) % 3 != 0 ||
+      resident_mask < 0 || resident_mask > all) {
+    return fail(MMX_ERR_INVALID_ARGUMENT, "mmx_host_fused_lds_bytes: shape out of range");
+  }
+  mmx::FusedResident res{resident_mask, numRec, nnz - numRec, Kp, (U - Kp) / 3, offsets != 0 ? 1 : 0};
+  *bytes = int64_t(mmx::fusedLdsBytes(nb, J, P, U, nsrc, n, cells, shape[8] != 0, 0, 0, false, 0, false, JP, res));
+  if (chosen_mask != nullptr) {
+    *chosen_mask = mmx::fusedResidentChoice(resident_mask, nb, J, JP, P, U, nsrc, n, cells, shape[8] != 0, res);
+  }
+  return MMX_OK;
 }
 
 int32_t mmx_problem_set_enabled(mmx_problem* pb, const uint8_t* enabled) {
@@ -2454,6 +2481,7 @@
   hipStream_t s = static_cast<hipStream_t>(stream);
   const bool escalation = sel.map != nullptr;
   pb->lastRoute = MMX_ROUTE_FUSED;
+  pb->lastResident = 0;
   MMX_HIP(pb->sIters.ensure(B * sizeof(int32_t)));
   MMX_HIP(pb->sStatus.ensure(B * sizeof(int32_t)));
   MMX_HIP(pb->sFinalErr.ensure(B * sizeof(double)));
@@ -2641,6 +2669,7 @@
       return fail(MMX_ERR_UNSUPPORTED, "MMX_ROUTE_WAVE: step_history is the LM schedule's");
     }
     pb->lastRoute = MMX_ROUTE_WAVE;
+    pb->lastResident = 0;
     pb->diagValid = false;
     MMX_HIP(pb->sIters.ensure(B * sizeof(int32_t)));
     MMX_HIP(pb->sStatus.ensure(B * sizeof(int32_t)));
@@ -2685,6 +2714,7 @@
   }
   if (takeFused) {
     pb->lastRoute = MMX_ROUTE_FUSED;
+    pb->lastResident = 0;
     MMX_HIP(pb->sIters.ensure(B * sizeof(int32_t)));
     MMX_HIP(pb->sStatus.ensure(B * sizeof(int32_t)));
     MMX_HIP(pb->sFinalErr.ensure(B * sizeof(double)));
@@ -2724,6 +2754,7 @@
     fp.lmDown = o->lm_down;
     fp.trustRadius = o->trust_region_radius > 0.f ? o->trust_region_radius : 1.f;
     fp.autoAbort = pb->autoAbort ? 1 : 0;
+    fp.resident = pb->tuning.resident_tables == 0 ? mmx::kResAll : (pb->tuning.resident_tables < 0 ? 0 : pb->tuning.resident_tables);
     long long* clk = nullptr;
     if (phaseClocksWanted()) {
       MMX_HIP(pb->sClk.ensure(32 * sizeof(long long)));
@@ -2735,7 +2766,7 @@
       MMX_ZONE("fused solve: all iterations of GaussNewtonSolverT::doIteration in one launch");
       MMX_HIP(pb->sFusedArgs.ensure(mmx::fusedArgsBytes()));
       const SolveView sv = solveView(pb);
-      MMX_HIP(mmx::launchFusedSolve(sv.rig, sv.pb, sv.fd, theta_dev, fst, fp, nullptr, nullptr, clk, pb->sFusedArgs.p, s));
+      MMX_HIP(mmx::launchFusedSolve(sv.rig, sv.pb, sv.fd, theta_dev, fst, fp, nullptr, nullptr, clk, pb->sFusedArgs.p, s, &pb->lastResident));
     }
     if (clk != nullptr) {
       long long h[32];
@@ -2769,6 +2800,7 @@
     return fail(MMX_ERR_UNSUPPORTED, "MMX_ROUTE_WIDE: the tree-refined wide solve is not available for this problem");
   }
   pb->lastRoute = treeRefine ? MMX_ROUTE_WIDE : MMX_ROUTE_EXPLICIT_JACOBIAN;
+  pb->lastResident = 0;
   rc = ensureStepScratch(pb, !treeRefine);
   if (rc != MMX_OK) {
     return rc;
@@ -3240,6 +3272,7 @@
   MMX_HIP(hipSetDevice(pb->rig->device));
   hipStream_t s = static_cast<hipStream_t>(stream);
   pb->lastRoute = MMX_ROUTE_WAVE;
+  pb->lastResident = 0;
   pb->diagValid = false;
   MMX_HIP(pb->sIters.ensure(B * sizeof(int32_t)));
   MMX_HIP(pb->sStatus.ensure(B * sizeof(int32_t)));
diff --git a/momentum_amd/csrc/mmx_fused.hip b/momentum_amd/csrc/mmx_fused.hip
--- a/momentum_amd/csrc/mmx_fused.hip
+++ b/momentum_amd/csrc/mmx_fused.hip
@@ -59,6 +59,32 @@
   const int4* rowRec;
   int32_t numRowRec;
 };
+struct ResidentLds {
+  bool rows = false, extras = false, units = false, joints = false;
+  int *recX = nullptr, *recY = nullptr, *recW = nullptr;
+  float* recZ = nullptr;
+  float* exValue = nullptr;
+  int16_t* exInner = nullptr;
+  int* unitJt = nullptr;
+  float *pos = nullptr, *ori = nullptr;
+  int posStride = 0, oriStride = 0;
+  float *jc = nullptr, *ptOff = nullptr;
+};
+__device__ __forceinline__ ResidentLds residentLdsAt(float* q, int mask, int numRowRec, int numExtra, int U, int Kp, int J) {
+  auto a4 = [](int x) { return (x + 3) & ~3; };
+  ResidentLds rs;
+  rs.rows = (mask & kResRows) != 0, rs.extras = rs.rows && numExtra > 0, rs.units = (mask & kResUnits) != 0, rs.joints = (mask & kResJoints) != 0;
+  const int recStride = a4(numRowRec), Ko = (U - Kp) / 3;
+  rs.recX = reinterpret_cast<int*>(q), rs.recY = rs.recX + recStride, rs.recZ = q + 2 * recStride, rs.recW = rs.recX + 3 * recStride;
+  q += rs.rows ? (rs.extras ? 4 : 3) * recStride : 0;
+  rs.exValue = q, rs.exInner = reinterpret_cast<int16_t*>(q + a4(numExtra));
+  q += rs.extras ? a4(numExtra) + a4((numExtra + 1) / 2) : 0;
+  rs.posStride = a4(Kp), rs.oriStride = a4(Ko);
+  rs.unitJt = reinterpret_cast<int*>(q), rs.pos = q + a4(U), rs.ori = rs.pos + 7 * rs.posStride;
+  q += rs.units ? a4(U) + 7 * rs.posStride + 9 * rs.oriStride : 0;
+  rs.jc = q, rs.ptOff = q + a4(7 * J);
+  return rs;
+}
 template <class I>
 struct FusedViewT {
   int32_t U, Kp;
@@ -323,9 +349,52 @@
   }
 }
 
+template <int kT = 256, typename Gather, typename Store>
+__device__ __forceinline__ void csrRowsFromRecordsLds(const ResidentLds& rs, int numRec, int R, int tid, Gather x, Store out) {
+  for (int t = tid; t < numRec; t += kT) {
+    const int qx = rs.recX[t], qy = rs.recY[t];
+    const int row = qx & 0xffff, span = int(uint32_t(qx) >> 16), in0 = qy & 0xffff, cnt = int(uint32_t(qy) >> 16);
+    auto acc = rs.recZ[t] * x(in0);
+    if (rs.extras) {
+      const int e0 = rs.recW[t] - t;
+      for (int k = e0; k < e0 + cnt - 1; ++k) {
+        acc += rs.exValue[k] * x(rs.exInner[k]);
+      }
+    }
+    out(row, acc);
+    for (int r = row + 1; r < row + span; ++r) {
+      out(r, decltype(acc)(0));
+    }
+    if (t == 0) {
+      for (int r = 0; r < row; ++r) {
+        out(r, decltype(acc)(0));
+      }
+    }
+  }
+}
+__device__ __forceinline__ UnitInput residentUnitInput(const ResidentLds& rs, int Kp, int u) {
+  UnitInput in;
+  const int jt = rs.unitJt[u];
+  in.joint = jt & 0xffff, in.tin = jt >> 16;
+  if (u < Kp) {
+    const float* p = rs.pos + u;
+    const int S = rs.posStride;
+    in.a[0] = p[0], in.a[1] = p[S], in.a[2] = p[2 * S], in.a[3] = 0.f;
+    in.t[0] = p[3 * S], in.t[1] = p[4 * S], in.t[2] = p[5 * S], in.t[3] = 0.f;
+    in.cw = p[6 * S];
+  } else {
+    const float* p = rs.ori + (u - Kp) / 3;
+    const int S = rs.oriStride;
+    in.a[0] = p[0], in.a[1] = p[S], in.a[2] = p[2 * S], in.a[3] = p[3 * S];
+    in.t[0] = p[4 * S], in.t[1] = p[5 * S], in.t[2] = p[6 * S], in.t[3] = p[7 * S];
+    in.cw = p[8 * S];
+  }
+  return in;
+}
+
 template <bool kGlobalTables = false, int kT = 256>
 __device__ __forceinline__ void
-blockFk(const RigView& rig, const FusedLds& s, const float* th, int tid, bool withAxes, long long* clk = nullptr, long long* clkLast = nullptr) {
+blockFk(const RigView& rig, const FusedLds& s, const float* th, int tid, bool withAxes, long long* clk = nullptr, long long* clkLast = nullptr, const ResidentLds& rs = ResidentLds{}) {
   auto stamp = [&](int slot) {
     if (clk != nullptr && blockIdx.x == 0 && threadIdx.x == 0) {
       const long long now = clock64();
@@ -333,12 +402,23 @@
       *clkLast = now;
     }
   };
-  if (kGlobalTables && rig.rowRec != nullptr) {
-    csrRowsFromRecords<kT>(
-        rig.rowRec, rig.numRowRec, rig.ptInner, rig.ptValue, rig.R, tid, [&](int c) { return th[c]; }, [&](int r, float acc) { s.jd[r] = acc + (rig.hasOffsets ? rig.ptOffsets[r] : 0.f); });
+  auto storeJd = [&](int r, float acc) {
+    float off = 0.f;
+    if (rig.hasOffsets) {
+      if (rs.joints) {
+        off = rs.ptOff[r];
+      } else {
+        off = rig.ptOffsets[r];
+      }
+    }
+    s.jd[r] = acc + off;
+  };
+  if (kGlobalTables && rs.rows) {
+    csrRowsFromRecordsLds<kT>(rs, rig.numRowRec, rig.R, tid, [&](int c) { return th[c]; }, storeJd);
+  } else if (kGlobalTables && rig.rowRec != nullptr) {
+    csrRowsFromRecords<kT>(rig.rowRec, rig.numRowRec, rig.ptInner, rig.ptValue, rig.R, tid, [&](int c) { return th[c]; }, storeJd);
   } else if (kGlobalTables) {
-    csrRowsPrefetched<kT>(
-        rig.ptOuter, rig.ptInner, rig.ptValue, rig.R, tid, [&](int c) { return th[c]; }, [&](int r, float acc) { s.jd[r] = acc + (rig.hasOffsets ? rig.ptOffsets[r] : 0.f); });
+    csrRowsPrefetched<kT>(rig.ptOuter, rig.ptInner, rig.ptValue, rig.R, tid, [&](int c) { return th[c]; }, storeJd);
   } else {
     for (int r = tid; r < rig.R; r += kT) {
       const float off = rig.hasOffsets ? rig.ptOffsets[r] : 0.f;
@@ -351,7 +431,18 @@
     }
   }
   float pre[4] = {0.f, 0.f, 0.f, 1.f}, off3[3] = {0.f, 0.f, 0.f};
-  if (tid < rig.J) {
+  if (rs.joints) {
+    if (tid < rig.J) {
+#pragma unroll
+      for (int d = 0; d < 4; ++d) {
+        pre[d] = rs.jc[7 * tid + d];
+      }
+#pragma unroll
+      for (int d = 0; d < 3; ++d) {
+        off3[d] = rs.jc[7 * tid + 4 + d];
+      }
+    }
+  } else if (tid < rig.J) {
 #pragma unroll
     for (int d = 0; d < 4; ++d) {
       pre[d] = rig.preRot[4 * tid + d];
@@ -387,7 +478,11 @@
   stamp(25);
   if (withAxes) {
     for (int j = tid; j < rig.J; j += kT) {
-      fkAxesInPlaceP(rig, j, rig.parent[j], s.js);
+      if (rs.joints) {
+        fkAxesInPlaceQ(rs.jc + 7 * j, j, rig.parent[j], s.js);
+      } else {
+        fkAxesInPlaceP(rig, j, rig.parent[j], s.js);
+      }
     }
     __syncthreads();
   }
@@ -672,19 +767,25 @@
   size_t umomFloats;
   size_t regionFloats;
   size_t genFloats;
+  size_t resRecFloats, resExtraFloats;
+  size_t resUnitFloats;
+  size_t resJointFloats;
   size_t total;
 };
-__host__ __device__ inline FusedLayout fusedLayout(int NB, int J, int P, int U, int nsrc, int n, int numCells, bool cellsBehindRho, int GT, int genRows, bool separateUy = false, size_t csrFloats = 0, bool mix = false) {
+__host__ __device__ inline FusedLayout fusedLayout(
+    int NB, int J, int P, int U, int nsrc, int n, int numCells, bool cellsBehindRho, int GT, int genRows, bool separateUy = false, size_t csrFloats = 0, bool mix = false, int pathJ = -1,
+    const FusedResident& res = FusedResident{}) {
   auto a4 = [](size_t x) { return (x + 3) & ~size_t(3); };
   auto h4 = [&](size_t x) { return a4((x + 1) / 2); };
   auto mx = [](size_t x, size_t y) { return x > y ? x : y; };
   const size_t T = size_t(NB) * (NB + 1) / 2, NP = 16 * size_t(NB);
+  const int JP = pathJ < 0 ? J : pathJ;
   FusedLayout l;
   l.cellOff = cellsBehindRho ? 2 * NP : 0;
   const size_t aux = a4(mx(2 * NP, mx(size_t(nsrc), l.cellOff + size_t(numCells))));
   l.auxOff = separateUy ? a4(3 * size_t(U)) : 0;
   l.uyFloats = separateUy ? l.auxOff + aux : mx(a4(3 * size_t(U)), aux);
-  l.t9 = a4(size_t(kTan) * J);
+  l.t9 = a4(mx(size_t(kTan) * J, mx(U <= JP ? size_t(kC1) * U : 0, nsrc <= kTan * JP ? size_t(nsrc) : 0)));
   l.arenaFloats = mx(size_t(kSrcCh - 1) * size_t(srcStrideFor(nsrc)), 2 * l.t9 + a4(P));
   if (mix) {
     l.arenaFloats = mx(size_t(kSrcCh - 1) * size_t(srcStrideFor(nsrc)), a4(2 * (mixXDoubles(J, nsrc) + mixYDoubles(J, P))));
@@ -699,7 +800,11 @@
   if (mix) {
     fixed = l.uyFloats + 40 + 8 + a4(2 * mixPersistentDoubles(J, P, U, int(NP))) + 2 * h4(J);
   }
-  l.total = meta + fixed + l.genFloats + l.arenaFloats + l.regionFloats + csrFloats;
+  l.resRecFloats = (res.mask & kResRows) ? (res.numExtra > 0 ? 4 : 3) * a4(size_t(res.numRowRec)) : 0;
+  l.resExtraFloats = (res.mask & kResRows) && res.numExtra > 0 ? a4(size_t(res.numExtra)) + h4(size_t(res.numExtra)) : 0;
+  l.resUnitFloats = (res.mask & kResUnits) ? a4(size_t(U)) + 7 * a4(size_t(res.Kp)) + 9 * a4(size_t(res.Ko)) : 0;
+  l.resJointFloats = (res.mask & kResJoints) ? (res.offsets ? 2 : 1) * a4(7 * size_t(J)) : 0;
+  l.total = meta + fixed + l.genFloats + l.arenaFloats + l.regionFloats + csrFloats + l.resRecFloats + l.resExtraFloats + l.resUnitFloats + l.resJointFloats;
   return l;
 }
 
@@ -855,12 +960,19 @@
     const float* th,
     int b,
     int tid,
-    double* unrounded = nullptr) {
+    double* unrounded = nullptr,
+    const ResidentLds& rs = ResidentLds{}) {
   const int lane = tid & 63, wave = tid >> 6;
-  blockFk<kGlobalCsr>(rig, s, th, tid, kStore);
+  blockFk<kGlobalCsr>(rig, s, th, tid, kStore, nullptr, nullptr, rs);
   double e = 0.0;
   for (int u = tid; u < fd.U; u += 256) {
-    const Unit un = evalUnit(pb, s.js, b, u);
+    UnitInput uin;
+    if (rs.units) {
+      uin = residentUnitInput(rs, fd.Kp, u);
+    } else {
+      uin = loadUnitInput(pb, b, u);
+    }
+    const Unit un = evalUnitFrom(pb, uin, s.js, u);
     if (kStore) {
       s.up[3 * u] = un.v.x, s.up[3 * u + 1] = un.v.y, s.up[3 * u + 2] = un.v.z;
       const float rx = un.sigma * un.f.x, ry = un.sigma * un.f.y, rz = un.sigma * un.f.z;
@@ -1338,6 +1450,7 @@
   const int kR = rig.R;
 
   FusedLds s;
+  int resOff = 0;
   int16_t *lParentPos, *lSubSize, *lPosUnitStart, *lPosUnits, *lUnitJoint, *lSolveList, *lDfsJoint, *lLoadedPos, *lColToSolve;
   int *lParent, *lPtOuter = nullptr, *lPtInner = nullptr;
   float *srcGu, *cells, *arena, *lPtValue = nullptr;
@@ -1348,7 +1461,13 @@
   constexpr bool kLeanOps = kFour;
   constexpr bool kLeanAcc = kFour;
   const int kNnz = fd.nnz;
-  const FusedLayout lay = fusedLayout(NB, JL, P, U, nsrc, n, fd.numCells, kRule < 0, kGen ? fd.GT : 0, kGen ? fd.genRows : 0, kTR, 0, kMix);
+  const int JS = kFour ? J : JL;
+  const int resMask = kFour ? fp.resident : 0;
+  const bool resRows = (resMask & kResRows) != 0, resUnits = (resMask & kResUnits) != 0, resJoints = (resMask & kResJoints) != 0;
+  const int numRowRec = rig.numRowRec, numExtra = kNnz - rig.numRowRec;
+  const bool resExtras = numExtra > 0;
+  const FusedLayout lay = fusedLayout(
+      NB, JS, P, U, nsrc, n, fd.numCells, kRule < 0, kGen ? fd.GT : 0, kGen ? fd.genRows : 0, kTR, 0, kMix, JL, FusedResident{resMask, numRowRec, numExtra, fd.Kp, (U - fd.Kp) / 3, rig.ptOffsetsNonZero != 0 ? 1 : 0});
   MixLds m{};
   m.layoutJ = JL;
   {
@@ -1363,15 +1482,15 @@
     s.mTin = reinterpret_cast<int*>(take(nsrc));
     s.mInfo = reinterpret_cast<int*>(take(nsrc));
     s.mW = take(nsrc);
-    lParent = reinterpret_cast<int*>(take(JL));
-    lParentPos = takeS(JL);
-    lSubSize = takeS(JL);
-    lPosUnitStart = takeS(JL + 1);
+    lParent = reinterpret_cast<int*>(take(JS));
+    lParentPos = takeS(JS);
+    lSubSize = takeS(JS);
+    lPosUnitStart = takeS(JS + 1);
     lPosUnits = takeS(U);
     lUnitJoint = takeS(U);
     lSolveList = takeS(n);
-    lDfsJoint = takeS(JL);
-    lLoadedPos = takeS(JL);
+    lDfsJoint = takeS(JS);
+    lLoadedPos = takeS(JS);
     lColToSolve = takeS(P);
     if (kCsrLds) {
       lPtOuter = reinterpret_cast<int*>(take(kR + 1));
@@ -1380,11 +1499,11 @@
     }
     if (kMix) {
       s.th = s.js = s.up = s.us = s.ur = s.g = s.d0 = nullptr;
-      m.lo = takeS(JL);
-      m.hi = takeS(JL);
+      m.lo = takeS(JS);
+      m.hi = takeS(JS);
     } else {
       s.th = take(P);
-      s.js = take(size_t(kJs) * JL);
+      s.js = take(size_t(kJs) * JS);
       s.up = take(3 * size_t(U));
       s.ur = take(3 * size_t(U));
       s.us = take(U);
@@ -1406,22 +1525,25 @@
     arena = take(lay.arenaFloats);
     if (kMix) {
       m.X = reinterpret_cast<double*>(arena);
-      m.Y = m.X + mixXDoubles(JL, nsrc);
+      m.Y = m.X + mixXDoubles(JS, nsrc);
     }
     s.srcT = arena;
     s.tanOwn = arena, s.jd = arena + lay.t9, s.tanPre = arena + lay.t9, s.dfull = arena + 2 * lay.t9;
     float* region = p;
-    s.fkA = reinterpret_cast<double*>(take(fkBufFloats(JL)));
+    s.fkA = reinterpret_cast<double*>(take(fkBufFloats(JS)));
     s.fkB = reinterpret_cast<double*>(p);
-    s.own2 = take(size_t(kC2) * JL);
-    s.sub2 = take(size_t(kC2) * JL);
+    s.own2 = take(size_t(kC2) * JS);
+    s.sub2 = take(size_t(kC2) * JS);
     s.umom = take(lay.umomFloats);
     s.own1 = region, s.sub1 = s.umom;
     s.L = region;
+    if (kFour) {
+      resOff = int((region + lay.regionFloats) - smem);
+    }
     if (kMix) {
-      double* d = reinterpret_cast<double*>(smem + (lay.total - alignUp4(2 * mixPersistentDoubles(JL, P, U, NP))));
+      double* d = reinterpret_cast<double*>(smem + (lay.total - alignUp4(2 * mixPersistentDoubles(JS, P, U, NP))));
       m.th = d, d += P;
-      m.js = d, d += size_t(kJsD) * JL;
+      m.js = d, d += size_t(kJsD) * JS;
       m.up = d, d += 3 * size_t(U);
       m.uf = d, d += 3 * size_t(U);
       m.us = d, d += U;
@@ -1433,6 +1555,15 @@
     }
   }
 
+  auto resView = [&]() {
+    ResidentLds r{};
+    if (kFour) {
+      int o = __builtin_amdgcn_readfirstlane(resOff), mk = __builtin_amdgcn_readfirstlane(fp.resident);
+      asm volatile("" : "+s"(o), "+s"(mk));
+      r = residentLdsAt(smem + o, mk, rig.numRowRec, fd.nnz - rig.numRowRec, U, fd.Kp, J);
+    }
+    return r;
+  };
   float* thg = theta + size_t(b) * P;
   if (kMix) {
     const float* th0 = sel.thetaInit != nullptr ? sel.thetaInit + size_t(b) * P : thg;
@@ -1467,6 +1598,54 @@
     for (int i = tid; i < kNnz; i += 256) {
       lPtInner[i] = rig.ptInner[i];
       lPtValue[i] = rig.ptValue[i];
+    }
+  }
+  if (kFour) {
+    const ResidentLds rs = resView();
+    if (resRows) {
+      const int4* rec = asGlobal(rig.ptRowRec);
+      for (int t = tid; t < numRowRec; t += 256) {
+        const int4 q = rec[t];
+        rs.recX[t] = q.x, rs.recY[t] = q.y, rs.recZ[t] = __int_as_float(q.z);
+        if (resExtras) {
+          rs.recW[t] = q.w;
+          const int cnt = int(uint32_t(q.y) >> 16);
+          for (int k = q.w + 1; k < q.w + cnt; ++k) {
+            rs.exValue[k - t - 1] = asGlobal(rig.ptValue)[k];
+            rs.exInner[k - t - 1] = int16_t(asGlobal(rig.ptInner)[k]);
+          }
+        }
+      }
+    }
+    if (resUnits) {
+      const int Kp = fd.Kp;
+      for (int u = tid; u < U; u += 256) {
+        const UnitInput in = loadUnitInput(pb, b, u);
+        rs.unitJt[u] = in.joint | (in.tin << 16);
+        if (u < Kp) {
+          float* o = rs.pos + u;
+          const int S = rs.posStride;
+          o[0] = in.a[0], o[S] = in.a[1], o[2 * S] = in.a[2], o[3 * S] = in.t[0], o[4 * S] = in.t[1], o[5 * S] = in.t[2], o[6 * S] = in.cw;
+        } else if ((u - Kp) % 3 == 0) {
+          float* o = rs.ori + (u - Kp) / 3;
+          const int S = rs.oriStride;
+          o[0] = in.a[0], o[S] = in.a[1], o[2 * S] = in.a[2], o[3 * S] = in.a[3];
+          o[4 * S] = in.t[0], o[5 * S] = in.t[1], o[6 * S] = in.t[2], o[7 * S] = in.t[3], o[8 * S] = in.cw;
+        }
+      }
+    }
+    if (resJoints) {
+      for (int i = tid; i < 4 * J; i += 256) {
+        rs.jc[7 * (i >> 2) + (i & 3)] = asGlobal(rig.preRot)[i];
+      }
+      for (int i = tid; i < 3 * J; i += 256) {
+        rs.jc[7 * (i / 3) + 4 + (i - 3 * (i / 3))] = asGlobal(rig.offset)[i];
+      }
+      if (rig.ptOffsetsNonZero != 0) {
+        for (int r = tid; r < kR; r += 256) {
+          rs.ptOff[r] = asGlobal(rig.ptOffsets)[r];
+        }
+      }
     }
   }
   for (int i = tid; i < U; i += 256) {
@@ -1618,12 +1797,19 @@
       curError = (s.red[0] + s.red[1]) + (s.red[2] + s.red[3]);
       MMX_CLK(1)
     } else {
-    blockFk<!kCsrLds>(rv, s, s.th, tid, true, MODE == 2 ? dbgClk : nullptr, &clkLast);
+    blockFk<!kCsrLds>(rv, s, s.th, tid, true, MODE == 2 ? dbgClk : nullptr, &clkLast, resView());
     MMX_CLK(1)
     {
       double e = 0.0;
+      const ResidentLds rs = resView();
       for (int u = tid; u < U; u += 256) {
-        const Unit un = evalUnitFrom(pb, (!kLateUnit && u == tid) ? uin0 : loadUnitInput(pb, b, u), s.js, u);
+        UnitInput uin;
+        if (kFour && rs.units) {
+          uin = residentUnitInput(rs, fv.Kp, u);
+        } else {
+          uin = (!kLateUnit && u == tid) ? uin0 : loadUnitInput(pb, b, u);
+        }
+        const Unit un = evalUnitFrom(pb, uin, s.js, u);
         s.up[3 * u] = un.v.x, s.up[3 * u + 1] = un.v.y, s.up[3 * u + 2] = un.v.z;
         const float rx = un.sigma * un.f.x, ry = un.sigma * un.f.y, rz = un.sigma * un.f.z;
         s.ur[3 * u] = rx, s.ur[3 * u + 1] = ry, s.ur[3 * u + 2] = rz;
@@ -2280,6 +2466,8 @@
             }
             od(r, a);
           }
+        } else if (kFour && (fp.resident & kResRows) != 0) {
+          csrRowsFromRecordsLds<256>(resView(), rv.numRowRec, rv.R, tid, xd, od);
         } else if (rv.rowRec != nullptr) {
           csrRowsFromRecords<256>(rv.rowRec, rv.numRowRec, rv.ptInner, rv.ptValue, rv.R, tid, xd, od);
         } else {
@@ -2618,7 +2806,7 @@
         s.dfull[fv.solveList[c]] -= s.d0[c];
       }
       __syncthreads();
-      const double eNew = blockError<kGen, false, !kCsrLds>(rig, rv, pb, fv, s, s.dfull, b, tid);
+      const double eNew = blockError<kGen, false, !kCsrLds>(rig, rv, pb, fv, s, s.dfull, b, tid, nullptr, resView());
       const float predicted = trDg + (trMu - 1e-20f) * trDn2;
       const float rho = float((curError - eNew) / double(predicted));
       if (rho < 0.25f) {
@@ -2653,7 +2841,7 @@
       }
       __syncthreads();
       double eFull = 0.0;
-      const double eNew = blockError<kGen, kReuse, !kCsrLds>(rig, rv, pb, fv, s, s.dfull, b, tid, &eFull);
+      const double eNew = blockError<kGen, kReuse, !kCsrLds>(rig, rv, pb, fv, s, s.dfull, b, tid, &eFull, resView());
       const float rho = predicted > 0.f ? float((curError - eNew) / double(predicted)) : -1.f;
       if (st.stepHistory != nullptr && tid == 0) {
         double* sh = st.stepHistory + (size_t(b) * fp.maxIterations + it) * 2;
@@ -2700,7 +2888,7 @@
           s.dfull[fv.solveList[c]] -= scale * s.d0[c];
         }
         __syncthreads();
-        const double eNew = blockError<kGen, kReuse, !kCsrLds>(rig, rv, pb, fv, s, s.dfull, b, tid, &stateError);
+        const double eNew = blockError<kGen, kReuse, !kCsrLds>(rig, rv, pb, fv, s, s.dfull, b, tid, &stateError, resView());
         if ((curError - eNew) >= (doLineSearch == 2 ? double(1e-4f * scale) * gd : double(scale * scaledError))) {
           break;
         }
@@ -3691,8 +3879,34 @@
   auto a4 = [](size_t x) { return (x + 3) & ~size_t(3); };
   return a4(7 * size_t(J) + 1) + 2 * a4(nnz);
 }
-size_t fusedLdsBytes(int NB, int J, int P, int U, int nsrc, int n, int numCells, bool cellsBehindRho, int GT, int genRows, bool separateUy, size_t csrFloats, bool mix) {
-  return fusedLayout(NB, J, P, U, nsrc, n, numCells, cellsBehindRho, GT, genRows, separateUy, csrFloats, mix).total * sizeof(float);
+size_t fusedLdsBytes(int NB, int J, int P, int U, int nsrc, int n, int numCells, bool cellsBehindRho, int GT, int genRows, bool separateUy, size_t csrFloats, bool mix, int pathJ, const FusedResident& res) {
+  return fusedLayout(NB, J, P, U, nsrc, n, numCells, cellsBehindRho, GT, genRows, separateUy, csrFloats, mix, pathJ, res).total * sizeof(float);
+}
+size_t fusedClassBudget(size_t bytes) {
+  const size_t cu = 160 * 1024;
+  for (size_t wg = 4; wg > 1; --wg) {
+    const size_t share = (cu / wg) & ~size_t(1023);
+    if (bytes <= share) {
+      return share;
+    }
+  }
+  return cu;
+}
+int fusedResidentChoice(int wanted, int NB, int J, int pathJ, int P, int U, int nsrc, int n, int numCells, bool cellsBehindRho, FusedResident shape) {
+  auto bytes = [&](int mask) {
+    shape.mask = mask;
+    return fusedLdsBytes(NB, J, P, U, nsrc, n, numCells, cellsBehindRho, 0, 0, false, 0, false, pathJ, shape);
+  };
+  const size_t budget = fusedClassBudget(bytes(0));
+  int mask = 0;
+  const int order[3] = {kResRows, kResJoints, kResUnits};
+  for (int bit : order) {
+    const bool applies = bit == kResRows ? shape.numRowRec > 0 : (bit == kResUnits ? U > 0 : J > 0 && J <= 256);
+    if ((wanted & bit) != 0 && applies && bytes(mask | bit) <= budget) {
+      mask |= bit;
+    }
+  }
+  return mask;
 }
 #endif
 
@@ -3703,14 +3917,27 @@
     const FusedDev& fd,
     float* theta,
     const SolveStateDev& st,
-    const FusedParams& fp,
+    const FusedParams& fpIn,
     float* dbgH,
     float* dbgG,
     long long* dbgClk,
     void* argsBuf,
-    hipStream_t stream) {
+    hipStream_t stream,
+    int32_t* residentOut) {
   constexpr bool kFourL = FusedFour<NB, kTR, kGen, kRule>::value;
-  const size_t lds = fusedLdsBytes(NB, rig.layoutJ, rig.P, fd.U, fd.nsrc, fd.n, fd.numCells, kRule < 0, kGen ? fd.GT : 0, kGen ? fd.genRows : 0, kTR, kFourL ? 0 : fusedCsrFloats(rig.layoutJ, fd.nnz));
+  FusedResident res{0, rig.ptRowRec != nullptr ? rig.numRowRec : 0, 0, fd.Kp, (fd.U - fd.Kp) / 3, rig.ptOffsetsNonZero != 0 ? 1 : 0};
+  res.numExtra = fd.nnz - res.numRowRec;
+  FusedParams fp = fpIn;
+  fp.resident = 0;
+  if (kFourL) {
+    const int wanted = fpIn.resident & (pb.instPosParent == nullptr && pb.instOriParent == nullptr ? kResAll : ~kResUnits);
+    fp.resident = res.mask = fusedResidentChoice(wanted, NB, rig.J, rig.layoutJ, rig.P, fd.U, fd.nsrc, fd.n, fd.numCells, kRule < 0, res);
+  }
+  if (residentOut != nullptr) {
+    *residentOut = fp.resident;
+  }
+  const size_t lds = fusedLdsBytes(
+      NB, kFourL ? rig.J : rig.layoutJ, rig.P, fd.U, fd.nsrc, fd.n, fd.numCells, kRule < 0, kGen ? fd.GT : 0, kGen ? fd.genRows : 0, kTR, kFourL ? 0 : fusedCsrFloats(rig.layoutJ, fd.nnz), false, rig.layoutJ, res);
   if (lds > 160 * 1024) {
     return hipErrorInvalidValue;
   }
@@ -3748,34 +3975,35 @@
     float* dbgG,
     long long* dbgClk,
     void* argsBuf,
-    hipStream_t stream) {
+    hipStream_t stream,
+    int32_t* residentOut) {
   if (fd.GT > 0) {
     if (fp.stepRule == 2) {
       return hipErrorInvalidValue;
     }
     if (dbgH != nullptr || dbgG != nullptr) {
-      return launchFusedMode<NB, 1, false, true>(rig, pb, fd, theta, st, fp, dbgH, dbgG, nullptr, argsBuf, stream);
-    }
-    return launchFusedMode<NB, 0, false, true>(rig, pb, fd, theta, st, fp, nullptr, nullptr, nullptr, argsBuf, stream);
+      return launchFusedMode<NB, 1, false, true>(rig, pb, fd, theta, st, fp, dbgH, dbgG, nullptr, argsBuf, stream, residentOut);
+    }
+    return launchFusedMode<NB, 0, false, true>(rig, pb, fd, theta, st, fp, nullptr, nullptr, nullptr, argsBuf, stream, residentOut);
   }
   if (fp.stepRule == 2) {
-    return launchFusedMode<NB, 0, true>(rig, pb, fd, theta, st, fp, nullptr, nullptr, nullptr, argsBuf, stream);
+    return launchFusedMode<NB, 0, true>(rig, pb, fd, theta, st, fp, nullptr, nullptr, nullptr, argsBuf, stream, residentOut);
   }
   if (dbgClk != nullptr) {
-    return launchFusedMode<NB, 2, false>(rig, pb, fd, theta, st, fp, dbgH, dbgG, dbgClk, argsBuf, stream);
+    return launchFusedMode<NB, 2, false>(rig, pb, fd, theta, st, fp, dbgH, dbgG, dbgClk, argsBuf, stream, residentOut);
   }
   if (dbgH != nullptr || dbgG != nullptr) {
-    return launchFusedMode<NB, 1, false>(rig, pb, fd, theta, st, fp, dbgH, dbgG, dbgClk, argsBuf, stream);
+    return launchFusedMode<NB, 1, false>(rig, pb, fd, theta, st, fp, dbgH, dbgG, dbgClk, argsBuf, stream, residentOut);
   }
   if (pb.M == pb.rowsJoint) {
     if (fp.stepRule == 0 && fp.doLineSearch == 0) {
-      return launchFusedMode<NB, 0, false, false, 0>(rig, pb, fd, theta, st, fp, nullptr, nullptr, nullptr, argsBuf, stream);
+      return launchFusedMode<NB, 0, false, false, 0>(rig, pb, fd, theta, st, fp, nullptr, nullptr, nullptr, argsBuf, stream, residentOut);
     }
     if (fp.stepRule == 1) {
-      return launchFusedMode<NB, 0, false, false, 1>(rig, pb, fd, theta, st, fp, nullptr, nullptr, nullptr, argsBuf, stream);
-    }
-  }
-  return launchFusedMode<NB, 0, false>(rig, pb, fd, theta, st, fp, dbgH, dbgG, dbgClk, argsBuf, stream);
+      return launchFusedMode<NB, 0, false, false, 1>(rig, pb, fd, theta, st, fp, nullptr, nullptr, nullptr, argsBuf, stream, residentOut);
+    }
+  }
+  return launchFusedMode<NB, 0, false>(rig, pb, fd, theta, st, fp, dbgH, dbgG, dbgClk, argsBuf, stream, residentOut);
 }
 
 template <int NB>
@@ -3808,8 +4036,8 @@
 
 #define MMX_FUSED_ARGS \
   const RigDev &rig, const ProblemDev &pb, const FusedDev &fd, float *theta, const SolveStateDev &st, const FusedParams &fp, \
-      float *dbgH, float *dbgG, long long *dbgClk, void *argsBuf, hipStream_t stream
-#define MMX_FUSED_PASS rig, pb, fd, theta, st, fp, dbgH, dbgG, dbgClk, argsBuf, stream
+      float *dbgH, float *dbgG, long long *dbgClk, void *argsBuf, hipStream_t stream, int32_t *residentOut
+#define MMX_FUSED_PASS rig, pb, fd, theta, st, fp, dbgH, dbgG, dbgClk, argsBuf, stream, residentOut
 
 hipError_t launchFusedGroup0(int nb, MMX_FUSED_ARGS);
 hipError_t launchFusedGroup1(int nb, MMX_FUSED_ARGS);
diff --git a/momentum_amd/csrc/mmx_kernels.hpp b/momentum_amd/csrc/mmx_kernels.hpp
--- a/momentum_amd/csrc/mmx_kernels.hpp
+++ b/momentum_amd/csrc/mmx_kernels.hpp
@@ -134,6 +134,18 @@
   float mixTol;
   int32_t mixMaxCg;
   int32_t autoAbort;
+  int32_t resident;
+};
+
+constexpr int kResRows = 1;
+constexpr int kResUnits = 2;
+constexpr int kResJoints = 4;
+constexpr int kResAll = kResRows | kResUnits | kResJoints;
+struct FusedResident {
+  int mask;
+  int numRowRec, numExtra;
+  int Kp, Ko;
+  int offsets;
 };
 
 struct MixSelect {
@@ -142,7 +154,9 @@
   const float* thetaInit;
 };
 
-size_t fusedLdsBytes(int NB, int J, int P, int U, int nsrc, int n, int numCells, bool cellsBehindRho, int GT = 0, int genRows = 0, bool separateUy = false, size_t csrFloats = 0, bool mix = false);
+size_t fusedLdsBytes(int NB, int J, int P, int U, int nsrc, int n, int numCells, bool cellsBehindRho, int GT = 0, int genRows = 0, bool separateUy = false, size_t csrFloats = 0, bool mix = false, int pathJ = -1, const FusedResident& res = FusedResident{});
+size_t fusedClassBudget(size_t bytes);
+int fusedResidentChoice(int wanted, int NB, int J, int pathJ, int P, int U, int nsrc, int n, int numCells, bool cellsBehindRho, FusedResident shape);
 size_t fusedCsrFloats(int J, int nnz);
 size_t treeNormalEquationsLdsBytes(int J, int P, int U, int nsrc, int n, int GT = 0, int genRows = 0);
 size_t treeRefineLdsBytes(int J, int P, int U, int n, int genRows);
@@ -187,7 +201,8 @@
     float* dbgG,
     long long* dbgClk,
     void* argsBuf,
-    hipStream_t stream);
+    hipStream_t stream,
+    int32_t* residentOut = nullptr);
 size_t fusedArgsBytes();
 bool fusedMixedUsable(int J, int P, int U, int nsrc, int n, int numCells);
 hipError_t launchFusedMixed(
```
